# jhbastek/PhysicsInformedDiffusionModels

Measured on AMD Instinct MI355X. Metric: training samples/sec (UNet+PDE-residual step), 64x64 Darcy, higher is better.
Workload: dtype f32

## Files before the change

include/pidm.h:

```cpp
#ifndef PIDM_H
#define PIDM_H
#include <stddef.h>
#include <stdint.h>

#ifdef __cplusplus
extern "C" {
#endif

#define PIDM_ABI_VERSION 1

int pidm_version(void);
const char* pidm_last_error(void);
const char* pidm_backend(void);

int pidm_prof_enable(int on);
int pidm_prof_collect(double* ms4, long long* launches4, double* work4);
int pidm_prof_kernels_begin(void* stream);
long long pidm_prof_kernels_collect(char* buf, size_t cap);

int pidm_darcy_residual_fwd(const float* x0, const float* f_s, float inv_h0, float inv_h1,
                            float* residual, int B, int P, void* stream);
int pidm_darcy_residual_bwd(const float* x0, const float* grad_res, float inv_h0, float inv_h1,
                            float* grad_x0, int B, int P, void* stream);

size_t pidm_darcy_loss_ws(int B, int P);
int pidm_darcy_loss_fwd_bwd(const float* x0, const float* x0_pred, const float* f_s, const float* p2w,
                            const float* inv_var, float c_data, float c_residual, float inv_h0, float inv_h1,
                            float* residual, float* grad_x0_pred, float* out_scalars, void* workspace,
                            int B, int P, void* stream);
int pidm_darcy_loss_fwd_bwd_t(const float* x0, const float* x0_pred, const float* f_s, const int64_t* t,
                              const float* p2w_table, const float* var_table, float c_data, float c_residual,
                              float inv_h0, float inv_h1, float* residual, float* grad_x0_pred, float* out_scalars,
                              void* workspace, int B, int P, void* stream);

int pidm_darcy_jacobian_max(const float* x0, float inv_h0, float inv_h1, float* max_dr_dp, int B, int P, void* stream);

#define PIDM_STENCIL_MAX_OPS 5
#define PIDM_STENCIL_MAX_TAPS 49
typedef struct pidm_stencil_op {
  const int32_t* table;
  int mio, max_offset, ntaps;
} pidm_stencil_op;
int pidm_stencil_apply(const float* x, long long x_stride, const pidm_stencil_op* ops_host, float* const* outs_host, int K,
                       long long out_stride, int N, int H, int W, int periodic, void* stream);
int pidm_stencil_apply_adjoint(const float* const* gs_host, long long g_stride, const pidm_stencil_op* ops_host, int K,
                               const float* add, long long add_stride, float* gx, long long gx_stride, int N, int H, int W,
                               int periodic, void* stream);
size_t pidm_darcy_general_ws(int B, int P);
int pidm_darcy_residual_general_fwd(const float* x0, const float* f_s, const pidm_stencil_op* ops4_host, int periodic, float bc1_sign,
                                    float* residual, void* workspace, int B, int P, void* stream);
int pidm_darcy_residual_general_bwd(const float* x0, const float* grad_res, const pidm_stencil_op* ops4_host, int periodic,
                                    float bc1_sign, float* grad_x0, void* workspace, int B, int P, void* stream);

int pidm_qsample_nhwc(const float* x0, const float* eps, const float* a_t, const float* am1_t, float* xt_nhwc,
                      int B, int C, int HW, void* stream);
int pidm_qsample_nhwc_t(const float* x0, const float* eps, const int64_t* t, const float* a_table, const float* am1_table,
                        float* xt_nhwc, int B, int C, int HW, void* stream);
int pidm_psample_update(const float* x0_pred, const float* x_t, const float* z, float c1, float c2, float sigma,
                        float* x_prev, size_t n, void* stream);

size_t pidm_clip_adam_ws_bytes(void);
int pidm_clip_adam_step(float* param, const float* grad, float* exp_avg, float* exp_avg_sq, size_t n, double lr, double beta1,
                        double beta2, double eps, long long step, double max_norm, float* total_norm_out, void* workspace,
                        void* stream);

int pidm_clip_adam_ema_step(float* param, const float* grad, float* exp_avg, float* exp_avg_sq, float* ema_shadow, size_t n,
// ... 38 lines not shown
int pidm_mech_fields(const float* u_dofs, const float* rho, const float* kloc, int kloc_stride, const int32_t* elem_dofs, int nel,
                     double nu, float* fields, int B, void* stream);

typedef struct pidm_unet pidm_unet;
typedef struct pidm_unet_cfg {
  int dim;
  int channels;
  int out_dim;
  int n_levels;
  int dim_mults[8];
  int heads;
  int dim_head;
  int groups;
  int init_kernel;
  int image_size;
  int sigmoid_last_channel;
  int self_condition;
} pidm_unet_cfg;

int pidm_unet_create(const pidm_unet_cfg* cfg, pidm_unet** out);
void pidm_unet_destroy(pidm_unet* h);
int pidm_unet_num_params(const pidm_unet* h);
const char* pidm_unet_param_name(const pidm_unet* h, int i);
size_t pidm_unet_param_numel(const pidm_unet* h, int i);
size_t pidm_unet_workspace_bytes(const pidm_unet* h, int B, int training);
int pidm_unet_bind(pidm_unet* h, const void* const* param_ptrs_host, void* const* grad_ptrs_host);
int pidm_unet_forward(pidm_unet* h, const float* x_nhwc, const int64_t* t, float* out_nchw, int B,
                      int save_for_backward, int repack_weights, void* workspace, size_t workspace_bytes, void* stream);
int pidm_unet_num_cond_params(const pidm_unet* h);
int pidm_unet_enable_cond(pidm_unet* h, int on);
int pidm_unet_set_condition(pidm_unet* h, const float* cond_nhwc);
int pidm_unet_backward(pidm_unet* h, const float* grad_out_nchw, float* grad_x_nhwc, int B, void* workspace,
                       size_t workspace_bytes, void* stream);

int pidm_unet_set_grad_events(pidm_unet* h, int n_phases, void* const* events);
int pidm_unet_grad_phase_range(const pidm_unet* h, int n_phases, int phase, int* first_param, int* end_param);

typedef struct pidm_conv_desc {
  int B, Hi, Wi;
  int C0, C1;
  int ld0, ld1;
  int Cout;
  int KH, KW, stride, pad;
  int transposed;
  int out_nchw;
  int ldo;
} pidm_conv_desc;
size_t pidm_conv_packed_weight_floats(const pidm_conv_desc* d);
int pidm_conv_pack_weights(const pidm_conv_desc* d, const float* w_ref, float* w_packed, int mode, void* stream);
int pidm_conv_forward(const pidm_conv_desc* d, const float* src0, const float* src1, const float* w_packed,
                      const float* bias, const float* residual, float* out, void* stream);
int pidm_conv_forward_gn_partials(const pidm_conv_desc* d, const float* src0, const float* src1, const float* w_packed,
                                  const float* bias, float* out, int groups, double* partial, void* stream);
size_t pidm_conv_dgrad_packed_weight_floats(const pidm_conv_desc* d);
int pidm_conv_dgrad(const pidm_conv_desc* d, const float* dy, int ld_dy, const float* w_packed_dgrad,
                    const float* residual, float* dx, int ld_dx, void* stream);
size_t pidm_conv_wgrad_ws(const pidm_conv_desc* d);
int pidm_conv_wgrad(const pidm_conv_desc* d, const float* src0, const float* src1, const float* dy, int ld_dy,
                    float* dw_ref, float* dbias, void* workspace, void* stream);

size_t pidm_linear_attention_ws(int B, int N, int heads);
int pidm_linear_attention_forward(const float* qkv, float* out, float* kstat, float* ctx, float* qstat, int B, int N,
                                  int heads, void* workspace, void* stream);
int pidm_linear_attention_backward(const float* qkv, const float* kstat, const float* qstat, const float* ctx,
                                   const float* d_out, float* dqkv, int B, int N, int heads, void* workspace, void* stream);
int pidm_linear_attention_out_forward(const float* qkv, const float* w_out, const float* bias, const float* residual, float* y,
                                      int Cout, float* kstat, float* ctx, float* qstat, int B, int N, int heads, void* workspace,
                                      void* stream);
size_t pidm_linear_attention_out_backward_ws(int B, int N, int heads, int Cout);
int pidm_linear_attention_out_backward(const float* qkv, const float* kstat, const float* qstat, const float* ctx,
                                       const float* d_y, int ld_dy, const float* w_out, int Cout, float* dqkv, float* dw_out,
                                       int B, int N, int heads, void* workspace, void* stream);

size_t pidm_lap_ws(int B, int N, int heads, int C);
size_t pidm_lap_saved_floats(int B, int heads, int C);
int pidm_lap_forward(const float* xn, const float* w_qkv, const float* w_out, const float* bias, const float* resid, float* y,
                     float* saved, float* qstat, int C, int B, int N, int heads, void* workspace, void* stream);
int pidm_lap_backward(const float* xn, const float* dy, const float* w_qkv, const float* w_out, const float* saved,
                      const float* qstat, float* d_xn, float* d_w_qkv, float* d_w_out, int C, int B, int N, int heads,
                      void* workspace, void* stream);

int pidm_debug_stream_trace(unsigned long long* out256);
int pidm_debug_conv_rs_trace(unsigned long long* out4);
int pidm_debug_lap_trace(unsigned long long* out256);
long long pidm_debug_reduce_table_uploads(void);
int pidm_debug_launch_counts(long long* out4);
int pidm_comm_available(void);
int pidm_comm_unique_id(void* out128);
int pidm_comm_init(int rank, int world, const void* unique_id128, void** comm);
int pidm_allreduce_f32(void* comm, float* buf, size_t count, int average, void* stream);
int pidm_comm_destroy(void* comm);

int pidm_reload_knobs(void);

#ifdef __cplusplus
}
#endif
#endif
```

physicsinformeddiffusionmodels_amd/_engine.py:

```python
from __future__ import annotations

import contextlib
import ctypes as C
import math

import torch

from ._lib import PidmError, PidmLib, UnetCfg, get_lib, ptr, stream_ptr, vp


class UnetEngine:

    def __init__(self, model, image_size: int, lib: PidmLib | None = None):
        self.lib = lib or get_lib()
        cfg = UnetCfg()
        cfg.dim = model.dim
        cfg.channels = model.channels
        cfg.out_dim = model.out_dim
        cfg.n_levels = len(model.dim_mults)
        for i, m in enumerate(model.dim_mults):
            cfg.dim_mults[i] = int(m)
        cfg.heads = model.attn_heads
        cfg.dim_head = model.attn_dim_head
        cfg.groups = model.resnet_groups
        cfg.init_kernel = model.init_kernel_size
        cfg.image_size = image_size
        cfg.sigmoid_last_channel = int(bool(model.sigmoid_last_channel))
        cfg.self_condition = int(bool(model.self_condition))
        self.image_size = image_size
        self.handle = vp()
        self.lib.check(self.lib.pidm_unet_create(C.byref(cfg), C.byref(self.handle)), "pidm_unet_create")
        n = self.lib.pidm_unet_num_params(self.handle)
        self.names = [self.lib.pidm_unet_param_name(self.handle, i).decode() for i in range(n)]
        self.numels = [self.lib.pidm_unet_param_numel(self.handle, i) for i in range(n)]
        named = dict(model.named_parameters())
        missing = [k for k in self.names if k not in named]
        if missing:
            raise PidmError(f"engine parameter(s) not found in the model: {missing[:4]}")
        for k, ne in zip(self.names, self.numels):
            if named[k].numel() != ne:
                raise PidmError(f"parameter {k}: numel {named[k].numel()} != engine's {ne}")
        self.params = [named[k] for k in self.names]
        self.n_cond = self.lib.pidm_unet_num_cond_params(self.handle)
        self.cond_enabled = False
        self.flat_grad = None
        self.grad_views = None
        self.early_grad = None
        self.early_views = None
        self.early_generation = -1
        self._bound_key = None
        self.workspace = None
        self.backward_calls = 0
        self.tape_generation = 0
        self.tape_busy = False
        self._packed_for = None

    def __del__(self):
        try:
            if self.handle:
                self.lib.pidm_unet_destroy(self.handle)
        except Exception:
            pass

    def _flat_buffer(self, dev):
        total = sum(self.numels)
        flat = torch.zeros(total, dtype=torch.float32, device=dev)
        views, off = [], 0
        for p, ne in zip(self.params, self.numels):
            views.append(flat[off:off + ne].view(p.shape))
            off += ne
        return flat, views

    def _ensure_bound(self, need_grad: bool, early: bool = False):
        dev = self.params[0].device
        for p in self.params:
            if p.dtype != torch.float32 or not p.is_contiguous() or p.device != dev:
                raise PidmError("engine parameters must be contiguous fp32 tensors on one device")
        if need_grad and (self.flat_grad is None or self.flat_grad.device != dev):
            self.flat_grad, self.grad_views = self._flat_buffer(dev)
            self._bound_key = None
        if early and (self.early_grad is None or self.early_grad.device != dev):
            self.early_grad, self.early_views = self._flat_buffer(dev)
        with_grad = need_grad or self.flat_grad is not None
        target = (self.early_views if early else self.grad_views) if with_grad else None
        key = (tuple(p.data_ptr() for p in self.params), with_grad and target[0].data_ptr())
        if key != self._bound_key:
            n = len(self.params)
            pp = (vp * n)(*[vp(p.data_ptr()) for p in self.params])
            if with_grad:
                gp = (vp * n)(*[vp(g.data_ptr()) for g in target])
                self.lib.check(self.lib.pidm_unet_bind(self.handle, pp, gp), "pidm_unet_bind")
            else:
                self.lib.check(self.lib.pidm_unet_bind(self.handle, pp, None), "pidm_unet_bind")
            self._bound_key = key

    def _ensure_workspace(self, B: int, training: bool, device):
        nbytes = self.lib.pidm_unet_workspace_bytes(self.handle, B, int(training))
        if nbytes == 0:
            raise PidmError("pidm_unet_workspace_bytes: " + self.lib.lib.pidm_last_error().decode())
        if self.workspace is None or self.workspace.numel() < nbytes + 256 or self.workspace.device != torch.device(device):
            self.workspace = None
            self.workspace = torch.empty(nbytes + 256, dtype=torch.uint8, device=device)
        return self.workspace

    def forward(self, x_nhwc: torch.Tensor, t: torch.Tensor, training: bool, repack: bool = True,
                cond: torch.Tensor | None = None, early: bool = False, frozen=None) -> torch.Tensor:
        B = x_nhwc.shape[0]
        dev = x_nhwc.device
        self._ensure_bound(training, early=early)
        if cond is not None:
            if not self.cond_enabled:
                self.lib.check(self.lib.pidm_unet_enable_cond(self.handle, 1), "pidm_unet_enable_cond")
                self.cond_enabled = True
            self.lib.check(self.lib.pidm_unet_set_condition(self.handle, ptr(cond)), "pidm_unet_set_condition")
        ws = self._ensure_workspace(B, training, dev)
        P = self.image_size
        out = torch.empty(B, self.lib_out_dim, P, P, dtype=torch.float32, device=dev)
        base = ws.data_ptr()
        al = (-base) % 256
        if frozen is not None and not training and repack:
            key = (frozen, self._bound_key, base)
            repack = key != self._packed_for
            self._packed_for = key
        else:
            self._packed_for = None
        self.lib.check(self.lib.pidm_unet_forward(self.handle, ptr(x_nhwc), ptr(t), ptr(out), B, int(training), int(repack),
                                                  vp(base + al), ws.numel() - al, stream_ptr(dev)), "pidm_unet_forward")
        return out

    def backward(self, grad_out: torch.Tensor, want_grad_x: bool, channels: int):
        B = grad_out.shape[0]
        dev = grad_out.device
        ws = self.workspace
        gx = torch.empty(B, self.image_size * self.image_size, channels, dtype=torch.float32, device=dev) if want_grad_x else None
        base = ws.data_ptr()
        al = (-base) % 256
        self.lib.check(self.lib.pidm_unet_backward(self.handle, ptr(grad_out), ptr(gx), B, vp(base + al), ws.numel() - al,
                                                   stream_ptr(dev)), "pidm_unet_backward")
        return gx


class _TapeLease:

    __slots__ = ("engine", "generation")

    def __init__(self, engine, generation):
        self.engine, self.generation = engine, generation

    def release(self):
        eng = self.engine
        if eng is not None and eng.tape_generation == self.generation:
            eng.tape_busy = False
        self.engine = None

    def __del__(self):
        try:
            self.release()
        except Exception:
            pass


class _UnetFunction(torch.autograd.Function):

    @staticmethod
    def forward(ctx, engine: UnetEngine, x_nhwc, t, anchor, training: bool, cond=None, primary=None, frozen=None):
        ctx.engine = engine
        ctx.primary = primary if primary is not None else engine
        ctx.used_cond = cond is not None
        ctx.x_requires_grad = x_nhwc.requires_grad
        ctx.channels = x_nhwc.shape[-1]
        ctx.training = training
        if training:
            engine.tape_generation += 1
            engine.tape_busy = True
        ctx.generation = engine.tape_generation
        ctx.lease = _TapeLease(engine, engine.tape_generation) if training else None
        out = engine.forward(x_nhwc, t, training=training, cond=cond, frozen=frozen)
        if cond is not None:
            ctx.save_for_backward(out, x_nhwc, cond)
        else:
            ctx.save_for_backward(out, x_nhwc)
        return out

    @staticmethod
    def backward(ctx, grad_out):
        eng = ctx.engine
        if not ctx.training:
            raise PidmError("backward through a forward that ran without gradient tracking")
        if ctx.generation != eng.tape_generation:
            raise PidmError("the engine's activation tape was overwritten by a later training-mode forward of the same "
                            "model: only the latest differentiable UNet call can be differentiated (the two calls of "
                            "x0_estimation='sample' get one tape each through DenoisingDiffusion.ddim_sample_x0)")
        primary = ctx.primary
        first = eng.params[0]
        if primary.flat_grad is None:
            primary._ensure_bound(True)
        aliased = first.grad is not None and first.grad.data_ptr() == primary.grad_views[0].data_ptr()
        prev = primary.flat_grad.clone() if (aliased and eng is primary) else None
        gx = eng.backward(grad_out.contiguous(), ctx.x_requires_grad, ctx.channels)
        if prev is not None:
            eng.flat_grad.add_(prev)
        if eng is not primary:
            if aliased:
                primary.flat_grad.add_(eng.flat_grad)
            else:
                primary.flat_grad.copy_(eng.flat_grad)
        if ctx.lease is not None:
            ctx.lease.release()
        eng.tape_busy = False
        primary.backward_calls += 1 if (eng is primary and prev is None) else 2
        n_plain = len(eng.params) - eng.n_cond
        for i, (p, g) in enumerate(zip(eng.params, primary.grad_views)):
            if not p.requires_grad:
                continue
            if i >= n_plain and not ctx.used_cond:
                continue
            if p.grad is None:
                p.grad = g
            elif p.grad.data_ptr() != g.data_ptr():
                p.grad.add_(eng.grad_views[i] if eng is not primary else g)
        return None, gx, None, None, None, None, None, None


def get_engine(model, image_size: int, lib: PidmLib | None = None, slot: int = 0) -> UnetEngine:
    cache = model.__dict__.setdefault("_engines", {})
    key = (image_size, id(lib), slot)
    eng = cache.get(key)
    if eng is None:
        eng = UnetEngine(model, image_size, lib)
        eng.lib_out_dim = model.out_dim
        cache[key] = eng
    return eng


def used_parameter_names(model, image_size: int = 64, with_condition: bool = False):
    eng = get_engine(model, image_size)
    return list(eng.names) if with_condition else list(eng.names[:len(eng.names) - eng.n_cond])


@contextlib.contextmanager
def frozen_weights(model):
    prev = getattr(model, "_pidm_frozen", None)
    model._pidm_frozen = prev if prev is not None else object()
    try:
        yield
    finally:
        model._pidm_frozen = prev


def unet_apply(model, x, time, lib: PidmLib | None = None, cond=None, x_self_cond=None):
    video = False
    if x.dim() == 3:
        B, N, Cc = x.shape
        P = int(math.isqrt(N))
        if P * P != N:
            raise ValueError('Input [B, P*P, C] needs a square number of pixels.')
        x_nhwc = x
    elif x.dim() == 4:
        B, Cc, P, P2 = x.shape
        x_nhwc = x.permute(0, 2, 3, 1).reshape(B, P * P2, Cc)
    elif x.dim() == 5:
        video = True
        B, Cc, F_, P, P2 = x.shape
# ... 4 lines not shown
        raise ValueError('Input must be image [BxCxPxP] or image sequence [BxCxFxPxP].')
    if Cc != model.channels:
        raise ValueError(f'expected {model.channels} input channels, got {Cc}')
    if lib is None and not x.is_cuda:
        raise PidmError("Unet3D.forward needs tensors on an MI355X (cuda device): the gfx950 engine has no CPU fallback")
    if model.self_condition:
        if x_self_cond is None:
            sc = torch.zeros_like(x_nhwc)
        elif x_self_cond.dim() == 3:
            sc = x_self_cond
        elif x_self_cond.dim() == 4:
            sc = x_self_cond.permute(0, 2, 3, 1).reshape(B, P * P, Cc)
        else:
            sc = x_self_cond[:, :, 0].permute(0, 2, 3, 1).reshape(B, P * P, Cc)
        x_nhwc = torch.cat((sc.to(x_nhwc.dtype), x_nhwc), dim=-1)
    elif x_self_cond is not None:
        raise ValueError('x_self_cond given but the model was built with self_condition=False')
    x_nhwc = x_nhwc.contiguous().float()
    t = time.to(device=x.device, dtype=torch.int64).contiguous()
    if t.numel() != B:
        raise ValueError('time must have one entry per batch element')
    primary = eng = get_engine(model, P, lib)
    anchor = eng.params[0]
    training = torch.is_grad_enabled() and (anchor.requires_grad or x_nhwc.requires_grad)
    slot = getattr(model, "_pidm_tape_slot", None)
    if training and slot:
        eng = get_engine(model, P, lib, int(slot))
    if not training and eng.tape_busy:
        eng = get_engine(model, P, lib, slot=-1)
    if cond is not None:
        if cond.shape != (B, P * P, model.channels):
            raise ValueError(f'cond must be [B, P*P, {model.channels}], got {tuple(cond.shape)}')
        cond = cond.detach().contiguous().float()
    out = _UnetFunction.apply(eng, x_nhwc, t, anchor, training, cond, primary, getattr(model, "_pidm_frozen", None))
    if video:
        out = out.unsqueeze(2)
    return out
```

physicsinformeddiffusionmodels_amd/_lib.py:

```python
from __future__ import annotations

import ctypes as C
import os

_HERE = os.path.dirname(os.path.abspath(__file__))
DEFAULT_LIB = os.path.join(_HERE, "csrc", "libpidm_hip.so")

c_float_p = C.POINTER(C.c_float)
vp = C.c_void_p


class UnetCfg(C.Structure):
    _fields_ = [("dim", C.c_int), ("channels", C.c_int), ("out_dim", C.c_int), ("n_levels", C.c_int),
                ("dim_mults", C.c_int * 8), ("heads", C.c_int), ("dim_head", C.c_int), ("groups", C.c_int),
                ("init_kernel", C.c_int), ("image_size", C.c_int), ("sigmoid_last_channel", C.c_int),
                ("self_condition", C.c_int)]


class ConvDesc(C.Structure):
    _fields_ = [("B", C.c_int), ("Hi", C.c_int), ("Wi", C.c_int), ("C0", C.c_int), ("C1", C.c_int),
                ("ld0", C.c_int), ("ld1", C.c_int), ("Cout", C.c_int), ("KH", C.c_int), ("KW", C.c_int),
                ("stride", C.c_int), ("pad", C.c_int), ("transposed", C.c_int), ("out_nchw", C.c_int),
                ("ldo", C.c_int)]

# ... 4 lines not shown

class PidmError(RuntimeError):
    pass


_loaded: list = []


class PidmLib:
    def __init__(self, path: str | None = None):
        path = path or DEFAULT_LIB
        if not os.path.exists(path):
            raise PidmError(
                f"{path} not found: the gfx950 engine is not built. Run `python -c 'import __graft_entry__ as g; "
                f"g.build()'` (or `make -C physicsinformeddiffusionmodels_amd/csrc`). There is no CPU fallback.")
        self.path = path
        self.lib = C.CDLL(path)
        L = self.lib
        L.pidm_version.restype = C.c_int
        L.pidm_last_error.restype = C.c_char_p
        L.pidm_backend.restype = C.c_char_p
        i, f, sz = C.c_int, C.c_float, C.c_size_t
        self._sig("pidm_debug_reduce_table_uploads", [], C.c_longlong)
        self._sig("pidm_debug_launch_counts", [C.POINTER(C.c_longlong)])
        self._sig("pidm_prof_enable", [i])
        self._sig("pidm_prof_collect", [C.POINTER(C.c_double), C.POINTER(C.c_longlong), C.POINTER(C.c_double)])
        self._sig("pidm_prof_kernels_begin", [vp])
        self._sig("pidm_prof_kernels_collect", [C.c_char_p, sz], C.c_longlong)
        self._sig("pidm_darcy_residual_fwd", [vp, vp, f, f, vp, i, i, vp])
        self._sig("pidm_darcy_residual_bwd", [vp, vp, f, f, vp, i, i, vp])
        self._sig("pidm_darcy_loss_ws", [i, i], sz)
        self._sig("pidm_darcy_loss_fwd_bwd", [vp, vp, vp, vp, vp, f, f, f, f, vp, vp, vp, vp, i, i, vp])
        self._sig("pidm_darcy_loss_fwd_bwd_t", [vp, vp, vp, vp, vp, vp, f, f, f, f, vp, vp, vp, vp, i, i, vp])
        self._sig("pidm_darcy_jacobian_max", [vp, f, f, vp, i, i, vp])
        ll, ops = C.c_longlong, C.POINTER(StencilOp)
        self._sig("pidm_stencil_apply", [vp, ll, ops, C.POINTER(vp), i, ll, i, i, i, i, vp])
        self._sig("pidm_stencil_apply_adjoint", [C.POINTER(vp), ll, ops, i, vp, ll, vp, ll, i, i, i, i, vp])
        self._sig("pidm_darcy_general_ws", [i, i], sz)
        self._sig("pidm_darcy_residual_general_fwd", [vp, vp, ops, i, f, vp, vp, i, i, vp])
        self._sig("pidm_darcy_residual_general_bwd", [vp, vp, ops, i, f, vp, vp, i, i, vp])
        self._sig("pidm_qsample_nhwc", [vp, vp, vp, vp, vp, i, i, i, vp])
        self._sig("pidm_qsample_nhwc_t", [vp, vp, vp, vp, vp, vp, i, i, i, vp])
        self._sig("pidm_psample_update", [vp, vp, vp, f, f, f, vp, sz, vp])
        self._sig("pidm_mech_apply", [vp, vp, vp, vp, i, vp, vp, i, vp, vp, i, vp])
        self._sig("pidm_mech_solve_ws_bytes", [i, i], sz)
        self._sig("pidm_mech_solve", [vp, vp, vp, i, vp, vp, i, f, f, f, i, C.c_double, vp, vp, vp, vp, vp, vp, i, vp])
        self._sig("pidm_floating_material", [vp, f, i, vp, i, vp])
        self._sig("pidm_darcy_gen_lds_bytes", [i], sz)
        self._sig("pidm_darcy_gen", [vp, vp, i, vp, i, C.c_double, C.c_double, C.c_double, vp, vp, i, C.c_double, vp, vp, vp, vp, vp,
                                     i, vp])
        d = C.c_double
        self._sig("pidm_simp_ws_bytes", [i, i], sz)
        self._sig("pidm_simp_step", [vp, vp, vp, vp, vp, vp, i, vp, vp, i, d, d, d, d, i, i, d, vp, vp, vp, vp, vp, vp, vp, i, vp])
        self._sig("pidm_mech_fields", [vp, vp, vp, i, vp, i, d, vp, i, vp])
        self._sig("pidm_unet_num_cond_params", [vp])
        self._sig("pidm_unet_enable_cond", [vp, i])
        self._sig("pidm_unet_set_condition", [vp, vp])
        self._sig("pidm_clip_adam_ws_bytes", [], sz)
        self._sig("pidm_clip_adam_step", [vp, vp, vp, vp, sz, C.c_double, C.c_double, C.c_double, C.c_double, C.c_longlong,
                                          C.c_double, vp, vp, vp])
        self._sig("pidm_clip_adam_ema_step", [vp, vp, vp, vp, vp, sz, C.c_double, C.c_double, C.c_double, C.c_double, C.c_longlong,
                                              C.c_double, C.c_double, vp, vp, vp])
        self._sig("pidm_ema_update", [vp, vp, sz, C.c_double, vp])
        self._sig("pidm_mech_loss_ws", [i], sz)
        self._sig("pidm_mech_loss_fwd_bwd", [vp, vp, vp, vp, vp, vp, vp, f, f, f, f, vp, i, vp, vp, i, vp, vp, vp, i, vp])
        self._sig("pidm_bilinear_resize", [vp, vp, i, i, i, vp])
        self._sig("pidm_mech_residual_fwd", [vp, vp, vp, vp, i, vp, vp, i, vp, vp, vp, i, vp])
        self._sig("pidm_mech_residual_bwd", [vp, vp, vp, i, vp, vp, i, vp, vp, vp, vp, i, vp])
        self._sig("pidm_unet_create", [C.POINTER(UnetCfg), C.POINTER(vp)])
        self._sig("pidm_unet_destroy", [vp], None)
        self._sig("pidm_unet_num_params", [vp])
        self._sig("pidm_unet_param_name", [vp, i], C.c_char_p)
        self._sig("pidm_unet_param_numel", [vp, i], sz)
        self._sig("pidm_unet_workspace_bytes", [vp, i, i], sz)
        self._sig("pidm_unet_bind", [vp, C.POINTER(vp), C.POINTER(vp)])
        self._sig("pidm_unet_forward", [vp, vp, vp, vp, i, i, i, vp, sz, vp])
        self._sig("pidm_unet_backward", [vp, vp, vp, i, vp, sz, vp])
        self._sig("pidm_unet_set_grad_events", [vp, i, C.POINTER(vp)])
        self._sig("pidm_unet_grad_phase_range", [vp, i, i, C.POINTER(C.c_int), C.POINTER(C.c_int)])
        self._sig("pidm_conv_packed_weight_floats", [C.POINTER(ConvDesc)], sz)
        self._sig("pidm_conv_pack_weights", [C.POINTER(ConvDesc), vp, vp, i, vp])
        self._sig("pidm_conv_forward", [C.POINTER(ConvDesc), vp, vp, vp, vp, vp, vp, vp])
        self._sig("pidm_conv_dgrad_packed_weight_floats", [C.POINTER(ConvDesc)], sz)
        self._sig("pidm_conv_dgrad", [C.POINTER(ConvDesc), vp, i, vp, vp, vp, i, vp])
        self._sig("pidm_conv_forward_gn_partials", [C.POINTER(ConvDesc), vp, vp, vp, vp, vp, i, vp, vp])
        self._sig("pidm_conv_wgrad_ws", [C.POINTER(ConvDesc)], sz)
        self._sig("pidm_conv_wgrad", [C.POINTER(ConvDesc), vp, vp, vp, i, vp, vp, vp, vp])
        self._sig("pidm_linear_attention_ws", [i, i, i], sz)
        self._sig("pidm_linear_attention_forward", [vp, vp, vp, vp, vp, i, i, i, vp, vp])
        self._sig("pidm_linear_attention_backward", [vp, vp, vp, vp, vp, vp, i, i, i, vp, vp])
        self._sig("pidm_linear_attention_out_forward", [vp, vp, vp, vp, vp, i, vp, vp, vp, i, i, i, vp, vp])
        self._sig("pidm_linear_attention_out_backward_ws", [i, i, i, i], sz)
        self._sig("pidm_linear_attention_out_backward", [vp, vp, vp, vp, vp, i, vp, i, vp, vp, i, i, i, vp, vp])
        self._sig("pidm_lap_ws", [i, i, i, i], sz)
        self._sig("pidm_lap_saved_floats", [i, i, i], sz)
        self._sig("pidm_lap_forward", [vp, vp, vp, vp, vp, vp, vp, vp, i, i, i, i, vp, vp])
        self._sig("pidm_lap_backward", [vp, vp, vp, vp, vp, vp, vp, vp, vp, i, i, i, i, vp, vp])
        self._sig("pidm_debug_stream_trace", [vp])
        self._sig("pidm_debug_conv_rs_trace", [C.POINTER(C.c_ulonglong)])
        self._sig("pidm_debug_lap_trace", [vp])
        self._sig("pidm_reload_knobs", [])
        self._sig("pidm_comm_available", [])
        self._sig("pidm_comm_unique_id", [vp])
        self._sig("pidm_comm_init", [i, i, vp, C.POINTER(vp)])
        self._sig("pidm_allreduce_f32", [vp, vp, sz, i, vp])
        self._sig("pidm_comm_destroy", [vp])
        _loaded.append(self)
        if L.pidm_version() != 1:
            raise PidmError(f"{path}: ABI version {L.pidm_version()} != 1")

# ... 49 lines not shown
```

physicsinformeddiffusionmodels_amd/csrc/k_attn.hip:

```cpp
#include "pidm_launch.h"

namespace pidm {

static const int DH = 32;

__device__ __forceinline__ float fexp(float x) { return __expf(x); }

__global__ void __launch_bounds__(256) la_kstats_kernel(const float* __restrict__ qkv, int N, int HD, int nseg,
                                                        float* __restrict__ kpart, float* __restrict__ kstat) {
  __shared__ float sm[4][64], ssum[4][64];
  const int b = blockIdx.y, seg = blockIdx.z, tid = threadIdx.x, cl = tid & 63, rl = tid >> 6;
  const int j = blockIdx.x * 64 + cl;
  const int per = (N + nseg - 1) / nseg;
  const int n_lo = seg * per, n_hi = (n_lo + per < N) ? n_lo + per : N;
  float m = -3.0e38f, s = 0.f;
  if (j < HD) {
    const float* base = qkv + (size_t)b * N * 3 * HD + HD + j;
    int n = n_lo + rl;
    for (; n + 28 < n_hi; n += 32) {
      float v[8];
#pragma unroll
      for (int u = 0; u < 8; ++u) v[u] = base[(size_t)(n + 4 * u) * 3 * HD];
      float gm = v[0];
#pragma unroll
// ... 17 lines not shown
  __syncthreads();
  if (rl == 0 && j < HD) {
    float M = fmaxf(fmaxf(sm[0][cl], sm[1][cl]), fmaxf(sm[2][cl], sm[3][cl]));
    float S = 0.f;
    for (int r = 0; r < 4; ++r) S += ssum[r][cl] * fexp(sm[r][cl] - M);
    if (kstat) {
      kstat[((size_t)b * HD + j) * 2] = M;
      kstat[((size_t)b * HD + j) * 2 + 1] = 1.f / S;
    } else {
      kpart[(((size_t)b * nseg + seg) * HD + j) * 2] = M;
      kpart[(((size_t)b * nseg + seg) * HD + j) * 2 + 1] = S;
    }
  }
}
__global__ void la_kstats_final_kernel(const float* __restrict__ kpart, int B, int HD, int nseg, float* __restrict__ kstat) {
  const int i = blockIdx.x * blockDim.x + threadIdx.x;
  if (i >= B * HD) return;
  const int b = i / HD, j = i % HD;
  float M = -3.0e38f;
  for (int sg = 0; sg < nseg; ++sg) M = fmaxf(M, kpart[(((size_t)b * nseg + sg) * HD + j) * 2]);
  float S = 0.f;
  for (int sg = 0; sg < nseg; ++sg) {
    const float* p = kpart + (((size_t)b * nseg + sg) * HD + j) * 2;
    S += p[1] * fexp(p[0] - M);
  }
  kstat[(size_t)i * 2] = M;
  kstat[(size_t)i * 2 + 1] = 1.f / S;
}

template <int MODE>
__global__ void __launch_bounds__(256) la_nreduce_kernel(const float* __restrict__ qkv, const float* __restrict__ stat,
                                                         const float* __restrict__ dA, const float* __restrict__ ctx,
                                                         float* __restrict__ Dpart, int N, int heads, float scale,
                                                         float* __restrict__ Dfinal, float* __restrict__ rowdot, float alpha) {
  __shared__ float red[4][1024];
  const int bh = blockIdx.x, b = bh / heads, h = bh % heads;
  const int ns = blockIdx.y, NS = gridDim.y;
  const int HD = heads * DH;
  const int tid = threadIdx.x, lane = tid & 63, half = lane >> 5, l31 = lane & 31;
  const int wave = __builtin_amdgcn_readfirstlane(tid >> 6);
  f32x16 acc;
  for (int r = 0; r < 16; ++r) acc[r] = 0.f;
  const float* q0 = qkv + (size_t)b * N * 3 * HD;
  float cm = 0.f, cis = 0.f;
  if (MODE == 0) {
    cm = stat[((size_t)b * HD + h * DH + l31) * 2];
    cis = stat[((size_t)b * HD + h * DH + l31) * 2 + 1];
  }
  const int per_blk = (N + NS - 1) / NS;
  const int blk_lo = ns * per_blk, blk_hi = (blk_lo + per_blk < N) ? blk_lo + per_blk : N;
  const int per = (blk_hi - blk_lo + 3) / 4;
  const int n_lo = blk_lo + wave * per, n_hi = (n_lo + per < blk_hi) ? n_lo + per : blk_hi;
  int n0 = n_lo;
  {
    constexpr int UNR = 4;
    const int la = half * 3 * HD + (MODE == 0 ? HD : 0) + h * DH + l31;
    const int lb = (MODE == 0) ? half * 3 * HD + 2 * HD + h * DH + l31 : half * HD + h * DH + l31;
    const int ls = (half * heads + h) * 2;
    for (; n0 + 2 * UNR <= n_hi; n0 += 2 * UNR) {
      const float* qrow = q0 + (size_t)n0 * 3 * HD;
      const float* brow = (MODE == 0) ? qrow : dA + ((size_t)b * N + n0) * HD;
      const float* srow = (MODE == 0) ? nullptr : stat + ((size_t)b * N + n0) * heads * 2;
      float av[UNR], bvv[UNR];
      float2 qs[UNR];
#pragma unroll
      for (int u = 0; u < UNR; ++u) {
        av[u] = (qrow + (size_t)(2 * u) * 3 * HD)[la];
        bvv[u] = (brow + (size_t)(2 * u) * (MODE == 0 ? 3 * HD : HD))[lb];
        if (MODE == 1) qs[u] = *reinterpret_cast<const float2*>(srow + (size_t)(2 * u) * heads * 2 + ls);
      }
#pragma unroll
      for (int u = 0; u < UNR; ++u) {
        const float a = (MODE == 0) ? fexp(av[u] - cm) * cis : fexp(av[u] - qs[u].x) * qs[u].y * scale;
        acc = __builtin_amdgcn_mfma_f32_32x32x2f32(a, bvv[u], acc, 0, 0, 0);
      }
    }
  }
  for (; n0 < n_hi; n0 += 2) {
// ... 892 lines not shown
#pragma unroll 8
      for (int s2 = 0; s2 < 32; ++s2)
        acc = __builtin_amdgcn_mfma_f32_32x32x2f32(sdS_[(32 * t + l31) * LS + 2 * s2 + half], sk[2 * s2 + half][l31], acc, 0, 0, 0);
    } else {
#pragma unroll 8
      for (int s2 = 0; s2 < 32; ++s2)
        acc = __builtin_amdgcn_mfma_f32_32x32x2f32(sdS_[(2 * s2 + half) * LS + 32 * t + l31], sq[2 * s2 + half][l31], acc, 0, 0, 0);
    }
    const float f = wave < 2 ? scale : 1.f;
    const size_t col = (wave < 2 ? 0 : HD) + h * DH + l31;
#pragma unroll
    for (int r = 0; r < 16; ++r)
      out[((size_t)b * N + 32 * t + (r & 3) + 8 * (r >> 2) + 4 * half) * 3 * HD + col] = acc[r] * f;
  }
}

static int la_nsplit(int N) {
  int ns = N / 512;
  if (ns < 1) ns = 1;
  if (ns > 8) ns = 8;
  return ns;
}
static int la_kseg(int N) {
  int s = N / 256;
  if (s < 1) s = 1;
  if (s > 16) s = 16;
  return s;
}
size_t la_scratch_floats(int B, int N, int heads) {
  const size_t a = (size_t)B * la_kseg(N) * heads * DH * 2, b = (size_t)B * heads * la_nsplit(N) * 1024;
  return a + b + (size_t)heads * DH * 128 + 64;
}

int launch_la_forward(const float* qkv, float* kstat, float* ctx, float* attn, float* qstat, int B, int N, int heads,
                      float* scratch, hipStream_t st) {
  const int HD = heads * DH;
  const float scale = 0.17677669529663687f;
  const int nseg = la_kseg(N), NS = la_nsplit(N);
  float* kpart = scratch;
  float* dpart = scratch + (size_t)B * nseg * HD * 2;
  hipLaunchKernelGGL(la_kstats_kernel, dim3(cdiv(HD, 64), B, nseg), dim3(256), 0, st, qkv, N, HD, nseg, kpart, nseg == 1 ? kstat : nullptr);
  PIDM_CHECK_LAUNCH("la_kstats_kernel");
  if (nseg > 1) {
    hipLaunchKernelGGL(la_kstats_final_kernel, dim3(cdiv(B * HD, 256)), dim3(256), 0, st, kpart, B, HD, nseg, kstat);
    PIDM_CHECK_LAUNCH("la_kstats_final_kernel");
  }
  hipLaunchKernelGGL(HIP_KERNEL_NAME(la_nreduce_kernel<0>), dim3(B * heads, NS), dim3(256), 0, st, qkv, kstat, nullptr, nullptr,
                     dpart, N, heads, scale, NS == 1 ? ctx : nullptr, nullptr, 1.f / (float)N);
  PIDM_CHECK_LAUNCH("la_context");
  if (NS > 1) {
    hipLaunchKernelGGL(HIP_KERNEL_NAME(la_nreduce_final_kernel<0>), dim3(B * heads), dim3(256), 0, st, dpart, nullptr, ctx, nullptr, NS,
                       1.f / (float)N);
    PIDM_CHECK_LAUNCH("la_context_final");
  }
  const size_t npix = (size_t)B * N;
  if (N % 32 == 0)
    hipLaunchKernelGGL(HIP_KERNEL_NAME(la_out_kernel<true>), dim3((unsigned)((npix + 127) / 128), (npix + 127) / 128 < 1024 ? heads : 1), dim3(256), 0, st, qkv, ctx, attn,
                       qstat, N, heads, npix, scale);
  else
    hipLaunchKernelGGL(HIP_KERNEL_NAME(la_out_kernel<false>), dim3((unsigned)((npix + 127) / 128), (npix + 127) / 128 < 1024 ? heads : 1), dim3(256), 0, st, qkv, ctx, attn,
                       qstat, N, heads, npix, scale);
  PIDM_CHECK_LAUNCH("la_out_kernel");
  return 0;
}

int launch_la_backward(const float* qkv, const float* kstat, const float* qstat, const float* ctx, const float* dA, float* dctx,
                       float* rowdot, float* dqkv, int B, int N, int heads, float* scratch, hipStream_t st) {
  const float scale = 0.17677669529663687f;
  const int NS = la_nsplit(N);
  float* dpart = scratch;
  hipLaunchKernelGGL(HIP_KERNEL_NAME(la_nreduce_kernel<1>), dim3(B * heads, NS), dim3(256), 0, st, qkv, qstat, dA, ctx, dpart, N, heads,
                     scale, NS == 1 ? dctx : nullptr, rowdot, 1.f);
  PIDM_CHECK_LAUNCH("la_dctx");
  if (NS > 1) {
    hipLaunchKernelGGL(HIP_KERNEL_NAME(la_nreduce_final_kernel<1>), dim3(B * heads), dim3(256), 0, st, dpart, ctx, dctx, rowdot, NS, 1.f);
    PIDM_CHECK_LAUNCH("la_dctx_final");
  }
  if (N % 32 == 0 && N >= 64) {
    const size_t npix = (size_t)B * N;
    int ppb = N % 128 == 0 ? 128 : (N % 64 == 0 ? 64 : 32);
    (void)npix;
    if (const char* pe = knob("PIDM_LA_PPB")) { const int v = atoi(pe); if ((v == 32 || v == 64 || v == 128) && N % v == 0) ppb = v; }
    PIDM_PROF_NAME("la_bwd_pix_mfma_kernel");
    hipLaunchKernelGGL(la_bwd_pix_mfma_kernel, dim3((unsigned)((size_t)B * N / ppb), heads), dim3(2 * ppb), 0, st, qkv, kstat, qstat, ctx,
                       dctx, rowdot, dA, dqkv, N, heads, scale, ppb);
  } else {
    hipLaunchKernelGGL(la_bwd_pix_kernel, dim3(cdiv(N, 256), B * heads), dim3(256), 0, st, qkv, kstat, qstat, ctx, dctx, rowdot,
                       dA, dqkv, N, heads, scale);
  }
  PIDM_CHECK_LAUNCH("la_bwd_pix_kernel");
  return 0;
}

bool la_fused_ok(int N, int heads, int Cout, int ld_dy) {
  const bool off = knob("PIDM_NO_LA_FUSED") != nullptr;
  return !off && N % 128 == 0 && (Cout == 32 || Cout == 64 || Cout == 128) && (ld_dy & 3) == 0 && heads >= 1 && heads <= 14;
}
int launch_la_forward_fused(const float* qkv, float* kstat, float* ctx, float* qstat, const float* w_out, const float* bias,
                            const float* resid, float* y, int Cout, int B, int N, int heads, float* scratch, hipStream_t st) {
  if (!la_fused_ok(N, heads, Cout, Cout)) return fail("fused attention forward: N=%d Cout=%d not eligible", N, Cout);
  const int HD = heads * DH;
  const float scale = 0.17677669529663687f;
  const int nseg = la_kseg(N), NS = la_nsplit(N);
  float* kpart = scratch;
  float* dpart = scratch + (size_t)B * nseg * HD * 2;
  hipLaunchKernelGGL(la_kstats_kernel, dim3(cdiv(HD, 64), B, nseg), dim3(256), 0, st, qkv, N, HD, nseg, kpart, nseg == 1 ? kstat : nullptr);
  PIDM_CHECK_LAUNCH("la_kstats_kernel");
  if (nseg > 1) {
    hipLaunchKernelGGL(la_kstats_final_kernel, dim3(cdiv(B * HD, 256)), dim3(256), 0, st, kpart, B, HD, nseg, kstat);
    PIDM_CHECK_LAUNCH("la_kstats_final_kernel");
  }
  hipLaunchKernelGGL(HIP_KERNEL_NAME(la_nreduce_kernel<0>), dim3(B * heads, NS), dim3(256), 0, st, qkv, kstat, nullptr, nullptr,
                     dpart, N, heads, scale, NS == 1 ? ctx : nullptr, nullptr, 1.f / (float)N);
  PIDM_CHECK_LAUNCH("la_context");
  if (NS > 1) {
    hipLaunchKernelGGL(HIP_KERNEL_NAME(la_nreduce_final_kernel<0>), dim3(B * heads), dim3(256), 0, st, dpart, nullptr, ctx, nullptr, NS,
                       1.f / (float)N);
    PIDM_CHECK_LAUNCH("la_context_final");
  }
  float* wt = dpart + (size_t)B * heads * NS * 1024;
  hipLaunchKernelGGL(la_wt_kernel, dim3(cdiv(Cout * HD, 256)), dim3(256), 0, st, w_out, wt, Cout, HD);
  PIDM_CHECK_LAUNCH("la_wt_kernel");
  const dim3 grid((unsigned)((size_t)B * N / 128));
  if (Cout == 32)
    hipLaunchKernelGGL(HIP_KERNEL_NAME(la_out_proj_kernel<1>), grid, dim3(256), 0, st, qkv, ctx, wt, bias, resid, y, qstat, N, heads, scale);
  else if (Cout == 64)
    hipLaunchKernelGGL(HIP_KERNEL_NAME(la_out_proj_kernel<2>), grid, dim3(256), 0, st, qkv, ctx, wt, bias, resid, y, qstat, N, heads, scale);
  else
    hipLaunchKernelGGL(HIP_KERNEL_NAME(la_out_proj_kernel<4>), grid, dim3(256), 0, st, qkv, ctx, wt, bias, resid, y, qstat, N, heads, scale);
  PIDM_CHECK_LAUNCH("la_out_proj_kernel");
  return 0;
}

bool la_fused_pays(int B, int N) {
  const char* mw = knob("PIDM_LA_FUSED_MIN_WGS");
  const long min_wgs = mw ? atol(mw) : 256;
  return (long)B * N / 128 >= min_wgs;
}
size_t la_fused_scratch_floats(int B, int N, int heads, int Cout) {
  return (size_t)B * heads * la_nsplit(N) * (Cout / 32) * 1024 + 64;
}
int launch_la_backward_fused(const float* qkv, const float* kstat, const float* qstat, const float* ctx, const float* dy, int ld_dy,
                             const float* w_out, int Cout, float* dctx, float* rowdot, float* dqkv, float* dwpart, int B, int N,
                             int heads, float* scratch, hipStream_t st) {
  if (!la_fused_ok(N, heads, Cout, ld_dy)) return fail("fused attention backward: N=%d Cout=%d not eligible", N, Cout);
  const float scale = 0.17677669529663687f;
  const int NS = la_nsplit(N);
  float* gpart = scratch;
  const dim3 grid(B * heads, NS);
#define PIDM_LA_G(NT_)                                                                                                        \
  {                                                                                                                           \
    hipLaunchKernelGGL(HIP_KERNEL_NAME(la_g_kernel<NT_>), grid, dim3(256), 0, st, qkv, qstat, dy, ld_dy, gpart, N, heads, scale); \
// ... 108 lines not shown
```

physicsinformeddiffusionmodels_amd/csrc/k_darcy.hip:

```cpp
#include <stdlib.h>

#include "pidm_common.h"

namespace pidm {

struct FdAxis {
  float c1[3][4];
  float c2[3][4];
};

__device__ __forceinline__ float fd_apply(const float (&c)[3][4], const float* a, int i, int P, int s, int ntap_edge) {
  float r = 0.f;
  if (i == 0) {
    for (int k = 0; k < ntap_edge; ++k) r = fmaf(c[0][k], a[k * s], r);
  } else if (i == P - 1) {
    for (int k = 0; k < ntap_edge; ++k) r = fmaf(c[2][k], a[(P - 1 - k) * s], r);
  } else {
    for (int k = 0; k < 3; ++k) r = fmaf(c[1][k], a[(i - 1 + k) * s], r);
  }
  return r;
}

__device__ __forceinline__ float fd_coef(const float (&c)[3][4], int i, int m, int P, int ntap_edge) {
  if (i == 0) return (m < ntap_edge) ? c[0][m] : 0.f;
// ... 75 lines not shown
}
struct FdTaps5 {
  int idx[5];
  float w1[5], w2[5];
};
__device__ __forceinline__ FdTaps5 fd_taps_T(const FdAxis& ax, int m, int P, int lo, int hi) {
  FdTaps5 t;
  const int rows[5] = {0, P - 1, m - 1, m, m + 1};
#pragma unroll
  for (int k = 0; k < 5; ++k) {
    const int i = rows[k];
    float a1 = 0.f, a2 = 0.f;
    if (k == 0) {
      const int q = m < 4 ? m : 3;
      a1 = (m < 3) ? ax.c1[0][q] : 0.f;
      a2 = (m < 4) ? ax.c2[0][q] : 0.f;
    } else if (k == 1) {
      const int d = P - 1 - m, q = d < 4 ? d : 3;
      a1 = (d < 3) ? ax.c1[2][q] : 0.f;
      a2 = (d < 4) ? ax.c2[2][q] : 0.f;
    } else {
      const bool ok = (i >= 1) & (i <= P - 2);
      const int q = m - (i - 1);
      a1 = ok ? ax.c1[1][q] : 0.f;
      a2 = ok ? ax.c2[1][q] : 0.f;
    }
    t.w1[k] = a1;
    t.w2[k] = a2;
    t.idx[k] = i < lo ? lo : (i > hi ? hi : i);
  }
  return t;
}

template <int MODE>
__global__ void __launch_bounds__(256) darcy_kernel(const float* __restrict__ x0,
                                                    const float* __restrict__ pred,
                                                    const float* __restrict__ f_s,
                                                    const float* __restrict__ grad_res,
                                                    const float* __restrict__ p2w, const float* __restrict__ inv_var,
                                                    const long long* __restrict__ tsteps,
                                                    float c_data, float c_res, float bc1_sign, FdAxis ax0, FdAxis ax1,
                                                    float* __restrict__ residual, float* __restrict__ grad_pred,
                                                    double* __restrict__ partial,
                                                    int B, int P, int R, int nb, int lds_rows) {
  HIP_DYNAMIC_SHARED(float, smem)
  const int N = P * P;
  const int b = blockIdx.x / nb, band = blockIdx.x - b * nb;
  const int tid = threadIdx.x;
  const int r0 = band * R, r1 = (r0 + R < P) ? r0 + R : P;
  int ilo = r0, ihi = r1;
  if (MODE != DARCY_RES_ONLY) {
    ilo = (r0 < 4) ? 0 : r0 - 1;
    ihi = (r1 > P - 4) ? P : r1 + 1;
  }
  int dlo = (ilo > 0) ? ilo - 1 : 0, dhi = (ihi < P) ? ihi + 1 : P;
  if (ilo == 0 && dhi < 4) dhi = 4;
  if (ihi == P && dlo > P - 4) dlo = P - 4;
  const int F = lds_rows * P;
  float* sp = smem - dlo * P;
  float* sK = sp + F;
  float* skg = sp + 2 * F;
  float* sa0 = sp + 3 * F;
  float* sa1 = sp + 4 * F;
  float* sb0 = sp + 5 * F;
  float* sb1 = sp + 6 * F;
  float* sd = sp + 7 * F;
  const float* pb = pred + (size_t)b * 2 * N;
  const int dj = 256 % P, di = 256 / P;

  double acc_data = 0.0, acc_r2 = 0.0, acc_rabs = 0.0;
  for (int n = dlo * P + tid; n < dhi * P; n += 256) {
    float vp = pb[n], vK = pb[N + n];
    sp[n] = vp;
    sK[n] = vK;
    if (MODE == DARCY_LOSS && n >= r0 * P && n < r1 * P) {
      float d0 = x0[(size_t)b * 2 * N + n] - vp, d1 = x0[(size_t)b * 2 * N + N + n] - vK;
      acc_data += (double)(d0 * d0) + (double)(d1 * d1);
// ... 64 lines not shown
        ++i;
        tj = fd_taps(ax1, j, P, 0, P - 1);
      } else if (dj) {
        tj = fd_taps(ax1, j, P, 0, P - 1);
      }
    }
  }
  if (MODE == DARCY_RES_ONLY) return;
  __syncthreads();

  const float dscale = (MODE == DARCY_LOSS) ? 2.f * c_data * darcy_p2w(p2w, tsteps, b) / ((float)B * 2.f * (float)N) : 0.f;
  {
    int i = r0 + tid / P, j = tid - (tid / P) * P;
    FdTaps5 tj = fd_taps_T(ax1, j, P, 0, P - 1);
    for (int n = r0 * P + tid; n < r1 * P; n += 256) {
      const FdTaps5 ti = fd_taps_T(ax0, i, P, ilo, ihi - 1);
      float g00 = 0.f, g11 = 0.f, ga0 = 0.f, ga1 = 0.f, gb0 = 0.f, gb1 = 0.f;
#pragma unroll
      for (int k = 0; k < 5; ++k) {
        const int c0 = ti.idx[k] * P + j, c1 = i * P + tj.idx[k];
        g00 = fmaf(ti.w2[k], skg[c0], g00);
        ga0 = fmaf(ti.w1[k], sa0[c0], ga0);
        gb0 = fmaf(ti.w1[k], sb0[c0], gb0);
        g11 = fmaf(tj.w2[k], skg[c1], g11);
        ga1 = fmaf(tj.w1[k], sa1[c1], ga1);
        gb1 = fmaf(tj.w1[k], sb1[c1], gb1);
      }
      float gp = ((g00 + g11) + ga0) + ga1;
      float gK = (sd[n] + gb0) + gb1;
      if (MODE == DARCY_LOSS) {
        gp += dscale * (sp[n] - x0[(size_t)b * 2 * N + n]);
        gK += dscale * (sK[n] - x0[(size_t)b * 2 * N + N + n]);
      }
      grad_pred[(size_t)b * 2 * N + n] = gp;
      grad_pred[(size_t)b * 2 * N + N + n] = gK;
      j += dj;
      i += di;
      if (j >= P) {
        j -= P;
        ++i;
        tj = fd_taps_T(ax1, j, P, 0, P - 1);
      } else if (dj) {
        tj = fd_taps_T(ax1, j, P, 0, P - 1);
      }
    }
  }

  if (MODE == DARCY_LOSS) {
    __shared__ double red[3][4];
    double v[3] = {acc_data, acc_r2, acc_rabs};
    for (int q = 0; q < 3; ++q) {
      double x = v[q];
      for (int off = 32; off > 0; off >>= 1) x += __shfl_down(x, off);
      if ((tid & 63) == 0) red[q][tid >> 6] = x;
    }
    __syncthreads();
    if (tid < 3) {
      double s = red[tid][0] + red[tid][1] + red[tid][2] + red[tid][3];
      partial[(size_t)blockIdx.x * 4 + tid] = s;
    }
  }
}

__device__ __forceinline__ float fd_edge3(const float (&c)[4], float a0, float a1, float a2) { return fmaf(c[2], a2, fmaf(c[1], a1, c[0] * a0)); }
__device__ __forceinline__ float fd_edge4(const float (&c)[4], float a0, float a1, float a2, float a3) {
  return fmaf(c[3], a3, fmaf(c[2], a2, fmaf(c[1], a1, c[0] * a0)));
}
__device__ __forceinline__ void quad_d1(const FdAxis& ax, const float (&w)[6], bool lowq, bool highq, float (&d)[4]) {
// ... 20 lines not shown
    const int col = j0 + m, d = P - 1 - col;
    const int qa = col < 4 ? col : 3, qb = d < 4 ? d : 3;
    t.e0[m] = (col < nt) ? c[0][qa] : 0.f;
    t.eP[m] = (d < nt) ? c[2][qb] : 0.f;
    t.m1[m] = (col - 1 >= 1 && col - 1 <= P - 2) ? c[1][2] : 0.f;
    t.z0[m] = (col >= 1 && col <= P - 2) ? c[1][1] : 0.f;
    t.p1[m] = (col + 1 >= 1 && col + 1 <= P - 2) ? c[1][0] : 0.f;
  }
  return t;
}
__device__ __forceinline__ void quad_gather(const QuadT& t, float a0, float aP, const float (&w)[6], float (&g)[4]) {
#pragma unroll
  for (int m = 0; m < 4; ++m) {
    float r = t.e0[m] * a0;
    r = fmaf(t.eP[m], aP, r);
    r = fmaf(t.m1[m], w[m], r);
    r = fmaf(t.z0[m], w[m + 1], r);
    g[m] = fmaf(t.p1[m], w[m + 2], r);
  }
}
__device__ __forceinline__ void quad_window(const float* rowp, int j0, int P, float (&w)[6]) {
  const f32x4 v = *reinterpret_cast<const f32x4*>(rowp + j0);
  w[0] = rowp[j0 > 0 ? j0 - 1 : 0];
  w[1] = v[0]; w[2] = v[1]; w[3] = v[2]; w[4] = v[3];
  w[5] = rowp[j0 + 4 < P ? j0 + 4 : P - 1];
}

template <int MODE>
__global__ void __launch_bounds__(512) darcy_quad_kernel(const float* __restrict__ x0, const float* __restrict__ pred,
                                                         const float* __restrict__ f_s, const float* __restrict__ grad_res,
                                                         const float* __restrict__ p2w, const float* __restrict__ inv_var,
                                                         const long long* __restrict__ tsteps, float c_data, float c_res, float bc1_sign,
                                                         FdAxis ax0, FdAxis ax1, float* __restrict__ residual, float* __restrict__ grad_pred,
                                                         double* __restrict__ partial, int B, int P, int R, int nb, int lds_rows) {
  HIP_DYNAMIC_SHARED(float, smem)
  const int N = P * P, QP = P >> 2;
  const int b = blockIdx.x / nb, band = blockIdx.x - b * nb;
  const int tid = threadIdx.x;
  const int r0 = band * R, r1 = (r0 + R < P) ? r0 + R : P;
  int ilo = r0, ihi = r1;
  if (MODE != DARCY_RES_ONLY) {
    ilo = (r0 < 4) ? 0 : r0 - 1;
    ihi = (r1 > P - 4) ? P : r1 + 1;
  }
  int dlo = (ilo > 0) ? ilo - 1 : 0, dhi = (ihi < P) ? ihi + 1 : P;
  if (ilo == 0 && dhi < 4) dhi = 4;
  if (ihi == P && dlo > P - 4) dlo = P - 4;
  const int F = lds_rows * P;
  float* sp = smem - dlo * P;
  float* sK = sp + F;
  float* skg = sp + 2 * F;
  float* sa0 = sp + 3 * F;
  float* sa1 = sp + 4 * F;
  float* sb0 = sp + 5 * F;
  float* sb1 = sp + 6 * F;
  float* sd = sp + 7 * F;
  const float* pb = pred + (size_t)b * 2 * N;
  const float* tb = x0 + (size_t)b * 2 * N;
  const int q = tid & (QP - 1), j0 = 4 * q, rstep = (int)blockDim.x / QP, rt = tid / QP;
  const bool lowq = q == 0, highq = q == QP - 1;

  double acc_data = 0.0, acc_r2 = 0.0, acc_rabs = 0.0;
  for (int i = dlo + rt; i < dhi; i += rstep) {
    const int n = i * P + j0;
    const f32x4 vp = *reinterpret_cast<const f32x4*>(pb + n), vK = *reinterpret_cast<const f32x4*>(pb + N + n);
    *reinterpret_cast<f32x4*>(sp + n) = vp;
    *reinterpret_cast<f32x4*>(sK + n) = vK;
// ... 107 lines not shown
      const f32x4 vkg = *reinterpret_cast<const f32x4*>(skg + c0), va = *reinterpret_cast<const f32x4*>(sa0 + c0),
                  vb = *reinterpret_cast<const f32x4*>(sb0 + c0);
#pragma unroll
      for (int m = 0; m < 4; ++m) {
        g00[m] = fmaf(ti.w2[k], vkg[m], g00[m]);
        ga0[m] = fmaf(ti.w1[k], va[m], ga0[m]);
        gb0[m] = fmaf(ti.w1[k], vb[m], gb0[m]);
      }
    }
    float w[6], g11[4], ga1[4], gb1[4];
    const int row = i * P;
    quad_window(skg + row, j0, P, w);
    quad_gather(t2, skg[row], skg[row + P - 1], w, g11);
    quad_window(sa1 + row, j0, P, w);
    quad_gather(t1, sa1[row], sa1[row + P - 1], w, ga1);
    quad_window(sb1 + row, j0, P, w);
    quad_gather(t1, sb1[row], sb1[row + P - 1], w, gb1);
    const f32x4 vd = *reinterpret_cast<const f32x4*>(sd + n);
    f32x4 gp, gK;
#pragma unroll
    for (int m = 0; m < 4; ++m) {
      gp[m] = ((g00[m] + g11[m]) + ga0[m]) + ga1[m];
      gK[m] = (vd[m] + gb0[m]) + gb1[m];
    }
    if (MODE == DARCY_LOSS) {
      const f32x4 vp = *reinterpret_cast<const f32x4*>(sp + n), vK = *reinterpret_cast<const f32x4*>(sK + n);
      const f32x4 t0 = *reinterpret_cast<const f32x4*>(tb + n), t1v = *reinterpret_cast<const f32x4*>(tb + N + n);
#pragma unroll
      for (int m = 0; m < 4; ++m) {
        gp[m] += dscale * (vp[m] - t0[m]);
        gK[m] += dscale * (vK[m] - t1v[m]);
      }
    }
    *reinterpret_cast<f32x4*>(grad_pred + (size_t)b * 2 * N + n) = gp;
    *reinterpret_cast<f32x4*>(grad_pred + (size_t)b * 2 * N + N + n) = gK;
  }

  if (MODE == DARCY_LOSS) {
    __shared__ double red[3][8];
    double v[3] = {acc_data, acc_r2, acc_rabs};
    for (int qq = 0; qq < 3; ++qq) {
      double x = v[qq];
      for (int off = 32; off > 0; off >>= 1) x += __shfl_down(x, off);
      if ((tid & 63) == 0) red[qq][tid >> 6] = x;
    }
    __syncthreads();
    if (tid < 3) {
      double sv = 0.0;
      for (int w = 0; w < (int)blockDim.x >> 6; ++w) sv += red[tid][w];
      partial[(size_t)blockIdx.x * 4 + tid] = sv;
    }
  }
}

__device__ __forceinline__ void quad_window_regs(const float (&v)[4], bool lowq, bool highq, float (&w)[6]) {
  const float left = __shfl_up(v[3], 1, 16), right = __shfl_down(v[0], 1, 16);
  w[0] = lowq ? v[0] : left;
  w[1] = v[0]; w[2] = v[1]; w[3] = v[2]; w[4] = v[3];
  w[5] = highq ? v[3] : right;
}
template <int MODE, int NT>
__global__ void __launch_bounds__(NT, 2) darcy_full_kernel(const float* __restrict__ x0, const float* __restrict__ pred,
                                                        const float* __restrict__ f_s, const float* __restrict__ grad_res,
                                                        const float* __restrict__ p2w, const float* __restrict__ inv_var,
                                                        const long long* __restrict__ tsteps, float c_data, float c_res, float bc1_sign,
                                                        FdAxis ax0, FdAxis ax1, float* __restrict__ residual, float* __restrict__ grad_pred,
                                                        double* __restrict__ partial, int B) {
  constexpr int P = 64, N = P * P, RS = NT / 16, NIT = P / RS;
  HIP_DYNAMIC_SHARED(float, smem)
  float* sp = smem;
  float* sK = sp + N;
  float* skg = sp + 2 * N;
  float* sa0 = sp + 3 * N;
  float* sb0 = sp + 4 * N;
  const int b = blockIdx.x, tid = threadIdx.x;
  const int q = tid & 15, j0 = 4 * q, rt = tid >> 4;
  const bool lowq = q == 0, highq = q == 15;
  const float* pb = pred + (size_t)b * 2 * N;
  const float* tb = x0 + (size_t)b * 2 * N;
  f32x4 vp[NIT], vK[NIT], t0[NIT], t1[NIT];
#pragma unroll
  for (int it = 0; it < NIT; ++it) {
    const int n = (rt + RS * it) * P + j0;
    vp[it] = *reinterpret_cast<const f32x4*>(pb + n);
    vK[it] = *reinterpret_cast<const f32x4*>(pb + N + n);
    if (MODE == DARCY_LOSS) {
      t0[it] = *reinterpret_cast<const f32x4*>(tb + n);
      t1[it] = *reinterpret_cast<const f32x4*>(tb + N + n);
    }
  }
  double acc_data = 0.0, acc_r2 = 0.0, acc_rabs = 0.0;
#pragma unroll
  for (int it = 0; it < NIT; ++it) {
    const int n = (rt + RS * it) * P + j0;
    *reinterpret_cast<f32x4*>(sp + n) = vp[it];
    *reinterpret_cast<f32x4*>(sK + n) = vK[it];
    if (MODE == DARCY_LOSS) {
#pragma unroll
      for (int m = 0; m < 4; ++m) {
        t0[it][m] = vp[it][m] - t0[it][m];
// ... 105 lines not shown
    float g00[4] = {0.f, 0.f, 0.f, 0.f}, ga0[4] = {0.f, 0.f, 0.f, 0.f}, gb0[4] = {0.f, 0.f, 0.f, 0.f};
#pragma unroll
    for (int k = 0; k < 5; ++k) {
      const int c0 = ti.idx[k] * P + j0;
      const f32x4 vkg = *reinterpret_cast<const f32x4*>(skg + c0), va = *reinterpret_cast<const f32x4*>(sa0 + c0),
                  vb = *reinterpret_cast<const f32x4*>(sb0 + c0);
#pragma unroll
      for (int m = 0; m < 4; ++m) {
        g00[m] = fmaf(ti.w2[k], vkg[m], g00[m]);
        ga0[m] = fmaf(ti.w1[k], va[m], ga0[m]);
        gb0[m] = fmaf(ti.w1[k], vb[m], gb0[m]);
      }
    }
    float w[6], g11[4], ga1[4], gb1[4];
    quad_window_regs(rkg[it], lowq, highq, w);
    quad_gather(tq2, __shfl(rkg[it][0], 0, 16), __shfl(rkg[it][3], 15, 16), w, g11);
    quad_window_regs(ra1[it], lowq, highq, w);
    quad_gather(tq1, __shfl(ra1[it][0], 0, 16), __shfl(ra1[it][3], 15, 16), w, ga1);
    quad_window_regs(rb1[it], lowq, highq, w);
    quad_gather(tq1, __shfl(rb1[it][0], 0, 16), __shfl(rb1[it][3], 15, 16), w, gb1);
    f32x4 gp, gK;
#pragma unroll
    for (int m = 0; m < 4; ++m) {
      gp[m] = ((g00[m] + g11[m]) + ga0[m]) + ga1[m];
      gK[m] = (rd[it][m] + gb0[m]) + gb1[m];
    }
    if (MODE == DARCY_LOSS) {
#pragma unroll
      for (int m = 0; m < 4; ++m) {
        gp[m] += dscale * t0[it][m];
        gK[m] += dscale * t1[it][m];
      }
    }
    *reinterpret_cast<f32x4*>(grad_pred + (size_t)b * 2 * N + n) = gp;
    *reinterpret_cast<f32x4*>(grad_pred + (size_t)b * 2 * N + N + n) = gK;
  }

  if (MODE == DARCY_LOSS) {
    double (*red)[NT / 64] = reinterpret_cast<double (*)[NT / 64]>(sp);
    double v[3] = {acc_data, acc_r2, acc_rabs};
    for (int qq = 0; qq < 3; ++qq) {
      double x = v[qq];
      for (int off = 32; off > 0; off >>= 1) x += __shfl_down(x, off);
      if ((tid & 63) == 0) red[qq][tid >> 6] = x;
    }
    __syncthreads();
    if (tid < 3) {
      double sv = 0.0;
      for (int w = 0; w < NT / 64; ++w) sv += red[tid][w];
      partial[(size_t)blockIdx.x * 4 + tid] = sv;
    }
  }
}

#ifndef PIDM_DARCY_TRACE_BUILD
#define PIDM_DARCY_TRACE_BUILD 0
#endif
#if PIDM_DARCY_TRACE_BUILD
__device__ unsigned long long g_darcy_trace[4 * 64];
#define PIDM_DARCY_STAMP(slot_) \
  do { if (blockIdx.x == 0 && threadIdx.x == 0 && n_done < 64) g_darcy_trace[4 * n_done + (slot_)] = clock64(); } while (0)
#else
#define PIDM_DARCY_STAMP(slot_) ((void)0)
#endif
__global__ void __launch_bounds__(512, 2) darcy_stream_kernel(const float* __restrict__ x0, const float* __restrict__ pred,
                                                              const float* __restrict__ f_s, const float* __restrict__ p2w,
                                                              const float* __restrict__ inv_var, const long long* __restrict__ tsteps,
                                                              float c_data, float c_res, float bc1_sign, FdAxis ax0, FdAxis ax1,
                                                              float* __restrict__ residual, float* __restrict__ grad_pred,
                                                              double* __restrict__ partial, int B) {
  constexpr int P = 64, N = P * P, NT = 512, RS = NT / 16, NIT = P / RS;
  HIP_DYNAMIC_SHARED(float, smem)
  float* spb = smem;
  float* sKb = smem + 2 * N;
  float* tg = smem + 3 * N;
  float* skg = smem + 5 * N;
  float* sa0 = smem + 6 * N;
  float* sb0 = smem + 7 * N;
  float* sfs = smem + 8 * N;
  double (*red)[NT / 64] = reinterpret_cast<double (*)[NT / 64]>(smem + 9 * N);
  FdTaps4* tab4 = reinterpret_cast<FdTaps4*>(smem + 9 * N + 48);
  int* tab5 = reinterpret_cast<int*>(smem + 9 * N + 48 + 64 * 12);
  QuadT* tabq = reinterpret_cast<QuadT*>(smem + 9 * N + 48 + 64 * 12 + 64 * 16);
  const int tid = threadIdx.x, wave = __builtin_amdgcn_readfirstlane(tid >> 6), lane = tid & 63;
  const int q0 = tid & 15, rt0 = tid >> 4;
  auto fetch = [&](const float* g, float* l) {
#pragma unroll
    for (int k = 0; k < 2; ++k) {
      const int piece = wave + 8 * k;
      pidm_glds_b128_untracked(g + piece * 256 + lane * 4, l + piece * 256);
    }
  };
  if (tid < P) {
    tab4[tid] = fd_taps(ax0, tid, P, 0, P - 1);
    *reinterpret_cast<FdTaps5*>(tab5 + tid * 16) = fd_taps_T(ax0, tid, P, 0, P - 1);
  } else if (tid < P + 16) {
    tabq[2 * (tid - P)] = quad_T(ax1.c1, 4 * (tid - P), P, 3);
    tabq[2 * (tid - P) + 1] = quad_T(ax1.c2, 4 * (tid - P), P, 4);
  }
  int b = blockIdx.x, b_prev = -1, cur = 0;
  [[maybe_unused]] int n_done = 0;
  if (b < B) {
    fetch(f_s, sfs);
// ... 126 lines not shown
    const QuadT tq1 = tabq[2 * q], tq2 = tabq[2 * q + 1];
#pragma unroll
    for (int it = 0; it < NIT; ++it) {
      const int i = rt + RS * it, n = i * P + j0;
      const FdTaps5 ti = *reinterpret_cast<const FdTaps5*>(tab5 + i * 16);
      float g00[4] = {0.f, 0.f, 0.f, 0.f}, ga0[4] = {0.f, 0.f, 0.f, 0.f}, gb0[4] = {0.f, 0.f, 0.f, 0.f};
#pragma unroll
      for (int k = 0; k < 5; ++k) {
        const int c0 = ti.idx[k] * P + j0;
        const f32x4 vkg = *reinterpret_cast<const f32x4*>(skg + c0), va = *reinterpret_cast<const f32x4*>(sa0 + c0),
                    vb = *reinterpret_cast<const f32x4*>(sb0 + c0);
#pragma unroll
        for (int m = 0; m < 4; ++m) {
          g00[m] = fmaf(ti.w2[k], vkg[m], g00[m]);
          ga0[m] = fmaf(ti.w1[k], va[m], ga0[m]);
          gb0[m] = fmaf(ti.w1[k], vb[m], gb0[m]);
        }
      }
      float w[6], g11[4], ga1[4], gb1[4];
      quad_window_regs(rkg[it], lowq, highq, w);
      quad_gather(tq2, __shfl(rkg[it][0], 0, 16), __shfl(rkg[it][3], 15, 16), w, g11);
      quad_window_regs(ra1[it], lowq, highq, w);
      quad_gather(tq1, __shfl(ra1[it][0], 0, 16), __shfl(ra1[it][3], 15, 16), w, ga1);
      quad_window_regs(rb1[it], lowq, highq, w);
      quad_gather(tq1, __shfl(rb1[it][0], 0, 16), __shfl(rb1[it][3], 15, 16), w, gb1);
      f32x4 gp, gK;
#pragma unroll
      for (int m = 0; m < 4; ++m) {
        gp[m] = ((g00[m] + g11[m]) + ga0[m]) + ga1[m];
        gK[m] = (rd[it][m] + gb0[m]) + gb1[m];
        gp[m] += dscale * t0[it][m];
        gK[m] += dscale * t1[it][m];
      }
      *reinterpret_cast<f32x4*>(grad_pred + (size_t)b * 2 * N + n) = gp;
      *reinterpret_cast<f32x4*>(grad_pred + (size_t)b * 2 * N + N + n) = gK;
    }
    double v[3] = {acc_data, acc_r2, acc_rabs};
    for (int qq = 0; qq < 3; ++qq) {
      double x = v[qq];
      for (int off = 32; off > 0; off >>= 1) x += __shfl_down(x, off);
      if (lane == 0) red[qq][wave] = x;
    }
    PIDM_DARCY_STAMP(3);
    ++n_done;
  }
  __syncthreads();
  if (b_prev >= 0 && tid < 3) {
    double sv = 0.0;
    for (int w = 0; w < NT / 64; ++w) sv += red[tid][w];
    partial[(size_t)b_prev * 4 + tid] = sv;
  }
}

__global__ void __launch_bounds__(256) darcy_loss_finalize(const double* __restrict__ partial, const float* __restrict__ p2w,
                                                           const float* __restrict__ inv_var, const long long* __restrict__ tsteps,
                                                           float c_data, float c_res, int B, int N, int nb, float* __restrict__ out) {
  __shared__ double red[3][4];
  const int tid = threadIdx.x;
  double v[3] = {0.0, 0.0, 0.0};
  for (int b = tid; b < B; b += 256) {
    double d = 0.0, r = 0.0, a = 0.0;
    for (int k = 0; k < nb; ++k) {
      const double* pp = partial + ((size_t)b * nb + k) * 4;
      d += pp[0];
      r += pp[1];
      a += pp[2];
    }
    v[0] += d / (2.0 * N) * (double)darcy_p2w(p2w, tsteps, b);
// ... 43 lines not shown
  float mx = 0.f;
  for (int n = tid; n < N; n += 256) {
    const int i = n / P, j = n - i * P;
    const float Kv = sK[n];
    const float K0 = fd_apply(ax0.c1, sK + j, i, P, P, 3);
    const float K1 = fd_apply(ax1.c1, sK + i * P, j, P, 1, 3);
    const float s0 = (i == 0) ? -1.f : ((i == P - 1) ? 1.f : 0.f);
    const float s1 = (j == 0) ? bc1_sign : ((j == P - 1) ? -bc1_sign : 0.f);
    const int klo = (i == 0) ? 0 : ((i == P - 1) ? P - 4 : i - 1), khi = (i == 0) ? 3 : ((i == P - 1) ? P - 1 : i + 1);
    const int llo = (j == 0) ? 0 : ((j == P - 1) ? P - 4 : j - 1), lhi = (j == 0) ? 3 : ((j == P - 1) ? P - 1 : j + 1);
    const float e1_c = -Kv * fd_coef(ax1.c2, j, j, P, 4) - K1 * fd_coef(ax1.c1, j, j, P, 3);
    for (int k = klo; k <= khi; ++k) {
      const float d0 = fd_coef(ax0.c1, i, k, P, 3);
      float e = -Kv * fd_coef(ax0.c2, i, k, P, 4) - K0 * d0;
      if (k == i) e += e1_c;
      mx = fmaxf(mx, e);
      mx = fmaxf(mx, s0 * d0);
    }
    for (int l = llo; l <= lhi; ++l) {
      const float d1 = fd_coef(ax1.c1, j, l, P, 3);
      if (l != j) mx = fmaxf(mx, -Kv * fd_coef(ax1.c2, j, l, P, 4) - K1 * d1);
      mx = fmaxf(mx, s1 * d1);
    }
  }
  for (int off = 32; off > 0; off >>= 1) mx = fmaxf(mx, __shfl_down(mx, off));
  if ((tid & 63) == 0) red[tid >> 6] = mx;
  __syncthreads();
  if (tid == 0) out[b] = fmaxf(fmaxf(red[0], red[1]), fmaxf(red[2], red[3]));
}

template <int MODE>
static int launch_darcy(const float* x0, const float* pred, const float* f_s, const float* grad_res, const float* p2w,
                        const float* inv_var, const long long* tsteps, float c_data, float c_res, float inv_h0, float inv_h1,
                        float* residual, float* grad_pred, double* partial, int B, int P, hipStream_t st) {
  if (B <= 0 || P < 5) return fail("darcy: need B>0 and P>=5 (got B=%d P=%d)", B, P);
  const DarcyBands bd = darcy_bands(B, P, MODE == DARCY_RES_ONLY);
  const int rows = darcy_lds_rows(P, bd.R);
  size_t lds = (size_t)(MODE == DARCY_RES_ONLY ? 2 : 8) * rows * P * sizeof(float);
  if (lds > 160 * 1024 - 256) return fail("darcy: P=%d does not fit the 160 KiB LDS", P);
  static bool attr_done = false;
  if (!attr_done) {
    (void)hipFuncSetAttribute(reinterpret_cast<const void*>(&darcy_kernel<MODE>),
                              hipFuncAttributeMaxDynamicSharedMemorySize, 160 * 1024 - 256);
    attr_done = true;
  }
  const int QP = P >> 2;
  const char* qe = knob("PIDM_DARCY_QUAD");
  const bool quad = (P & 3) == 0 && P >= 8 && QP <= 256 && (QP & (QP - 1)) == 0 && !(qe && !atoi(qe)) &&
                    ((reinterpret_cast<size_t>(pred) | reinterpret_cast<size_t>(x0) | reinterpret_cast<size_t>(f_s) |
                      reinterpret_cast<size_t>(residual) | reinterpret_cast<size_t>(grad_pred) | reinterpret_cast<size_t>(grad_res)) & 15) == 0;
  if (quad && MODE == DARCY_LOSS && darcy_full_on(B, P) && darcy_stream_on()) {
    static bool attr_s = false;
    const size_t lds_s = (size_t)9 * 64 * 64 * sizeof(float) + 3 * 8 * sizeof(double) + (64 * 12 + 64 * 16 + 16 * 40) * sizeof(float);
    if (!attr_s) {
      if (hipFuncSetAttribute(reinterpret_cast<const void*>(&darcy_stream_kernel), hipFuncAttributeMaxDynamicSharedMemorySize, (int)lds_s) != hipSuccess) {
        (void)hipGetLastError();
        return fail("darcy_stream_kernel: the device refuses %zu bytes of dynamic LDS", lds_s);
      }
      attr_s = true;
    }
    const char* e = knob("PIDM_DARCY_STREAM_WGS");
    int wgs = e ? atoi(e) : 256;
    if (wgs < 1) wgs = 1;
    if (wgs > B) wgs = B;
    hipLaunchKernelGGL(darcy_stream_kernel, dim3((unsigned)wgs), dim3(512), lds_s, st, x0, pred, f_s, p2w, inv_var, tsteps, c_data, c_res,
                       (inv_h1 < 0.f) ? 1.f : -1.f, make_axis(inv_h0), make_axis(inv_h1), residual, grad_pred, partial, B);
    PIDM_CHECK_LAUNCH("darcy_stream_kernel");
    return 0;
  }
  if (quad && MODE != DARCY_RES_ONLY && darcy_full_on(B, P)) {
    static bool attr_f = false;
    const size_t lds_f = (size_t)5 * 64 * 64 * sizeof(float);
    if (!attr_f) {
      if (hipFuncSetAttribute(reinterpret_cast<const void*>(&darcy_full_kernel<MODE, 512>), hipFuncAttributeMaxDynamicSharedMemorySize, (int)lds_f) != hipSuccess) {
        (void)hipGetLastError();
        return fail("darcy_full_kernel: the device refuses %zu bytes of dynamic LDS", lds_f);
      }
      attr_f = true;
    }
    hipLaunchKernelGGL(HIP_KERNEL_NAME(darcy_full_kernel<MODE, 512>), dim3((unsigned)B), dim3(512), lds_f, st, x0, pred, f_s, grad_res, p2w, inv_var,
                       tsteps, c_data, c_res, (inv_h1 < 0.f) ? 1.f : -1.f, make_axis(inv_h0), make_axis(inv_h1), residual, grad_pred, partial, B);
    PIDM_CHECK_LAUNCH("darcy_full_kernel");
    return 0;
  }
  if (quad) {
    static bool attr_q = false;
    if (!attr_q) {
      (void)hipFuncSetAttribute(reinterpret_cast<const void*>(&darcy_quad_kernel<MODE>), hipFuncAttributeMaxDynamicSharedMemorySize, 160 * 1024 - 256);
      attr_q = true;
    }
    int nt = QP * ((bd.R + 4 < P) ? bd.R + 4 : P);
    nt = (nt + 63) / 64 * 64;
    if (nt > 256) nt = 256;
    if (nt < QP) nt = QP;
    if (nt < 64) nt = 64;
    hipLaunchKernelGGL(HIP_KERNEL_NAME(darcy_quad_kernel<MODE>), dim3((unsigned)B * bd.nb), dim3(nt), lds, st, x0, pred, f_s, grad_res, p2w,
                       inv_var, tsteps, c_data, c_res, (inv_h1 < 0.f) ? 1.f : -1.f, make_axis(inv_h0), make_axis(inv_h1), residual,
                       grad_pred, partial, B, P, bd.R, bd.nb, rows);
    PIDM_CHECK_LAUNCH("darcy_quad_kernel");
    return 0;
  }
  hipLaunchKernelGGL(HIP_KERNEL_NAME(darcy_kernel<MODE>), dim3((unsigned)B * bd.nb), dim3(256), lds, st, x0, pred, f_s, grad_res, p2w,
                     inv_var, tsteps, c_data, c_res, (inv_h1 < 0.f) ? 1.f : -1.f, make_axis(inv_h0), make_axis(inv_h1), residual,
                     grad_pred, partial, B, P, bd.R, bd.nb, rows);
  PIDM_CHECK_LAUNCH("darcy_kernel");
  return 0;
}

static int darcy_loss_impl(const float* x0, const float* x0_pred, const float* f_s, const float* p2w, const float* inv_var,
                           const long long* tsteps, float c_data, float c_residual, float inv_h0, float inv_h1, float* residual,
                           float* grad_x0_pred, float* out_scalars, void* workspace, int B, int P, hipStream_t st) {
  double* partial = reinterpret_cast<double*>(workspace);
  int rc = launch_darcy<DARCY_LOSS>(x0, x0_pred, f_s, nullptr, p2w, inv_var, tsteps, c_data, c_residual, inv_h0, inv_h1, residual,
                                    grad_x0_pred, partial, B, P, st);
  if (rc) return rc;
  hipLaunchKernelGGL(darcy_loss_finalize, dim3(1), dim3(256), 0, st, partial, p2w, inv_var, tsteps, c_data, c_residual, B, P * P,
                     darcy_bands(B, P).nb, out_scalars);
  PIDM_CHECK_LAUNCH("darcy_loss_finalize");
  return 0;
}

}

using namespace pidm;

extern "C" int pidm_darcy_residual_fwd(const float* x0, const float* f_s, float inv_h0, float inv_h1, float* residual,
                                       int B, int P, void* stream) {
  return launch_darcy<DARCY_RES_ONLY>(nullptr, x0, f_s, nullptr, nullptr, nullptr, nullptr, 0.f, 0.f, inv_h0, inv_h1, residual,
                                      nullptr, nullptr, B, P, as_stream(stream));
}

extern "C" int pidm_darcy_residual_bwd(const float* x0, const float* grad_res, float inv_h0, float inv_h1,
                                       float* grad_x0, int B, int P, void* stream) {
  return launch_darcy<DARCY_BWD>(nullptr, x0, nullptr, grad_res, nullptr, nullptr, nullptr, 0.f, 0.f, inv_h0, inv_h1, nullptr,
                                 grad_x0, nullptr, B, P, as_stream(stream));
}

extern "C" size_t pidm_darcy_loss_ws(int B, int P) {
  if (B <= 0 || P < 5) return 0;
  return (size_t)B * darcy_bands(B, P).nb * 4 * sizeof(double);
}

extern "C" int pidm_darcy_loss_fwd_bwd(const float* x0, const float* x0_pred, const float* f_s, const float* p2w,
                                       const float* inv_var, float c_data, float c_residual, float inv_h0,
                                       float inv_h1, float* residual, float* grad_x0_pred, float* out_scalars,
                                       void* workspace, int B, int P, void* stream) {
  return darcy_loss_impl(x0, x0_pred, f_s, p2w, inv_var, nullptr, c_data, c_residual, inv_h0, inv_h1, residual, grad_x0_pred,
                         out_scalars, workspace, B, P, as_stream(stream));
}

extern "C" int pidm_darcy_loss_fwd_bwd_t(const float* x0, const float* x0_pred, const float* f_s, const int64_t* t,
                                         const float* p2w_table, const float* var_table, float c_data, float c_residual,
                                         float inv_h0, float inv_h1, float* residual, float* grad_x0_pred, float* out_scalars,
                                         void* workspace, int B, int P, void* stream) {
  if (!t || !p2w_table || !var_table) return fail("darcy_loss_fwd_bwd_t: null time steps / tables");
  return darcy_loss_impl(x0, x0_pred, f_s, p2w_table, var_table, reinterpret_cast<const long long*>(t), c_data, c_residual, inv_h0,
                         inv_h1, residual, grad_x0_pred, out_scalars, workspace, B, P, as_stream(stream));
}

extern "C" int pidm_darcy_jacobian_max(const float* x0, float inv_h0, float inv_h1, float* max_dr_dp, int B, int P, void* stream) {
  if (!x0 || !max_dr_dp) return fail("darcy_jacobian_max: null buffer");
  if (B <= 0 || P < 5) return fail("darcy: need B>0 and P>=5 (got B=%d P=%d)", B, P);
  const size_t lds = (size_t)P * P * sizeof(float);
  if (lds > 160 * 1024 - 256) return fail("darcy: P=%d does not fit the 160 KiB LDS", P);
  static bool attr_done = false;
  if (!attr_done) {
    (void)hipFuncSetAttribute(reinterpret_cast<const void*>(&darcy_jacmax_kernel), hipFuncAttributeMaxDynamicSharedMemorySize, 160 * 1024 - 256);
    attr_done = true;
  }
  hipLaunchKernelGGL(darcy_jacmax_kernel, dim3(B), dim3(256), lds, as_stream(stream), x0, (inv_h1 < 0.f) ? 1.f : -1.f,
                     make_axis(inv_h0), make_axis(inv_h1), max_dr_dp, P);
  PIDM_CHECK_LAUNCH("darcy_jacmax_kernel");
  return 0;
}

#if PIDM_DARCY_TRACE_BUILD
extern "C" int pidm_debug_darcy_trace(unsigned long long* out256) {
  return hipMemcpyFromSymbol(out256, HIP_SYMBOL(pidm::g_darcy_trace), sizeof(unsigned long long) * 256) == hipSuccess ? 0 : -1;
}
#endif
```

physicsinformeddiffusionmodels_amd/csrc/k_norm.hip:

```cpp
#include "pidm_launch.h"

namespace pidm {

__device__ __forceinline__ float sigmoidf_(float v) { return pidm_sigmoid(v); }

__global__ void __launch_bounds__(256) gn_stats_partial_kernel(const float* __restrict__ x, int HW, int C, int G, int ppb,
                                                               double* __restrict__ partial) {
  __shared__ double red[4][64][2];
  const int b = blockIdx.y, chunk = blockIdx.x, tid = threadIdx.x;
  const int cpg = C / G;
  const int g = tid % G, pl = tid / G, ppi = 256 / G;
  const int p0 = chunk * ppb;
  const int p1 = (p0 + ppb < HW) ? p0 + ppb : HW;
  float s = 0.f, ss = 0.f;
  for (int p = p0 + pl; p < p1; p += ppi) {
    const float* row = x + ((size_t)b * HW + p) * C + g * cpg;
    if ((cpg & 3) == 0) {
      for (int k = 0; k < cpg; k += 4) {
        const float4 v = *reinterpret_cast<const float4*>(row + k);
        s += (v.x + v.y) + (v.z + v.w);
        ss += (v.x * v.x + v.y * v.y) + (v.z * v.z + v.w * v.w);
      }
    } else {
      for (int k = 0; k < cpg; ++k) {
// ... 692 lines not shown
  for (size_t i = (size_t)blockIdx.x * blockDim.x + threadIdx.x; i < n; i += (size_t)gridDim.x * blockDim.x) {
    const float v = x[i];
    y[i] = act == 0 ? v * sigmoidf_(v) : 0.5f * v * (1.f + erff(v * 0.70710678118654752440f));
  }
}
__global__ void act_bwd_kernel(const float* __restrict__ x, const float* __restrict__ dy, float* __restrict__ dx, size_t n,
                               int act) {
  for (size_t i = (size_t)blockIdx.x * blockDim.x + threadIdx.x; i < n; i += (size_t)gridDim.x * blockDim.x) {
    const float v = x[i];
    float d;
    if (act == 0) {
      const float sg = sigmoidf_(v);
      d = sg * (1.f + v * (1.f - sg));
    } else {
      const float cdf = 0.5f * (1.f + erff(v * 0.70710678118654752440f));
      d = cdf + v * 0.39894228040143267794f * expf(-0.5f * v * v);
    }
    dx[i] = dy[i] * d;
  }
}

__global__ void sinusoid_kernel(const int64_t* __restrict__ t, float* __restrict__ emb, int B, int dim) {
  const int i = blockIdx.x * blockDim.x + threadIdx.x;
  const int half = dim / 2;
  if (i >= B * half) return;
  const int b = i / half, k = i % half;
  const float e = (float)(9.210340371976184 / (double)(half - 1));
  const float w = expf((float)k * -e);
  const float arg = (float)t[b] * w;
  emb[(size_t)b * dim + k] = sinf(arg);
  emb[(size_t)b * dim + half + k] = cosf(arg);
}

__global__ void copy_add_kernel(float* __restrict__ dst, int ldd, const float* __restrict__ a, int lda,
                                const float* __restrict__ b, int ldb, size_t rows, int cols) {
  const int c4 = cols / 4;
  const size_t total = rows * c4;
  for (size_t i = (size_t)blockIdx.x * blockDim.x + threadIdx.x; i < total; i += (size_t)gridDim.x * blockDim.x) {
    const size_t r = i / c4;
    const int c = (int)(i % c4) * 4;
    float4 v = *reinterpret_cast<const float4*>(a + r * lda + c);
    if (b) {
      const float4 w = *reinterpret_cast<const float4*>(b + r * ldb + c);
      v.x += w.x; v.y += w.y; v.z += w.z; v.w += w.w;
    }
    *reinterpret_cast<float4*>(dst + r * ldd + c) = v;
  }
}

__global__ void nchw_to_nhwc_kernel(const float* __restrict__ src, float* __restrict__ dst, int B, int C, int HW,
                                    const float* __restrict__ y_for_sigmoid_bwd) {
  const size_t total = (size_t)B * C * HW;
  for (size_t i = (size_t)blockIdx.x * blockDim.x + threadIdx.x; i < total; i += (size_t)gridDim.x * blockDim.x) {
    const int c = (int)(i % C);
    const size_t p = (i / C) % HW, b = i / ((size_t)C * HW);
    float v = src[(b * C + c) * HW + p];
    if (y_for_sigmoid_bwd && c == C - 1) {
      const float y = y_for_sigmoid_bwd[(b * C + c) * HW + p];
      v *= y * (1.f - y);
    }
    dst[i] = v;
  }
}

__global__ void qsample_kernel(const float* __restrict__ x0, const float* __restrict__ eps, const float* __restrict__ a,
                               const float* __restrict__ am1, const long long* __restrict__ t, float* __restrict__ xt, int B, int C,
// ... 169 lines not shown
  else if (C <= 512)
    hipLaunchKernelGGL(HIP_KERNEL_NAME(layernorm_kernel<true, 2>), dim3(nb), dim3(256), 0, st, x, gamma, dy, res, dx, partial, partial2, npix, C,
                     1e-5f, gs);
  else
    hipLaunchKernelGGL(HIP_KERNEL_NAME(layernorm_kernel<true, 4>), dim3(nb), dim3(256), 0, st, x, gamma, dy, res, dx, partial, partial2, npix, C,
                     1e-5f, gs);
  PIDM_CHECK_LAUNCH("layernorm_bwd");
  if (defer) {
    defer->push(partial, dgamma, nullptr, nullptr, (size_t)C, nb, 1, C, 1, 1, C);
    if (res_colsum) defer->push(partial2, res_colsum, nullptr, nullptr, (size_t)C, nb, 1, C, 1, 1, C);
    return 0;
  }
  char* ws2 = reinterpret_cast<char*>(ws) + (size_t)2 * nb * C * sizeof(float);
  if (launch_colsum(partial, (size_t)nb, C, C, dgamma, ws2, st)) return -1;
  return res_colsum ? launch_colsum(partial2, (size_t)nb, C, C, res_colsum, ws2, st) : 0;
}

int launch_act_fwd(const float* x, float* y, size_t n, int act, hipStream_t st) {
  hipLaunchKernelGGL(act_fwd_kernel, dim3(ew_blocks(n)), dim3(256), 0, st, x, y, n, act);
  PIDM_CHECK_LAUNCH("act_fwd_kernel");
  return 0;
}
int launch_act_bwd(const float* x, const float* dy, float* dx, size_t n, int act, hipStream_t st) {
  hipLaunchKernelGGL(act_bwd_kernel, dim3(ew_blocks(n)), dim3(256), 0, st, x, dy, dx, n, act);
  PIDM_CHECK_LAUNCH("act_bwd_kernel");
  return 0;
}
int launch_sinusoid(const int64_t* t, float* emb, int B, int dim, hipStream_t st) {
  if (dim < 4 || (dim & 1)) return fail("sinusoidal embedding: dim=%d must be even and >= 4", dim);
  hipLaunchKernelGGL(sinusoid_kernel, dim3(cdiv(B * dim / 2, 256)), dim3(256), 0, st, t, emb, B, dim);
  PIDM_CHECK_LAUNCH("sinusoid_kernel");
  return 0;
}
int launch_copy_add(float* dst, int ldd, const float* a, int lda, const float* b, int ldb, size_t rows, int cols, hipStream_t st) {
  if ((cols | ldd | lda | (b ? ldb : 0)) & 3) return fail("copy_add: widths must be multiples of 4");
  hipLaunchKernelGGL(copy_add_kernel, dim3(ew_blocks(rows * (cols / 4))), dim3(256), 0, st, dst, ldd, a, lda, b, ldb, rows, cols);
  PIDM_CHECK_LAUNCH("copy_add_kernel");
  return 0;
}
int launch_nchw_to_nhwc(const float* src, float* dst, int B, int C, int HW, const float* y_sig, hipStream_t st) {
  hipLaunchKernelGGL(nchw_to_nhwc_kernel, dim3(ew_blocks((size_t)B * C * HW)), dim3(256), 0, st, src, dst, B, C, HW, y_sig);
  PIDM_CHECK_LAUNCH("nchw_to_nhwc_kernel");
  return 0;
}

}

using namespace pidm;

extern "C" int pidm_qsample_nhwc(const float* x0, const float* eps, const float* a_t, const float* am1_t, float* xt_nhwc,
                                 int B, int C, int HW, void* stream) {
  hipLaunchKernelGGL(qsample_kernel, dim3(ew_blocks((size_t)B * C * HW)), dim3(256), 0, as_stream(stream), x0, eps, a_t,
                     am1_t, static_cast<const long long*>(nullptr), xt_nhwc, B, C, HW);
  PIDM_CHECK_LAUNCH("qsample_kernel");
  return 0;
}

extern "C" int pidm_qsample_nhwc_t(const float* x0, const float* eps, const int64_t* t, const float* a_table, const float* am1_table,
                                   float* xt_nhwc, int B, int C, int HW, void* stream) {
  if (!t || !a_table || !am1_table) return fail("qsample_nhwc_t: null time steps / tables");
  hipLaunchKernelGGL(qsample_kernel, dim3(ew_blocks((size_t)B * C * HW)), dim3(256), 0, as_stream(stream), x0, eps, a_table,
                     am1_table, reinterpret_cast<const long long*>(t), xt_nhwc, B, C, HW);
  PIDM_CHECK_LAUNCH("qsample_kernel");
  return 0;
}

// ... 8 lines not shown
```

physicsinformeddiffusionmodels_amd/csrc/pidm_launch.h:

```cpp
#pragma once
#include <vector>

#include "pidm_common.h"

namespace pidm {
struct ReduceQueue {
  std::vector<ReduceDesc> v;
  unsigned nblocks = 0;
  void push(const float* src, float* dst, const float* bsrc, float* bdst, size_t sstride, int nsplit, int M, int N, int T,
            int MP, int NP) {
    ReduceDesc d{};
    d.src = src; d.dst = dst; d.bsrc = bsrc; d.bdst = bdst; d.sstride = sstride;
    d.nsplit = nsplit; d.M = M; d.N = N; d.T = T; d.MP = MP; d.NP = NP;
    const size_t total = (size_t)M * N * T + (bdst ? M : 0);
    const size_t flat = (size_t)MP * T * NP;
    d.blk0 = nblocks;
    d.mode = (nsplit <= 8 && T <= 16 && (size_t)M * N * T >= 32768) ? 1 : 0;
    if (d.mode == 0 && nsplit > 8 && flat >= 4096 && (flat & 3) == 0 && (sstride & 3) == 0 && (reinterpret_cast<size_t>(src) & 15) == 0) {
      d.mode = 2;
      d.bsrc = nullptr;
      d.bdst = nullptr;
      d.nblk = (unsigned)((flat / 4 + 31) / 32);
      nblocks += d.nblk;
      v.push_back(d);
// ... 86 lines not shown
size_t wgrad_ws_bytes(const ConvGeom& g);
int launch_wgrad(const ConvGeom& g, const float* src0, const float* src1, const float* dy, int ld_dy, float* dw_ref,
                 float* dbias, void* workspace, hipStream_t st, ReduceQueue* defer = nullptr, WgradQueue* wq = nullptr);
bool launch_wgrad_rs(const WgradGeom& plan, const float* src0, const float* src1, const float* dy, int ld_dy, float* partial,
                     float* bias_partial, hipStream_t st, WgradGeom* used, WgradQueue* wq = nullptr);
bool wgrad_rs_queueable(const ConvGeom& g, const float* src0, const float* dy, int ld_dy);
bool wgrad_rs4_eligible(const ConvGeom& g, int ld_dy);
bool launch_wgrad_rs4(const WgradGeom& plan, const float* src0, const float* src1, const float* dy, int ld_dy, float* partial,
                      float* bias_partial, hipStream_t st, WgradGeom* used, WgradQueue* wq = nullptr);
bool launch_wgrad_rs7(const WgradGeom& plan, const float* src0, const float* dy, int ld_dy, float* partial, float* bias_partial,
                      hipStream_t st, WgradGeom* used);
size_t colsum_ws_bytes(size_t rows, int C);
int launch_colsum(const float* x, size_t rows, int C, int ld, float* out, void* workspace, hipStream_t st,
                  ReduceQueue* defer = nullptr);
size_t gn_ws_bytes(int B, int HW, int C, int G);
int launch_gn_stats(const float* x, int B, int HW, int C, int G, float* stats, void* ws, hipStream_t st);
bool gn_apply_ln_ok(int C);
int launch_gn_apply(const float* x, float* stats, const float* gamma, const float* beta, const float* ss, const float* ssb,
                    int ldss, const float* res, float* y, int B, int HW, int C, int G, void* ws, hipStream_t st, int part_chunks = 0,
                    const float* ln_gamma = nullptr, float* ln_out = nullptr);
int launch_gn_bwd(const float* x, const float* dy, const float* stats, const float* gamma, const float* beta, const float* ss,
                  const float* ssb, int ldss, float* dss, float* dx, float* dgamma, float* dbeta, int B, int HW, int C, int G,
                  void* ws, hipStream_t st, float* dgb_persist = nullptr, ReduceQueue* defer = nullptr, int part_chunks = 0);
int launch_layernorm_fwd(const float* x, const float* gamma, float* y, size_t npix, int C, hipStream_t st);
size_t layernorm_bwd_ws_bytes(int C);
int layernorm_bwd_gn_chunks(int B, int HW);
int launch_layernorm_bwd(const float* x, const float* gamma, const float* dy, const float* res, float* dx, float* dgamma,
                         size_t npix, int C, void* ws, hipStream_t st, ReduceQueue* defer = nullptr, float* res_colsum = nullptr,
                         const float* gn_x = nullptr, const float* gn_stats = nullptr, const float* gn_gamma = nullptr,
                         const float* gn_beta = nullptr, int gn_G = 0, int gn_B = 0, int gn_HW = 0, void* gn_part = nullptr);
int launch_act_fwd(const float* x, float* y, size_t n, int act, hipStream_t st);
int launch_act_bwd(const float* x, const float* dy, float* dx, size_t n, int act, hipStream_t st);
int launch_sinusoid(const int64_t* t, float* emb, int B, int dim, hipStream_t st);
int launch_copy_add(float* dst, int ldd, const float* a, int lda, const float* b, int ldb, size_t rows, int cols, hipStream_t st);
int launch_nchw_to_nhwc(const float* src, float* dst, int B, int C, int HW, const float* y_sig, hipStream_t st);
size_t la_scratch_floats(int B, int N, int heads);
int launch_la_forward(const float* qkv, float* kstat, float* ctx, float* attn, float* qstat, int B, int N, int heads,
                      float* scratch, hipStream_t st);
bool la_fused_ok(int N, int heads, int Cout, int ld_dy);
bool la_fused_pays(int B, int N);
size_t la_fused_scratch_floats(int B, int N, int heads, int Cout);
int launch_la_forward_fused(const float* qkv, float* kstat, float* ctx, float* qstat, const float* w_out, const float* bias,
                            const float* resid, float* y, int Cout, int B, int N, int heads, float* scratch, hipStream_t st);
int launch_la_backward_fused(const float* qkv, const float* kstat, const float* qstat, const float* ctx, const float* dy, int ld_dy,
                             const float* w_out, int Cout, float* dctx, float* rowdot, float* dqkv, float* dwpart, int B, int N,
                             int heads, float* scratch, hipStream_t st);
int launch_la_backward(const float* qkv, const float* kstat, const float* qstat, const float* ctx, const float* dA, float* dctx,
                       float* rowdot, float* dqkv, int B, int N, int heads, float* scratch, hipStream_t st);
bool lap_ok(int N, int heads, int C, int Cout);
size_t lap_scratch_floats(int B, int N, int heads, int C);
size_t lap_saved_floats(int B, int heads, int C);
size_t lap_dw_ranges(int N, int C);
size_t lap_bwd_tmp_floats(int B, int heads, int C);
int launch_lap_forward(const float* xn, const float* wqkv, const float* wout, const float* bias, const float* resid, float* y,
                       float* saved, float* qstat, int C, int B, int N, int heads, float* scratch, hipStream_t st);
int launch_lap_backward(const float* xn, const float* dy, const float* wqkv, const float* wout, const float* saved, const float* qstat,
                        float* dxn, float* dwqk_part, float* dwv_part, float* dwout_part, float* tmp, int C, int B, int N, int heads,
                        float* scratch, hipStream_t st);
int launch_mid_attn(const float* qkv, const float* dO, float* out, int B, int N, int heads, bool bwd, hipStream_t st);
}
```

physicsinformeddiffusionmodels_amd/csrc/unet_engine.hip:

```cpp
#include <map>
#include <string>
#include <vector>

#include <stdlib.h>

#include "pidm_launch.h"

extern char** environ;

namespace pidm {

struct Arena {
  char* base = nullptr;
  size_t off = 0, hwm = 0, cap = 0;
  bool dry = false;
  float* alloc(size_t nfloats) {
    off = align_up(off, 256);
    char* p = base + off;
    off += nfloats * sizeof(float);
    if (off > hwm) hwm = off;
    return reinterpret_cast<float*>(p);
  }
  size_t mark() const { return off; }
  void release(size_t m) { off = m; }
// ... 158 lines not shown
static int wgrad_group_limit() {
  const char* e = knob("PIDM_WGRAD_GROUP");
  int n = e ? atoi(e) : kWgradGroupDefault;
  return n < 0 ? 0 : n;
}
static bool backward_eager(int widest) {
  const char* e = knob("PIDM_GRAPH");
  if (e && !atoi(e)) return true;
  const char* b = knob("PIDM_GRAPH_BWD");
  if (b) return !atoi(b);
  const char* w = knob("PIDM_GRAPH_BWD_WIDE");
  return widest >= (w && atoi(w) > 0 ? atoi(w) : 512);
}
struct Run {
  pidm_unet* U;
  int B;
  bool train, dry;
  hipStream_t st;
  float* wpack;
  Arena tape, tmp;
  float* scratch = nullptr;
  size_t scratch_floats = 0;
  Arena defer;
  ReduceQueue rq;
  WgradQueue wq;
  WgradItem* wq_dev = nullptr;
  bool group_on = false;
  bool defer_on = false;
  bool overlap = false;
  bool keep_frames() const { return overlap || group_on || (dry && side_allowed); }
  bool side_allowed = false;
  bool side_pending = false;
  GraphCapture* cap = nullptr;
  float* part_alloc(size_t bytes) { return defer_on ? defer.alloc(bytes / 4 + 64) : scratch; }
  ReduceQueue* q() { return defer_on ? &rq : nullptr; }
  WgradQueue* wgq() {
    if (!(defer_on && group_on)) return nullptr;
    for (const auto& q : wq.f)
      if (q.v.size() >= kMaxWgradItems) return nullptr;
    return &wq;
  }
};

#define RUN(call)                 \
  do {                            \
    if (!r.dry) {                 \
      int rc__ = (call);          \
      if (rc__) return rc__;      \
    }                             \
  } while (0)

static int add_param(pidm_unet* U, const std::string& name, size_t numel) {
  U->index[name] = (int)U->names.size();
  U->names.push_back(name);
  U->numels.push_back(numel);
  return (int)U->names.size() - 1;
}

static pidm_conv_desc desc_of(const ConvLayer& L, int B) {
  pidm_conv_desc d;
  memset(&d, 0, sizeof(d));
  d.B = B; d.Hi = L.H; d.Wi = L.H; d.C0 = L.C0; d.C1 = L.C1; d.ld0 = L.C0; d.ld1 = L.C1; d.Cout = L.Cout;
  d.KH = d.KW = L.K; d.stride = L.stride; d.pad = L.pad; d.transposed = L.transposed; d.out_nchw = 0; d.ldo = L.Cout;
  return d;
}

// ... 457 lines not shown
  if (!a.mid && (la_fused_ok(N, heads, C, C) && la_fused_pays(B, N))) {
    a.attn = nullptr;
    a.kstat = act_alloc(r, (size_t)B * HD * 2);
    a.ctx = act_alloc(r, (size_t)B * heads * 1024);
    a.qstat = act_alloc(r, npix * heads * 2);
    RUN(launch_la_forward_fused(a.qkvb, a.kstat, a.ctx, a.qstat, U->P[a.out.w], a.out.b >= 0 ? U->P[a.out.b] : nullptr, x, out, C, B,
                                N, heads, r.scratch, r.st));
    r.tmp.release(mk);
    *out_p = out;
    return 0;
  }
  a.attn = act_alloc(r, npix * HD);
  if (a.mid) {
    RUN(launch_mid_attn(a.qkvb, nullptr, a.attn, B, N, heads, false, r.st));
  } else {
    a.kstat = act_alloc(r, (size_t)B * HD * 2);
    a.ctx = act_alloc(r, (size_t)B * heads * 1024);
    a.qstat = act_alloc(r, npix * heads * 2);
    RUN(launch_la_forward(a.qkvb, a.kstat, a.ctx, a.attn, a.qstat, B, N, heads, r.scratch, r.st));
  }
  if (conv_fwd(r, a.out, a.attn, nullptr, x, out)) return -1;
  r.tmp.release(mk);
  *out_p = out;
  return 0;
}

static int forward_impl(Run& r, const float* x_nhwc, const int64_t* t, float* out_nchw, const float* cond_nhwc) {
  pidm_unet* U = r.U;
  const int B = r.B, P = U->cfg.image_size, dim = U->cfg.dim, n = U->n_lv, td = U->tdim;
  U->tape_B = B;
  U->x_in = x_nhwc;
  U->out_nchw = out_nchw;
  U->emb = act_alloc(r, (size_t)B * dim);
  RUN(launch_sinusoid(t, U->emb, B, dim, r.st));
  U->h1 = act_alloc(r, (size_t)B * td);
  if (conv_fwd(r, U->lin1, U->emb, nullptr, nullptr, U->h1)) return -1;
  U->h1g = act_alloc(r, (size_t)B * td);
  RUN(launch_act_fwd(U->h1, U->h1g, (size_t)B * td, 1, r.st));
  U->temb = act_alloc(r, (size_t)B * td);
  if (conv_fwd(r, U->lin2, U->h1g, nullptr, nullptr, U->temb)) return -1;
  U->st = act_alloc(r, (size_t)B * td);
  RUN(launch_act_fwd(U->temb, U->st, (size_t)B * td, 0, r.st));
  U->ss = act_alloc(r, (size_t)B * U->ss_total);
  if (conv_fwd(r, U->lincat, U->st, nullptr, nullptr, U->ss)) return -1;

  U->h0 = act_alloc(r, (size_t)B * P * P * dim);
  if (conv_fwd(r, U->init_conv, x_nhwc, nullptr, nullptr, U->h0)) return -1;
  U->tape_cond = cond_nhwc != nullptr;
  if (cond_nhwc) {
    const size_t nh = (size_t)B * P * P * dim;
    U->cond_in = cond_nhwc;
    U->h0pre = U->h0;
    U->e1 = act_alloc(r, nh);
    if (conv_fwd(r, U->emb1, cond_nhwc, nullptr, nullptr, U->e1)) return -1;
    U->e1g = act_alloc(r, nh);
    RUN(launch_act_fwd(U->e1, U->e1g, nh, 1, r.st));
    U->e2 = act_alloc(r, nh);
    if (conv_fwd(r, U->emb2, U->e1g, nullptr, nullptr, U->e2)) return -1;
    float* hc = act_alloc(r, nh);
    if (conv_fwd(r, U->comb, U->h0pre, U->e2, nullptr, hc)) return -1;
    U->h0 = hc;
  }
  float* x = U->h0;
  int irb = 0, iat = 0;
  for (int i = 0; i < n; ++i) {
    if (resblock_fwd(r, U->rb[irb++], x, nullptr, &x)) return -1;
    if (resblock_fwd(r, U->rb[irb++], x, nullptr, &x, &U->attn[iat])) return -1;
    if (attn_fwd(r, U->attn[iat++], x, &x)) return -1;
    U->skip[i] = x;
    if (i < n - 1) {
      U->down_in[i] = x;
      const int Ho = out_h(U->down[i]);
      float* y = act_alloc(r, (size_t)B * Ho * Ho * U->down[i].Cout);
      if (conv_fwd(r, U->down[i], x, nullptr, nullptr, y)) return -1;
      x = y;
    }
  }
// ... 390 lines not shown
      if (hipMemcpyAsync(red_dev + first, U->red_table.data() + first, (n - first) * sizeof(ReduceDesc), hipMemcpyHostToDevice, r.st) != hipSuccess)
        return fail("backward: reduction table upload failed");
      ++g_red_table_uploads;
      U->red_table_dev = red_dev;
      U->red_table_owner = U->arena_sig;
    }
    const unsigned blk0 = r.rq.v[first].blk0;
    RUN(launch_reduce_multi(red_dev + first, (int)(n - first), r.rq.nblocks - blk0, r.st, blk0));
    *done = n;
  }
  hipEvent_t ev = (phase >= 0 && phase < 3) ? U->phase_ev[phase] : nullptr;
  if (r.cap) {
    if (ev || final_flush) return cap_end_segment(r, ev, !final_flush);
    return 0;
  }
  if (ev && hipEventRecord(ev, r.st) != hipSuccess) return fail("backward: phase event record failed");
  return 0;
}

static int backward_impl(Run& r, const float* grad_out_nchw, float* grad_x_nhwc) {
  pidm_unet* U = r.U;
  const int B = r.B, P = U->cfg.image_size, dim = U->cfg.dim, n = U->n_lv, td = U->tdim, od = U->cfg.out_dim;
  const size_t HW = (size_t)P * P;
  r.defer_on = true;
  r.rq.v.clear();
  r.rq.nblocks = 0;
  ReduceDesc* red_dev = reinterpret_cast<ReduceDesc*>(r.defer.alloc(kMaxReduceDesc * sizeof(ReduceDesc) / 4));
  size_t red_done = 0;
  r.wq.clear();
  r.wq_dev = reinterpret_cast<WgradItem*>(r.defer.alloc(kWgFams * kMaxWgradItems * sizeof(WgradItem) / 4));
  const int n_phases = U->n_phases;
  float* dss = r.tmp.alloc((size_t)B * U->ss_total);
  float* g_o = r.tmp.alloc((size_t)B * HW * od);
  RUN(launch_nchw_to_nhwc(grad_out_nchw, g_o, B, od, (int)HW, U->cfg.sigmoid_last_channel ? U->out_nchw : nullptr, r.st));
  {
    const ConvLayer& L = U->final_conv;
    if (U->have_grads || r.dry) {
      ConvGeom g;
      if (geom_fwd_layer(L, B, 0, &g)) return -1;
      float* part = r.part_alloc(wgrad_ws_bytes(g));
      RUN(launch_wgrad(g, U->xfinal, nullptr, g_o, od, U->G[L.w], U->G[L.b], part, r.st, r.q()));
    }
  }
  float* g_x = r.tmp.alloc((size_t)B * HW * dim);
  if (conv_dgrad(r, U->final_conv, g_o, nullptr, g_x)) return -1;
  int irb = (int)U->rb.size() - 1, iat = (int)U->attn.size() - 1;
  float* g_cat = r.tmp.alloc((size_t)B * HW * 2 * dim);
  if (resblock_bwd(r, U->rb[irb--], g_x, g_cat, dss)) return -1;
  const float* g_r = g_cat + dim;
  g_x = r.tmp.alloc((size_t)B * HW * dim);
  RUN(launch_copy_add(g_x, dim, g_cat, 2 * dim, nullptr, 0, (size_t)B * HW, dim, r.st));
  std::vector<const float*> g_skip(n, nullptr);
  std::vector<int> g_skip_ld(n, 0);
  int ld_gx = 0;
  for (int j = n - 1; j >= 0; --j) {
    const int lvl = n - 1 - j;
    const int din = U->dims[lvl], dout = U->dims[lvl + 1], H = P >> lvl;
    const size_t npix = (size_t)B * H * H;
    if (j < n - 1) {
      const ConvLayer& L = U->up[j];
      if (conv_wgrad(r, L, U->up_in[j], nullptr, g_x, ld_gx)) return -1;
      float* g = r.tmp.alloc(npix * din);
      if (conv_dgrad(r, L, g_x, nullptr, g, ld_gx)) return -1;
      g_x = g;
      ld_gx = 0;
    }
    float* g1 = r.tmp.alloc(npix * din);
// ... 309 lines not shown
}
static void touch_arena(pidm_unet* h, int B, bool train, const void* workspace, size_t workspace_bytes) {
  const uint64_t w[4] = {(uint64_t)B, (uint64_t)train, (uint64_t)reinterpret_cast<uintptr_t>(workspace), (uint64_t)workspace_bytes};
  const uint64_t sig = hash_words(w, 4);
  if (sig != h->arena_sig && sig != h->red_table_owner && h->red_table_dev) {
    size_t tape_b = 0, tmp_b = 0;
    const char* ws = reinterpret_cast<const char*>(workspace);
    const char* tab = reinterpret_cast<const char*>(h->red_table_dev);
    const size_t packed_b = packed_region_bytes(h) + io_region(h, B, nullptr).total;
    const bool planned = plan_sizes(h, B, train ? 1 : 0, &tape_b, &tmp_b) == 0;
    const bool inside = tab >= ws && tab < ws + workspace_bytes;
    if (knob("PIDM_DEBUG_ARENA")) fprintf(stderr, "[pidm] arena touch B=%d train=%d: extent %zu, table at %zu\n", B, (int)train, packed_b + tape_b + tmp_b, (size_t)(tab - ws));
    if (!planned || !inside || ws + packed_b + tape_b + tmp_b > tab) h->red_table_dev = h->wq_table_dev = nullptr;
  }
  h->arena_sig = sig;
}

static int forward_body(pidm_unet* h, const float* x_nhwc, const int64_t* t, float* out_nchw, int B, bool train, bool repack,
                        const float* cond, void* workspace, size_t workspace_bytes, hipStream_t st, GraphCapture* cap) {
  Run r;
  r.cap = cap;
  if (setup_run(r, h, B, train, workspace, workspace_bytes, st)) return -1;
  if (cap && cap_begin(r)) return -1;
  if (repack || h->packed_zeroed_for != r.wpack || !h->pack_table_valid) {
    if (pack_all(r)) return -1;
  }
  if (forward_impl(r, x_nhwc, t, out_nchw, cond)) return -1;
  if (r.tape.overflow() || r.tmp.overflow()) return fail("unet_forward: internal arena overflow");
  if (cap && cap->open && cap_end_segment(r, nullptr, false)) return -1;
  return 0;
}

static int backward_body(pidm_unet* h, const float* grad_out_nchw, float* grad_x_nhwc, int B, void* workspace, size_t workspace_bytes,
                         hipStream_t st, GraphCapture* cap) {
  Run r;
  r.cap = cap;
  if (setup_run(r, h, B, true, workspace, workspace_bytes, st, true)) return -1;
  r.side_allowed = backward_eager(widest_level(h));
  r.overlap = h->side_ok && !prof_enabled() && !cap && r.side_allowed;
  r.group_on = wgrad_group_on(B, h->cfg.image_size, r.side_allowed);
  if (!r.group_on && h->wq_table_dev) {
    h->wq_table_dev = nullptr;
    for (auto& t : h->wq_table) t.clear();
  }
  if (cap && cap_begin(r)) return -1;
  if (backward_impl(r, grad_out_nchw, grad_x_nhwc)) return -1;
  if (r.tmp.overflow() || r.defer.overflow()) return fail("unet_backward: internal arena overflow");
  if (cap && cap->open && cap_end_segment(r, nullptr, false)) return -1;
  return 0;
}

static void cap_abort(pidm_unet* h, GraphCapture* cap) {
  if (cap->open) {
    hipGraph_t g = nullptr;
    (void)hipStreamEndCapture(h->cap_stream, &g);
    if (g) (void)hipGraphDestroy(g);
    (void)hipGetLastError();
    cap->open = false;
  }
}

}

extern "C" int pidm_unet_forward(pidm_unet* h, const float* x_nhwc, const int64_t* t, float* out_nchw, int B,
                                 int save_for_backward, int repack_weights, void* workspace, size_t workspace_bytes,
                                 void* stream) {
  if (!h || !x_nhwc || !t || !out_nchw || !workspace) return fail("unet_forward: null argument");
  if (B <= 0) return fail("unet_forward: B must be positive");
  for (size_t i = 0; i < h->P.size(); ++i)
    if (!h->P[i]) return fail("unet_forward: parameters not bound (pidm_unet_bind)");
  const float* cond = h->cond_next;
  h->cond_next = nullptr;
  if (cond && !h->cond_enabled) return fail("unet_forward: conditioning input given but pidm_unet_enable_cond was not called");
  const bool train = save_for_backward != 0;
  const hipStream_t st = as_stream(stream);
  touch_arena(h, B, train, workspace, workspace_bytes);
  if (reinterpret_cast<uintptr_t>(workspace) & 255) return fail("unet: workspace must be 256-byte aligned");
  if (workspace_bytes < packed_region_bytes(h) + io_region(h, B, nullptr).total) return fail("unet: workspace too small");
  const IoRegion io = io_region(h, B, reinterpret_cast<char*>(workspace) + packed_region_bytes(h));
  if (x_nhwc != io.x && hipMemcpyAsync(io.x, x_nhwc, io.x_bytes, hipMemcpyDeviceToDevice, st) != hipSuccess) return fail("unet_forward: input copy failed");
  if (hipMemcpyAsync(io.t, t, io.t_bytes, hipMemcpyDeviceToDevice, st) != hipSuccess) return fail("unet_forward: time-step copy failed");
  if (cond && hipMemcpyAsync(io.cond, cond, io.cond_bytes, hipMemcpyDeviceToDevice, st) != hipSuccess) return fail("unet_forward: condition copy failed");
  const float* cond_s = cond ? io.cond : nullptr;
  const uint64_t kw[11] = {0xF0, (uint64_t)B, (uint64_t)train, (uint64_t)(repack_weights != 0), (uint64_t)(cond != nullptr),
                           (uint64_t)reinterpret_cast<uintptr_t>(workspace), (uint64_t)workspace_bytes,
                           h->param_sig, env_signature(), (uint64_t)h->cond_enabled, 0};
  const std::vector<uint64_t> key(kw, kw + 11);
  if (train) h->fwd_key_hash = hash_words(kw, 11);
  int rc = -1;
  bool done = false;
  const bool tables_ok = h->packed_zeroed_for == workspace && h->pack_table_valid;
  if (graphs_enabled() && tables_ok) {
    if (GraphEntry* e = graph_find(h, 0, key)) {
      rc = graph_replay(e, st);
      if (rc == 0 && train) tape_restore(h, e->tape);
      done = true;
    } else if (graph_second_sighting(h, 0, key) && ensure_cap_stream(h)) {
      e = graph_new_entry(h, 0, key);
      GraphCapture cap;
      cap.entry = e;
      cap.user_st = st;
      rc = forward_body(h, io.x, io.t, io.out, B, train, repack_weights != 0, cond_s, workspace, workspace_bytes, h->cap_stream, &cap);
      cap_abort(h, &cap);
      if (rc == 0 && !cap.failed) {
        ++g_graph_captures;
        if (train) tape_save(h, &e->tape);
        done = true;
      } else {
        graph_drop_entry(h, 0, e);
      }
    }
  }
  if (!done) rc = forward_body(h, io.x, io.t, io.out, B, train, repack_weights != 0, cond_s, workspace, workspace_bytes, st, nullptr);
  if (rc) return rc;
  if (out_nchw != io.out && hipMemcpyAsync(out_nchw, io.out, io.out_bytes, hipMemcpyDeviceToDevice, st) != hipSuccess) return fail("unet_forward: output copy failed");
  return 0;
}

extern "C" int pidm_unet_backward(pidm_unet* h, const float* grad_out_nchw, float* grad_x_nhwc, int B, void* workspace,
                                  size_t workspace_bytes, void* stream) {
  if (!h || !grad_out_nchw || !workspace) return fail("unet_backward: null argument");
  if (h->tape_B != B) return fail("unet_backward: no matching forward (tape holds B=%d)", h->tape_B);
  if (!h->have_grads) return fail("unet_backward: gradient buffers not bound");
  const hipStream_t st = as_stream(stream);
  if (!h->side_ok && !h->side) {
    const char* e = knob("PIDM_NO_OVERLAP");
    if (!(e && atoi(e))) {
      h->side_ok = hipStreamCreateWithFlags(&h->side, hipStreamNonBlocking) == hipSuccess &&
                   hipEventCreateWithFlags(&h->ev_fork, hipEventDisableTiming) == hipSuccess &&
                   hipEventCreateWithFlags(&h->ev_join, hipEventDisableTiming) == hipSuccess;
    } else {
      h->side = reinterpret_cast<hipStream_t>(1);
    }
  }
  touch_arena(h, B, true, workspace, workspace_bytes);
  if (!h->tape_cond && h->cond_grads_dirty) {
    for (size_t i = (size_t)h->cond_first_param; i < h->names.size(); ++i)
      if (hipMemsetAsync(h->G[i], 0, h->numels[i] * sizeof(float), st) != hipSuccess) return fail("backward: memset failed");
    h->cond_grads_dirty = false;
  }
  const IoRegion io = io_region(h, B, reinterpret_cast<char*>(workspace) + packed_region_bytes(h));
  if (grad_out_nchw != io.gout && hipMemcpyAsync(io.gout, grad_out_nchw, io.out_bytes, hipMemcpyDeviceToDevice, st) != hipSuccess)
    return fail("unet_backward: gradient copy failed");
  float* gx_s = grad_x_nhwc ? io.gx : nullptr;
  const uint64_t kw[14] = {0xB0, (uint64_t)B, (uint64_t)(grad_x_nhwc != nullptr),
                           (uint64_t)reinterpret_cast<uintptr_t>(workspace), (uint64_t)workspace_bytes, h->bind_sig, env_signature(),
                           h->fwd_key_hash, (uint64_t)h->n_phases, (uint64_t)reinterpret_cast<uintptr_t>(h->phase_ev[0]),
                           (uint64_t)reinterpret_cast<uintptr_t>(h->phase_ev[1]), (uint64_t)reinterpret_cast<uintptr_t>(h->phase_ev[2]),
                           (uint64_t)h->tape_cond, (uint64_t)h->side_ok};
  const std::vector<uint64_t> key(kw, kw + 14);
  int rc = -1;
  bool done = false;
  if (graphs_enabled() && !backward_eager(widest_level(h))) {
    GraphEntry* e = graph_find(h, 1, key);
    if (e && e->red_dev == h->red_table_dev && h->red_table_dev) {
      rc = graph_replay(e, st);
      done = true;
    } else if (!e && h->red_table_dev && graph_second_sighting(h, 1, key) && ensure_cap_stream(h)) {
      e = graph_new_entry(h, 1, key);
      GraphCapture cap;
      cap.entry = e;
      cap.user_st = st;
      rc = backward_body(h, io.gout, gx_s, B, workspace, workspace_bytes, h->cap_stream, &cap);
      cap_abort(h, &cap);
      if (rc == 0 && !cap.failed) {
        ++g_graph_captures;
        e->red_dev = h->red_table_dev;
        done = true;
      } else {
        graph_drop_entry(h, 1, e);
      }
    }
  }
  if (!done) rc = backward_body(h, io.gout, gx_s, B, workspace, workspace_bytes, st, nullptr);
  if (rc == 0 && h->tape_cond) h->cond_grads_dirty = true;
  if (rc == 0 && grad_x_nhwc && grad_x_nhwc != io.gx &&
      hipMemcpyAsync(grad_x_nhwc, io.gx, io.x_bytes, hipMemcpyDeviceToDevice, st) != hipSuccess)
    return fail("unet_backward: input-gradient copy failed");
  return rc;
}

extern "C" int pidm_debug_launch_counts(long long* out4) {
  if (!out4) return fail("debug_launch_counts: null argument");
  out4[0] = pidm::g_kernel_enqueues;
  out4[1] = pidm::g_graph_launches;
  out4[2] = pidm::g_graph_kernels;
  out4[3] = pidm::g_graph_captures;
  return 0;
}

extern "C" int pidm_unet_set_grad_events(pidm_unet* h, int n_phases, void* const* events) {
  if (!h) return fail("unet_set_grad_events: null handle");
  if (n_phases < 1 || n_phases > 3) return fail("unet_set_grad_events: n_phases must be 1..3 (got %d)", n_phases);
  h->n_phases = n_phases;
  for (int i = 0; i < 3; ++i) h->phase_ev[i] = (events && i < n_phases) ? reinterpret_cast<hipEvent_t>(events[i]) : nullptr;
  return 0;
}

extern "C" int pidm_unet_grad_phase_range(const pidm_unet* h, int n_phases, int phase, int* first_param, int* end_param) {
  if (!h || !first_param || !end_param) return fail("unet_grad_phase_range: null argument");
  if (n_phases < 1 || n_phases > 3 || phase < 0 || phase >= n_phases) return fail("unet_grad_phase_range: bad phase %d of %d", phase, n_phases);
  const int n = (int)h->names.size();
  if (n_phases == 1) { *first_param = 0; *end_param = n; return 0; }
  if (phase == 0) { *first_param = h->idx_ups_first; *end_param = h->cond_first_param; return 0; }
  if (n_phases == 3 && phase == 1) { *first_param = h->idx_downs_first; *end_param = h->idx_ups_first; return 0; }
  *first_param = 0;
  *end_param = (n_phases == 3) ? h->idx_downs_first : h->idx_ups_first;
  return 0;
}

extern "C" long long pidm_debug_reduce_table_uploads(void) { return pidm::g_red_table_uploads; }

extern "C" int pidm_unet_num_cond_params(const pidm_unet* h) { return h ? (int)h->names.size() - h->cond_first_param : 0; }

extern "C" int pidm_unet_enable_cond(pidm_unet* h, int on) {
  if (!h) return fail("unet_enable_cond: null handle");
  const bool v = on != 0;
  if (v != h->cond_enabled) {
    h->cond_enabled = v;
    h->ws_cache[0].clear();
// ... 12 lines not shown
```

physicsinformeddiffusionmodels_amd/denoising_utils.py:

```python
from __future__ import annotations

import contextlib
import os
from pathlib import Path

import numpy as np
import torch
import torch.nn as nn
import torch.nn.functional as F
import yaml

from ._lib import get_lib, ptr, stream_ptr
from .residuals_darcy import ResidualsDarcy
from .unet_model import (default, exists, generalized_b_xy_c_to_image, generalized_image_to_b_xy_c,
                         noop)

device = torch.device('cuda' if torch.cuda.is_available() else 'cpu')


def fix_seeds(seed=42):
    torch.manual_seed(seed)
    torch.cuda.manual_seed(seed)
    np.random.seed(seed)

# ... 262 lines not shown
    def _v(self):
        v = self._src.values()
        for i in self._idx:
            v = v[i]
        return v

    def __float__(self): return float(self._v())
    def __format__(self, spec): return format(self._v(), spec)
    def __repr__(self): return repr(self._v())
    __str__ = __repr__
    def __bool__(self): return bool(self._v())
    def __hash__(self): return hash(self._v())
    def __eq__(self, o): return self._v() == float(o)
    def __lt__(self, o): return self._v() < float(o)
    def __le__(self, o): return self._v() <= float(o)
    def __gt__(self, o): return self._v() > float(o)
    def __ge__(self, o): return self._v() >= float(o)
    def __neg__(self): return -self._v()
    def __abs__(self): return abs(self._v())
    def __add__(self, o): return self._v() + float(o)
    __radd__ = __add__
    def __sub__(self, o): return self._v() - float(o)
    def __rsub__(self, o): return float(o) - self._v()
    def __mul__(self, o): return self._v() * float(o)
    __rmul__ = __mul__
    def __truediv__(self, o): return self._v() / float(o)
    def __rtruediv__(self, o): return float(o) / self._v()
    def item(self): return self._v()


class _DarcyPidmLossFn(torch.autograd.Function):

    @staticmethod
    def forward(ctx, x0_pred, x0, f_s, t, p2w_table, var_table, c_data, c_residual, inv_h0, inv_h1, lib):
        pred = x0_pred.contiguous()
        B, C, P, _ = pred.shape
        dev = pred.device
        res = torch.empty(B, P * P, 3, dtype=torch.float32, device=dev)
        grad = torch.empty_like(pred)
        out = torch.empty(4, dtype=torch.float32, device=dev)
        ws = torch.empty(lib.pidm_darcy_loss_ws(B, P), dtype=torch.uint8, device=dev)
        lib.check(lib.pidm_darcy_loss_fwd_bwd_t(ptr(x0), ptr(pred), ptr(f_s), ptr(t), ptr(p2w_table), ptr(var_table),
                                                float(c_data), float(c_residual), inv_h0, inv_h1, ptr(res), ptr(grad), ptr(out),
                                                ptr(ws), B, P, stream_ptr(dev)), 'pidm_darcy_loss_fwd_bwd_t')
        ctx.save_for_backward(grad)
        ctx.mark_non_differentiable(out, res)
        return out[0].clone(), out, res

    @staticmethod
    def backward(ctx, g_loss, _g_out, _g_res):
        (grad,) = ctx.saved_tensors
        return grad * g_loss, None, None, None, None, None, None, None, None, None, None


class _EarlyStepFn(torch.autograd.Function):

    @staticmethod
    def forward(ctx, anchor, eng, diffusion, x_bxyc, t, loss_call):
        eng.tape_generation += 1
        ctx.generation = eng.tape_generation
        pred = eng.forward(x_bxyc, t, training=True, early=True)
        grad, out = loss_call(pred)
        ctx.fetch = diffusion._start_scalar_fetch(out) if out.is_cuda else None
        loss_t = out[0].clone()
        eng.backward(grad, False, x_bxyc.shape[-1])
        eng.early_generation = ctx.generation
        eng.tape_busy = False
        ctx.eng = eng
        diffusion._early_fetch = ctx.fetch
        ctx.mark_non_differentiable(out)
        return loss_t, out

    @staticmethod
    def backward(ctx, g_loss, _g_out):
        eng = ctx.eng
        if eng.early_generation != ctx.generation:
            from ._lib import PidmError
            raise PidmError("the staged gradients of this step were overwritten by a later training-mode forward of the same model "
                            "(only the latest step can be differentiated)")
        first = eng.params[0]
        aliased = first.grad is not None and first.grad.data_ptr() == eng.grad_views[0].data_ptr()
        g = g_loss.to(eng.early_grad.dtype)
        if aliased:
            eng.flat_grad.add_(eng.early_grad * g)
        else:
            torch.mul(eng.early_grad, g, out=eng.flat_grad)
        eng.early_generation = -1
        eng.backward_calls += 1 if not aliased else 2
        n_plain = len(eng.params) - eng.n_cond
        for i, (p, gv) in enumerate(zip(eng.params, eng.grad_views)):
            if not p.requires_grad or i >= n_plain:
                continue
            if p.grad is None:
                p.grad = gv
            elif p.grad.data_ptr() != gv.data_ptr():
                p.grad.add_(eng.early_views[i] * g)
        return None, None, None, None, None, None


class DenoisingDiffusion(nn.Module):

    def __init__(self, n_steps, device, residual_grad_guidance=False, lib=None):
        super().__init__()
        self.n_steps = n_steps
        self.device = device
        self.diff_dict = self.create_diff_dict()
        self.residual_grad_guidance = residual_grad_guidance
        self._lib = lib
        self.data_parallel_world = 1
        self.data_parallel_group = None
        self.deferred_scalars = False
        self._scalar_ring, self._scalar_slot = [], 0
        self._early_fetch = None

    def _host_scalars(self, scalars, idx_list):
        if not (self.deferred_scalars and scalars.is_cuda):
            s = scalars.tolist()
            out = []
            for idx in idx_list:
                v = s
                for i in idx:
                    v = v[i]
                out.append(v)
            return out
        fetch = self._start_scalar_fetch(scalars)
        return [DeferredFloat(fetch, tuple(idx)) for idx in idx_list]

    def _start_scalar_fetch(self, scalars):
        if not self._scalar_ring:
            self._scalar_ring = [[torch.empty(16, dtype=torch.float32).pin_memory(), None] for _ in range(64)]
# ... 163 lines not shown
                                                  return_optimizer=return_optimizer, return_inequality=return_inequality,
                                                  ddim_func=self.ddim_sample_x0)
        residual, output = out_dict['residual'], out_dict['model_out']
        if output.dim() == 3:
            output = b_xy_c_to_image(output)
        loss = ((x_0 - output) ** 2).reshape(batch_size, -1).mean(dim=1)
        loss = (loss * extract(self.diff_dict['p2_loss_weight'], t, loss)).mean()
        data_loss = c_data * loss
        data_loss_track = data_loss.item()
        loss = data_loss
        var = extract(self.diff_dict['posterior_variance_clipped'], t, residual)
        residual_loss_track = residual.abs().mean().item()
        loss = loss + (c_residual * 0.5 * residual ** 2 / var).mean()
        ineq_loss_track = 0.
        if return_inequality:
            ineq = out_dict['inequality']
            ineq_loss_track = ineq.mean().item()
            loss = loss + (c_ineq * 0.5 * ineq ** 2 / var).mean()
        opt_loss_track = 0.
        if return_optimizer:
            opt_loss_track = out_dict['optimizer'].mean().item()
            loss = loss + (lambda_opt * out_dict['optimizer']).mean()
        return loss, data_loss_track, residual_loss_track, ineq_loss_track, opt_loss_track

    def _darcy_step(self, x_0, e, t, residual_func, c_data, c_residual):
        lib = residual_func.lib
        B, C, P, _ = x_0.shape
        dev = x_0.device
        dd = self._kernel_tables(dev)
        x_0 = x_0.contiguous()
        t = t.to(device=dev, dtype=torch.int64).contiguous()
        if residual_func._f_s_flat.device != dev:
            residual_func._f_s_flat = residual_func._f_s_flat.to(dev)
        xt = torch.empty(B, P * P, C, dtype=torch.float32, device=dev)
        lib.check(lib.pidm_qsample_nhwc_t(ptr(x_0), ptr(e.contiguous()), ptr(t), ptr(dd['alphas_bar_sqrt']),
                                          ptr(dd['one_minus_alphas_bar_sqrt']), ptr(xt), B, C, P * P, stream_ptr(dev)),
                  'pidm_qsample_nhwc_t')
        eng = self._early_backward_engine(residual_func, xt.shape[-1], P) if not residual_func.use_ddim_x0 else None
        if eng is not None:
            f_s = residual_func._f_s_flat

            def loss_call(pred):
                res = torch.empty(B, P * P, 3, dtype=torch.float32, device=dev)
                grad = torch.empty_like(pred)
                out = torch.empty(4, dtype=torch.float32, device=dev)
                ws = torch.empty(lib.pidm_darcy_loss_ws(B, P), dtype=torch.uint8, device=dev)
                lib.check(lib.pidm_darcy_loss_fwd_bwd_t(ptr(x_0), ptr(pred), ptr(f_s), ptr(t), ptr(dd['p2_loss_weight']),
                                                        ptr(dd['posterior_variance_clipped']), float(c_data), float(c_residual),
                                                        residual_func.inv_h0, residual_func.inv_h1, ptr(res), ptr(grad), ptr(out), ptr(ws),
                                                        B, P, stream_ptr(dev)), 'pidm_darcy_loss_fwd_bwd_t')
                return grad, out
            loss, scalars = _EarlyStepFn.apply(eng.params[0], eng, self, xt, t, loss_call)
            fetch, self._early_fetch = self._early_fetch, None
            if fetch is not None:
                v = fetch.values()
                return loss, v[1], v[2], 0., 0.
            d, r = self._host_scalars(scalars, [(1,), (2,)])
            return loss, d, r, 0., 0.
        if residual_func._f_s_flat.device != dev:
            residual_func._f_s_flat = residual_func._f_s_flat.to(dev)
        args = (residual_func._f_s_flat, t, dd['p2_loss_weight'], dd['posterior_variance_clipped'])
        geo = (residual_func.inv_h0, residual_func.inv_h1, lib)
        if residual_func.use_ddim_x0:
            x0_pred, model_out = self.ddim_sample_x0(xt, t, residual_func.model, xt.shape, residual_func.ddim_steps, 0.)
            l_data, s_data, _ = _DarcyPidmLossFn.apply(model_out, x_0, *args, c_data, 0., *geo)
            l_res, s_res, _res = _DarcyPidmLossFn.apply(x0_pred, x_0, *args, 0., c_residual, *geo)
            d, r = self._host_scalars(torch.stack((s_data, s_res)), [(0, 1), (1, 2)])
            return l_data + l_res, d, r, 0., 0.
        x0_pred = residual_func.model(xt, t)
        loss, scalars, _res = _DarcyPidmLossFn.apply(x0_pred, x_0, *args, c_data, c_residual, *geo)
        d, r = self._host_scalars(scalars, [(1,), (2,)])
        return loss, d, r, 0., 0.

    def _kernel_tables(self, dev):
        cache = self.__dict__.setdefault('_pidm_tables', {})
        got = cache.get(dev)
        if got is None or got[0] is not self.diff_dict:
            tabs = {}
            for k in ('alphas_bar_sqrt', 'one_minus_alphas_bar_sqrt', 'p2_loss_weight', 'posterior_variance_clipped'):
                v = self.diff_dict[k]
                if v.device != dev or v.dtype != torch.float32 or not v.is_contiguous():
                    v = v.to(device=dev, dtype=torch.float32).contiguous()
                if v.dim() != 1 or v.numel() != self.n_steps:
                    raise ValueError(f'schedule table {k!r} has shape {tuple(v.shape)}, expected ({self.n_steps},)')
                tabs[k] = v
            cache[dev] = got = (self.diff_dict, tabs)
        return got[1]

    def _early_backward_engine(self, residual_func, channels, image_size):
        from ._engine import get_engine
        from .unet_model import Unet3D
        model = residual_func.model
        first = next(model.parameters())
        if (self.deferred_scalars or not torch.is_grad_enabled() or os.environ.get('PIDM_EARLY_BACKWARD') == '0'
                or type(model) is not Unet3D or not model.training or model.self_condition
                or not (first.is_cuda or self._lib is not None) or model._forward_hooks or model._forward_pre_hooks
                or channels != model.channels or getattr(model, '_pidm_tape_slot', None)):
            return None
        eng = get_engine(model, image_size, model._pidm_lib)
        if getattr(eng, '_exchange_owner', None) is not None or eng.tape_busy or not all(p.requires_grad for p in eng.params):
            return None
        return eng

    def _mech_step(self, x_0, conditioning, bcs, e, t, residual_func, c_data, c_residual, c_ineq, lambda_opt):
        from .residuals_mechanics_K import _MechLossFn, resize_image
        lib = residual_func.lib
        dd = self.diff_dict
        a = extract(dd['alphas_bar_sqrt'], t, x_0)
        am1 = extract(dd['one_minus_alphas_bar_sqrt'], t, x_0)
        x = torch.cat((x_0 * a + e * am1, conditioning), dim=1)
        P = residual_func.pixels_per_dim
        net_in = torch.cat((resize_image(x, P, lib), resize_image(bcs, P, lib)), dim=1)
        vf = conditioning[:, 0, 0, 0].contiguous()
        p2w = dd['p2_loss_weight'][t].contiguous()
        inv_var = (1.0 / dd['posterior_variance_clipped'][t]).contiguous()
        if residual_func.stiffs.kloc_dev.device != x_0.device:
            residual_func.stiffs.to(x_0.device)
        ivs = None
        if c_ineq > 0. and self.data_parallel_world > 1:
            import torch.distributed as dist
# ... 162 lines not shown
```

Measured before the change: 8140.

## Write UNet IO directly into workspace buffers and fuse linear-attention key stats

Measured after the change: 8197 (median of 6 runs). No clear change (+0.7%).

```diff
diff --git a/include/pidm.h b/include/pidm.h
--- a/include/pidm.h
+++ b/include/pidm.h
@@ -32,6 +32,10 @@
                               const float* p2w_table, const float* var_table, float c_data, float c_residual,
                               float inv_h0, float inv_h1, float* residual, float* grad_x0_pred, float* out_scalars,
                               void* workspace, int B, int P, void* stream);
+int pidm_darcy_loss_fwd_bwd_t_cl(const float* x0, const float* x0_pred, const float* f_s, const int64_t* t,
+                                 const float* p2w_table, const float* var_table, float c_data, float c_residual,
+                                 float inv_h0, float inv_h1, float* residual, float* grad_x0_pred_nhwc, float* out_scalars,
+                                 void* workspace, int B, int P, void* stream);
 
 int pidm_darcy_jacobian_max(const float* x0, float inv_h0, float inv_h1, float* max_dr_dp, int B, int P, void* stream);
 
@@ -136,6 +140,10 @@
 int pidm_unet_set_condition(pidm_unet* h, const float* cond_nhwc);
 int pidm_unet_backward(pidm_unet* h, const float* grad_out_nchw, float* grad_x_nhwc, int B, void* workspace,
                        size_t workspace_bytes, void* stream);
+int pidm_unet_backward_cl(pidm_unet* h, const float* grad_out_nhwc, float* grad_x_nhwc, int B, void* workspace,
+                          size_t workspace_bytes, void* stream);
+int pidm_unet_io_addresses(const pidm_unet* h, int B, void* workspace, size_t workspace_bytes, void** x, void** t, void** out,
+                           void** gout);
 
 int pidm_unet_set_grad_events(pidm_unet* h, int n_phases, void* const* events);
 int pidm_unet_grad_phase_range(const pidm_unet* h, int n_phases, int phase, int* first_param, int* end_param);
@@ -189,6 +197,7 @@
 int pidm_debug_lap_trace(unsigned long long* out256);
 long long pidm_debug_reduce_table_uploads(void);
 int pidm_debug_launch_counts(long long* out4);
+long long pidm_unet_debug_time_path(const pidm_unet* h, float* ss_out, void* stream);
 int pidm_comm_available(void);
 int pidm_comm_unique_id(void* out128);
 int pidm_comm_init(int rank, int world, const void* unique_id128, void** comm);
diff --git a/physicsinformeddiffusionmodels_amd/_engine.py b/physicsinformeddiffusionmodels_amd/_engine.py
--- a/physicsinformeddiffusionmodels_amd/_engine.py
+++ b/physicsinformeddiffusionmodels_amd/_engine.py
@@ -54,6 +54,7 @@
         self.tape_generation = 0
         self.tape_busy = False
         self._packed_for = None
+        self._io_cache = None
 
     def __del__(self):
         try:
@@ -103,8 +104,33 @@
             self.workspace = torch.empty(nbytes + 256, dtype=torch.uint8, device=device)
         return self.workspace
 
+    def io_views(self, B: int, training: bool, device):
+        ws = self._ensure_workspace(B, training, device)
+        base = ws.data_ptr()
+        key = (base, ws.numel(), B)
+        if self._io_cache is not None and self._io_cache[0] == key:
+            return self._io_cache[1]
+        al = (-base) % 256
+        a = [vp() for _ in range(4)]
+        self.lib.check(self.lib.pidm_unet_io_addresses(self.handle, B, vp(base + al), ws.numel() - al, *[C.byref(v) for v in a]),
+                       "pidm_unet_io_addresses")
+        views = None
+        if all(v.value for v in a):
+            P = self.image_size
+            c_in, c_out = self.x_channels, self.lib_out_dim
+
+            def view(addr, nbytes, dtype, shape):
+                off = addr - base
+                return ws[off:off + nbytes].view(dtype).view(shape)
+            views = (view(a[0].value, 4 * B * P * P * c_in, torch.float32, (B, P * P, c_in)),
+                     view(a[1].value, 8 * B, torch.int64, (B,)),
+                     view(a[2].value, 4 * B * P * P * c_out, torch.float32, (B, c_out, P, P)),
+                     view(a[3].value, 4 * B * P * P * c_out, torch.float32, (B, P * P, c_out)))
+        self._io_cache = (key, views)
+        return views
+
     def forward(self, x_nhwc: torch.Tensor, t: torch.Tensor, training: bool, repack: bool = True,
-                cond: torch.Tensor | None = None, early: bool = False, frozen=None) -> torch.Tensor:
+                cond: torch.Tensor | None = None, early: bool = False, frozen=None, out_static: bool = False) -> torch.Tensor:
         B = x_nhwc.shape[0]
         dev = x_nhwc.device
         self._ensure_bound(training, early=early)
@@ -115,7 +141,8 @@
             self.lib.check(self.lib.pidm_unet_set_condition(self.handle, ptr(cond)), "pidm_unet_set_condition")
         ws = self._ensure_workspace(B, training, dev)
         P = self.image_size
-        out = torch.empty(B, self.lib_out_dim, P, P, dtype=torch.float32, device=dev)
+        io = self.io_views(B, training, dev) if out_static else None
+        out = io[2] if io is not None else torch.empty(B, self.lib_out_dim, P, P, dtype=torch.float32, device=dev)
         base = ws.data_ptr()
         al = (-base) % 256
         if frozen is not None and not training and repack:
@@ -128,15 +155,15 @@
                                                   vp(base + al), ws.numel() - al, stream_ptr(dev)), "pidm_unet_forward")
         return out
 
-    def backward(self, grad_out: torch.Tensor, want_grad_x: bool, channels: int):
+    def backward(self, grad_out: torch.Tensor, want_grad_x: bool, channels: int, channels_last: bool = False):
         B = grad_out.shape[0]
         dev = grad_out.device
         ws = self.workspace
         gx = torch.empty(B, self.image_size * self.image_size, channels, dtype=torch.float32, device=dev) if want_grad_x else None
         base = ws.data_ptr()
         al = (-base) % 256
-        self.lib.check(self.lib.pidm_unet_backward(self.handle, ptr(grad_out), ptr(gx), B, vp(base + al), ws.numel() - al,
-                                                   stream_ptr(dev)), "pidm_unet_backward")
+        fn = self.lib.pidm_unet_backward_cl if channels_last else self.lib.pidm_unet_backward
+        self.lib.check(fn(self.handle, ptr(grad_out), ptr(gx), B, vp(base + al), ws.numel() - al, stream_ptr(dev)), "pidm_unet_backward")
         return gx
 
 
@@ -163,7 +190,7 @@
 class _UnetFunction(torch.autograd.Function):
 
     @staticmethod
-    def forward(ctx, engine: UnetEngine, x_nhwc, t, anchor, training: bool, cond=None, primary=None, frozen=None):
+    def forward(ctx, engine: UnetEngine, x_nhwc, t, anchor, training: bool, cond=None, primary=None, frozen=None, out_static=False):
         ctx.engine = engine
         ctx.primary = primary if primary is not None else engine
         ctx.used_cond = cond is not None
@@ -175,7 +202,7 @@
             engine.tape_busy = True
         ctx.generation = engine.tape_generation
         ctx.lease = _TapeLease(engine, engine.tape_generation) if training else None
-        out = engine.forward(x_nhwc, t, training=training, cond=cond, frozen=frozen)
+        out = engine.forward(x_nhwc, t, training=training, cond=cond, frozen=frozen, out_static=out_static)
         if cond is not None:
             ctx.save_for_backward(out, x_nhwc, cond)
         else:
@@ -197,7 +224,12 @@
             primary._ensure_bound(True)
         aliased = first.grad is not None and first.grad.data_ptr() == primary.grad_views[0].data_ptr()
         prev = primary.flat_grad.clone() if (aliased and eng is primary) else None
-        gx = eng.backward(grad_out.contiguous(), ctx.x_requires_grad, ctx.channels)
+        io = eng._io_cache[1] if eng._io_cache is not None else None
+        if (io is not None and grad_out.data_ptr() == io[3].data_ptr() and grad_out.dim() == 4
+                and grad_out.permute(0, 2, 3, 1).is_contiguous() and not eng.sigmoid_last_channel):
+            gx = eng.backward(grad_out, ctx.x_requires_grad, ctx.channels, channels_last=True)
+        else:
+            gx = eng.backward(grad_out.contiguous(), ctx.x_requires_grad, ctx.channels)
         if prev is not None:
             eng.flat_grad.add_(prev)
         if eng is not primary:
@@ -219,7 +251,7 @@
                 p.grad = g
             elif p.grad.data_ptr() != g.data_ptr():
                 p.grad.add_(eng.grad_views[i] if eng is not primary else g)
-        return None, gx, None, None, None, None, None, None
+        return None, gx, None, None, None, None, None, None, None
 
 
 def get_engine(model, image_size: int, lib: PidmLib | None = None, slot: int = 0) -> UnetEngine:
@@ -229,6 +261,8 @@
     if eng is None:
         eng = UnetEngine(model, image_size, lib)
         eng.lib_out_dim = model.out_dim
+        eng.x_channels = model.channels * (2 if model.self_condition else 1)
+        eng.sigmoid_last_channel = bool(model.sigmoid_last_channel)
         cache[key] = eng
     return eng
 
@@ -299,7 +333,8 @@
         if cond.shape != (B, P * P, model.channels):
             raise ValueError(f'cond must be [B, P*P, {model.channels}], got {tuple(cond.shape)}')
         cond = cond.detach().contiguous().float()
-    out = _UnetFunction.apply(eng, x_nhwc, t, anchor, training, cond, primary, getattr(model, "_pidm_frozen", None))
+    out = _UnetFunction.apply(eng, x_nhwc, t, anchor, training, cond, primary, getattr(model, "_pidm_frozen", None),
+                              bool(getattr(model, "_pidm_out_static", False)))
     if video:
         out = out.unsqueeze(2)
     return out
diff --git a/physicsinformeddiffusionmodels_amd/_lib.py b/physicsinformeddiffusionmodels_amd/_lib.py
--- a/physicsinformeddiffusionmodels_amd/_lib.py
+++ b/physicsinformeddiffusionmodels_amd/_lib.py
@@ -60,6 +60,7 @@
         self._sig("pidm_darcy_loss_ws", [i, i], sz)
         self._sig("pidm_darcy_loss_fwd_bwd", [vp, vp, vp, vp, vp, f, f, f, f, vp, vp, vp, vp, i, i, vp])
         self._sig("pidm_darcy_loss_fwd_bwd_t", [vp, vp, vp, vp, vp, vp, f, f, f, f, vp, vp, vp, vp, i, i, vp])
+        self._sig("pidm_darcy_loss_fwd_bwd_t_cl", [vp, vp, vp, vp, vp, vp, f, f, f, f, vp, vp, vp, vp, i, i, vp])
         self._sig("pidm_darcy_jacobian_max", [vp, f, f, vp, i, i, vp])
         ll, ops = C.c_longlong, C.POINTER(StencilOp)
         self._sig("pidm_stencil_apply", [vp, ll, ops, C.POINTER(vp), i, ll, i, i, i, i, vp])
@@ -104,6 +105,9 @@
         self._sig("pidm_unet_bind", [vp, C.POINTER(vp), C.POINTER(vp)])
         self._sig("pidm_unet_forward", [vp, vp, vp, vp, i, i, i, vp, sz, vp])
         self._sig("pidm_unet_backward", [vp, vp, vp, i, vp, sz, vp])
+        self._sig("pidm_unet_backward_cl", [vp, vp, vp, i, vp, sz, vp])
+        self._sig("pidm_unet_io_addresses", [vp, i, vp, sz, C.POINTER(vp), C.POINTER(vp), C.POINTER(vp), C.POINTER(vp)])
+        self._sig("pidm_unet_debug_time_path", [vp, vp, vp], C.c_longlong)
         self._sig("pidm_unet_set_grad_events", [vp, i, C.POINTER(vp)])
         self._sig("pidm_unet_grad_phase_range", [vp, i, i, C.POINTER(C.c_int), C.POINTER(C.c_int)])
         self._sig("pidm_conv_packed_weight_floats", [C.POINTER(ConvDesc)], sz)
diff --git a/physicsinformeddiffusionmodels_amd/csrc/k_attn.hip b/physicsinformeddiffusionmodels_amd/csrc/k_attn.hip
--- a/physicsinformeddiffusionmodels_amd/csrc/k_attn.hip
+++ b/physicsinformeddiffusionmodels_amd/csrc/k_attn.hip
@@ -73,8 +73,10 @@
 __global__ void __launch_bounds__(256) la_nreduce_kernel(const float* __restrict__ qkv, const float* __restrict__ stat,
                                                          const float* __restrict__ dA, const float* __restrict__ ctx,
                                                          float* __restrict__ Dpart, int N, int heads, float scale,
-                                                         float* __restrict__ Dfinal, float* __restrict__ rowdot, float alpha) {
+                                                         float* __restrict__ Dfinal, float* __restrict__ rowdot, float alpha,
+                                                         float* __restrict__ kstat_out) {
   __shared__ float red[4][1024];
+  __shared__ float ksm[4][32], kss[4][32], kfin[2][32];
   const int bh = blockIdx.x, b = bh / heads, h = bh % heads;
   const int ns = blockIdx.y, NS = gridDim.y;
   const int HD = heads * DH;
@@ -84,7 +86,50 @@
   for (int r = 0; r < 16; ++r) acc[r] = 0.f;
   const float* q0 = qkv + (size_t)b * N * 3 * HD;
   float cm = 0.f, cis = 0.f;
-  if (MODE == 0) {
+  if (MODE == 0 && kstat_out) {
+    if (tid < 128) {
+      const int cl = tid & 31, rl = tid >> 5;
+      const float* base = q0 + HD + h * DH + cl;
+      float m = -3.0e38f, s = 0.f;
+      int n = rl;
+      for (; n + 28 < N; n += 32) {
+        float v[8];
+#pragma unroll
+        for (int u = 0; u < 8; ++u) v[u] = base[(size_t)(n + 4 * u) * 3 * HD];
+        float gm = v[0];
+#pragma unroll
+        for (int u = 1; u < 8; ++u) gm = fmaxf(gm, v[u]);
+        const float mn = fmaxf(m, gm);
+        float gs = 0.f;
+#pragma unroll
+        for (int u = 0; u < 8; ++u) gs += fexp(v[u] - mn);
+        s = s * fexp(m - mn) + gs;
+        m = mn;
+      }
+      for (; n < N; n += 4) {
+        const float v = base[(size_t)n * 3 * HD];
+        const float mn = fmaxf(m, v);
+        s = s * fexp(m - mn) + fexp(v - mn);
+        m = mn;
+      }
+      ksm[rl][cl] = m;
+      kss[rl][cl] = s;
+    }
+    __syncthreads();
+    if (tid < 32) {
+      const float M = fmaxf(fmaxf(ksm[0][tid], ksm[1][tid]), fmaxf(ksm[2][tid], ksm[3][tid]));
+      float S = 0.f;
+      for (int r = 0; r < 4; ++r) S += kss[r][tid] * fexp(ksm[r][tid] - M);
+      const float inv = 1.f / S;
+      kstat_out[((size_t)b * HD + h * DH + tid) * 2] = M;
+      kstat_out[((size_t)b * HD + h * DH + tid) * 2 + 1] = inv;
+      kfin[0][tid] = M;
+      kfin[1][tid] = inv;
+    }
+    __syncthreads();
+    cm = kfin[0][l31];
+    cis = kfin[1][l31];
+  } else if (MODE == 0) {
     cm = stat[((size_t)b * HD + h * DH + l31) * 2];
     cis = stat[((size_t)b * HD + h * DH + l31) * 2 + 1];
   }
@@ -1043,27 +1088,39 @@
   return a + b + (size_t)heads * DH * 128 + 64;
 }
 
-int launch_la_forward(const float* qkv, float* kstat, float* ctx, float* attn, float* qstat, int B, int N, int heads,
-                      float* scratch, hipStream_t st) {
+static int la_context(const float* qkv, float* kstat, float* ctx, int B, int N, int heads, float* kpart, float* dpart, hipStream_t st) {
   const int HD = heads * DH;
   const float scale = 0.17677669529663687f;
   const int nseg = la_kseg(N), NS = la_nsplit(N);
-  float* kpart = scratch;
-  float* dpart = scratch + (size_t)B * nseg * HD * 2;
-  hipLaunchKernelGGL(la_kstats_kernel, dim3(cdiv(HD, 64), B, nseg), dim3(256), 0, st, qkv, N, HD, nseg, kpart, nseg == 1 ? kstat : nullptr);
-  PIDM_CHECK_LAUNCH("la_kstats_kernel");
-  if (nseg > 1) {
-    hipLaunchKernelGGL(la_kstats_final_kernel, dim3(cdiv(B * HD, 256)), dim3(256), 0, st, kpart, B, HD, nseg, kstat);
-    PIDM_CHECK_LAUNCH("la_kstats_final_kernel");
+  const char* fk = knob("PIDM_FUSE_LA_STATS");
+  const bool fuse = nseg == 1 && NS == 1 && !(fk && !atoi(fk));
+  if (!fuse) {
+    hipLaunchKernelGGL(la_kstats_kernel, dim3(cdiv(HD, 64), B, nseg), dim3(256), 0, st, qkv, N, HD, nseg, kpart, nseg == 1 ? kstat : nullptr);
+    PIDM_CHECK_LAUNCH("la_kstats_kernel");
+    if (nseg > 1) {
+      hipLaunchKernelGGL(la_kstats_final_kernel, dim3(cdiv(B * HD, 256)), dim3(256), 0, st, kpart, B, HD, nseg, kstat);
+      PIDM_CHECK_LAUNCH("la_kstats_final_kernel");
+    }
   }
   hipLaunchKernelGGL(HIP_KERNEL_NAME(la_nreduce_kernel<0>), dim3(B * heads, NS), dim3(256), 0, st, qkv, kstat, nullptr, nullptr,
-                     dpart, N, heads, scale, NS == 1 ? ctx : nullptr, nullptr, 1.f / (float)N);
+                     dpart, N, heads, scale, NS == 1 ? ctx : nullptr, nullptr, 1.f / (float)N, fuse ? kstat : nullptr);
   PIDM_CHECK_LAUNCH("la_context");
   if (NS > 1) {
     hipLaunchKernelGGL(HIP_KERNEL_NAME(la_nreduce_final_kernel<0>), dim3(B * heads), dim3(256), 0, st, dpart, nullptr, ctx, nullptr, NS,
                        1.f / (float)N);
     PIDM_CHECK_LAUNCH("la_context_final");
   }
+  return 0;
+}
+
+int launch_la_forward(const float* qkv, float* kstat, float* ctx, float* attn, float* qstat, int B, int N, int heads,
+                      float* scratch, hipStream_t st) {
+  const int HD = heads * DH;
+  const float scale = 0.17677669529663687f;
+  const int nseg = la_kseg(N);
+  float* kpart = scratch;
+  float* dpart = scratch + (size_t)B * nseg * HD * 2;
+  if (la_context(qkv, kstat, ctx, B, N, heads, kpart, dpart, st)) return -1;
   const size_t npix = (size_t)B * N;
   if (N % 32 == 0)
     hipLaunchKernelGGL(HIP_KERNEL_NAME(la_out_kernel<true>), dim3((unsigned)((npix + 127) / 128), (npix + 127) / 128 < 1024 ? heads : 1), dim3(256), 0, st, qkv, ctx, attn,
@@ -1081,7 +1138,7 @@
   const int NS = la_nsplit(N);
   float* dpart = scratch;
   hipLaunchKernelGGL(HIP_KERNEL_NAME(la_nreduce_kernel<1>), dim3(B * heads, NS), dim3(256), 0, st, qkv, qstat, dA, ctx, dpart, N, heads,
-                     scale, NS == 1 ? dctx : nullptr, rowdot, 1.f);
+                     scale, NS == 1 ? dctx : nullptr, rowdot, 1.f, nullptr);
   PIDM_CHECK_LAUNCH("la_dctx");
   if (NS > 1) {
     hipLaunchKernelGGL(HIP_KERNEL_NAME(la_nreduce_final_kernel<1>), dim3(B * heads), dim3(256), 0, st, dpart, ctx, dctx, rowdot, NS, 1.f);
@@ -1115,20 +1172,7 @@
   const int nseg = la_kseg(N), NS = la_nsplit(N);
   float* kpart = scratch;
   float* dpart = scratch + (size_t)B * nseg * HD * 2;
-  hipLaunchKernelGGL(la_kstats_kernel, dim3(cdiv(HD, 64), B, nseg), dim3(256), 0, st, qkv, N, HD, nseg, kpart, nseg == 1 ? kstat : nullptr);
-  PIDM_CHECK_LAUNCH("la_kstats_kernel");
-  if (nseg > 1) {
-    hipLaunchKernelGGL(la_kstats_final_kernel, dim3(cdiv(B * HD, 256)), dim3(256), 0, st, kpart, B, HD, nseg, kstat);
-    PIDM_CHECK_LAUNCH("la_kstats_final_kernel");
-  }
-  hipLaunchKernelGGL(HIP_KERNEL_NAME(la_nreduce_kernel<0>), dim3(B * heads, NS), dim3(256), 0, st, qkv, kstat, nullptr, nullptr,
-                     dpart, N, heads, scale, NS == 1 ? ctx : nullptr, nullptr, 1.f / (float)N);
-  PIDM_CHECK_LAUNCH("la_context");
-  if (NS > 1) {
-    hipLaunchKernelGGL(HIP_KERNEL_NAME(la_nreduce_final_kernel<0>), dim3(B * heads), dim3(256), 0, st, dpart, nullptr, ctx, nullptr, NS,
-                       1.f / (float)N);
-    PIDM_CHECK_LAUNCH("la_context_final");
-  }
+  if (la_context(qkv, kstat, ctx, B, N, heads, kpart, dpart, st)) return -1;
   float* wt = dpart + (size_t)B * heads * NS * 1024;
   hipLaunchKernelGGL(la_wt_kernel, dim3(cdiv(Cout * HD, 256)), dim3(256), 0, st, w_out, wt, Cout, HD);
   PIDM_CHECK_LAUNCH("la_wt_kernel");
diff --git a/physicsinformeddiffusionmodels_amd/csrc/k_darcy.hip b/physicsinformeddiffusionmodels_amd/csrc/k_darcy.hip
--- a/physicsinformeddiffusionmodels_amd/csrc/k_darcy.hip
+++ b/physicsinformeddiffusionmodels_amd/csrc/k_darcy.hip
@@ -131,6 +131,18 @@
   return t;
 }
 
+__device__ __forceinline__ void darcy_store_grad4(float* __restrict__ grad_pred, size_t b, int N, int n, f32x4 gp, f32x4 gK, int gcl) {
+  if (gcl) {
+    const f32x4 lo = {gp[0], gK[0], gp[1], gK[1]}, hi = {gp[2], gK[2], gp[3], gK[3]};
+    float* o = grad_pred + (b * N + n) * 2;
+    *reinterpret_cast<f32x4*>(o) = lo;
+    *reinterpret_cast<f32x4*>(o + 4) = hi;
+  } else {
+    *reinterpret_cast<f32x4*>(grad_pred + b * 2 * N + n) = gp;
+    *reinterpret_cast<f32x4*>(grad_pred + b * 2 * N + N + n) = gK;
+  }
+}
+
 template <int MODE>
 __global__ void __launch_bounds__(256) darcy_kernel(const float* __restrict__ x0,
                                                     const float* __restrict__ pred,
@@ -141,7 +153,7 @@
                                                     float c_data, float c_res, float bc1_sign, FdAxis ax0, FdAxis ax1,
                                                     float* __restrict__ residual, float* __restrict__ grad_pred,
                                                     double* __restrict__ partial,
-                                                    int B, int P, int R, int nb, int lds_rows) {
+                                                    int B, int P, int R, int nb, int lds_rows, int gcl) {
   HIP_DYNAMIC_SHARED(float, smem)
   const int N = P * P;
   const int b = blockIdx.x / nb, band = blockIdx.x - b * nb;
@@ -272,8 +284,13 @@
         gp += dscale * (sp[n] - x0[(size_t)b * 2 * N + n]);
         gK += dscale * (sK[n] - x0[(size_t)b * 2 * N + N + n]);
       }
-      grad_pred[(size_t)b * 2 * N + n] = gp;
-      grad_pred[(size_t)b * 2 * N + N + n] = gK;
+      if (gcl) {
+        grad_pred[((size_t)b * N + n) * 2] = gp;
+        grad_pred[((size_t)b * N + n) * 2 + 1] = gK;
+      } else {
+        grad_pred[(size_t)b * 2 * N + n] = gp;
+        grad_pred[(size_t)b * 2 * N + N + n] = gK;
+      }
       j += dj;
       i += di;
       if (j >= P) {
@@ -360,7 +377,7 @@
                                                          const float* __restrict__ p2w, const float* __restrict__ inv_var,
                                                          const long long* __restrict__ tsteps, float c_data, float c_res, float bc1_sign,
                                                          FdAxis ax0, FdAxis ax1, float* __restrict__ residual, float* __restrict__ grad_pred,
-                                                         double* __restrict__ partial, int B, int P, int R, int nb, int lds_rows) {
+                                                         double* __restrict__ partial, int B, int P, int R, int nb, int lds_rows, int gcl) {
   HIP_DYNAMIC_SHARED(float, smem)
   const int N = P * P, QP = P >> 2;
   const int b = blockIdx.x / nb, band = blockIdx.x - b * nb;
@@ -534,8 +551,7 @@
         gK[m] += dscale * (vK[m] - t1v[m]);
       }
     }
-    *reinterpret_cast<f32x4*>(grad_pred + (size_t)b * 2 * N + n) = gp;
-    *reinterpret_cast<f32x4*>(grad_pred + (size_t)b * 2 * N + N + n) = gK;
+    darcy_store_grad4(grad_pred, (size_t)b, N, n, gp, gK, gcl);
   }
 
   if (MODE == DARCY_LOSS) {
@@ -567,7 +583,7 @@
                                                         const float* __restrict__ p2w, const float* __restrict__ inv_var,
                                                         const long long* __restrict__ tsteps, float c_data, float c_res, float bc1_sign,
                                                         FdAxis ax0, FdAxis ax1, float* __restrict__ residual, float* __restrict__ grad_pred,
-                                                        double* __restrict__ partial, int B) {
+                                                        double* __restrict__ partial, int B, int gcl) {
   constexpr int P = 64, N = P * P, RS = NT / 16, NIT = P / RS;
   HIP_DYNAMIC_SHARED(float, smem)
   float* sp = smem;
@@ -739,8 +755,7 @@
         gK[m] += dscale * t1[it][m];
       }
     }
-    *reinterpret_cast<f32x4*>(grad_pred + (size_t)b * 2 * N + n) = gp;
-    *reinterpret_cast<f32x4*>(grad_pred + (size_t)b * 2 * N + N + n) = gK;
+    darcy_store_grad4(grad_pred, (size_t)b, N, n, gp, gK, gcl);
   }
 
   if (MODE == DARCY_LOSS) {
@@ -775,7 +790,7 @@
                                                               const float* __restrict__ inv_var, const long long* __restrict__ tsteps,
                                                               float c_data, float c_res, float bc1_sign, FdAxis ax0, FdAxis ax1,
                                                               float* __restrict__ residual, float* __restrict__ grad_pred,
-                                                              double* __restrict__ partial, int B) {
+                                                              double* __restrict__ partial, int B, int gcl) {
   constexpr int P = 64, N = P * P, NT = 512, RS = NT / 16, NIT = P / RS;
   HIP_DYNAMIC_SHARED(float, smem)
   float* spb = smem;
@@ -968,8 +983,7 @@
         gp[m] += dscale * t0[it][m];
         gK[m] += dscale * t1[it][m];
       }
-      *reinterpret_cast<f32x4*>(grad_pred + (size_t)b * 2 * N + n) = gp;
-      *reinterpret_cast<f32x4*>(grad_pred + (size_t)b * 2 * N + N + n) = gK;
+      darcy_store_grad4(grad_pred, (size_t)b, N, n, gp, gK, gcl);
     }
     double v[3] = {acc_data, acc_r2, acc_rabs};
     for (int qq = 0; qq < 3; ++qq) {
@@ -1079,7 +1093,7 @@
 template <int MODE>
 static int launch_darcy(const float* x0, const float* pred, const float* f_s, const float* grad_res, const float* p2w,
                         const float* inv_var, const long long* tsteps, float c_data, float c_res, float inv_h0, float inv_h1,
-                        float* residual, float* grad_pred, double* partial, int B, int P, hipStream_t st) {
+                        float* residual, float* grad_pred, double* partial, int B, int P, hipStream_t st, int gcl = 0) {
   if (B <= 0 || P < 5) return fail("darcy: need B>0 and P>=5 (got B=%d P=%d)", B, P);
   const DarcyBands bd = darcy_bands(B, P, MODE == DARCY_RES_ONLY);
   const int rows = darcy_lds_rows(P, bd.R);
@@ -1111,7 +1125,7 @@
     if (wgs < 1) wgs = 1;
     if (wgs > B) wgs = B;
     hipLaunchKernelGGL(darcy_stream_kernel, dim3((unsigned)wgs), dim3(512), lds_s, st, x0, pred, f_s, p2w, inv_var, tsteps, c_data, c_res,
-                       (inv_h1 < 0.f) ? 1.f : -1.f, make_axis(inv_h0), make_axis(inv_h1), residual, grad_pred, partial, B);
+                       (inv_h1 < 0.f) ? 1.f : -1.f, make_axis(inv_h0), make_axis(inv_h1), residual, grad_pred, partial, B, gcl);
     PIDM_CHECK_LAUNCH("darcy_stream_kernel");
     return 0;
   }
@@ -1126,7 +1140,7 @@
       attr_f = true;
     }
     hipLaunchKernelGGL(HIP_KERNEL_NAME(darcy_full_kernel<MODE, 512>), dim3((unsigned)B), dim3(512), lds_f, st, x0, pred, f_s, grad_res, p2w, inv_var,
-                       tsteps, c_data, c_res, (inv_h1 < 0.f) ? 1.f : -1.f, make_axis(inv_h0), make_axis(inv_h1), residual, grad_pred, partial, B);
+                       tsteps, c_data, c_res, (inv_h1 < 0.f) ? 1.f : -1.f, make_axis(inv_h0), make_axis(inv_h1), residual, grad_pred, partial, B, gcl);
     PIDM_CHECK_LAUNCH("darcy_full_kernel");
     return 0;
   }
@@ -1143,23 +1157,23 @@
     if (nt < 64) nt = 64;
     hipLaunchKernelGGL(HIP_KERNEL_NAME(darcy_quad_kernel<MODE>), dim3((unsigned)B * bd.nb), dim3(nt), lds, st, x0, pred, f_s, grad_res, p2w,
                        inv_var, tsteps, c_data, c_res, (inv_h1 < 0.f) ? 1.f : -1.f, make_axis(inv_h0), make_axis(inv_h1), residual,
-                       grad_pred, partial, B, P, bd.R, bd.nb, rows);
+                       grad_pred, partial, B, P, bd.R, bd.nb, rows, gcl);
     PIDM_CHECK_LAUNCH("darcy_quad_kernel");
     return 0;
   }
   hipLaunchKernelGGL(HIP_KERNEL_NAME(darcy_kernel<MODE>), dim3((unsigned)B * bd.nb), dim3(256), lds, st, x0, pred, f_s, grad_res, p2w,
                      inv_var, tsteps, c_data, c_res, (inv_h1 < 0.f) ? 1.f : -1.f, make_axis(inv_h0), make_axis(inv_h1), residual,
-                     grad_pred, partial, B, P, bd.R, bd.nb, rows);
+                     grad_pred, partial, B, P, bd.R, bd.nb, rows, gcl);
   PIDM_CHECK_LAUNCH("darcy_kernel");
   return 0;
 }
 
 static int darcy_loss_impl(const float* x0, const float* x0_pred, const float* f_s, const float* p2w, const float* inv_var,
                            const long long* tsteps, float c_data, float c_residual, float inv_h0, float inv_h1, float* residual,
-                           float* grad_x0_pred, float* out_scalars, void* workspace, int B, int P, hipStream_t st) {
+                           float* grad_x0_pred, float* out_scalars, void* workspace, int B, int P, hipStream_t st, int gcl = 0) {
   double* partial = reinterpret_cast<double*>(workspace);
   int rc = launch_darcy<DARCY_LOSS>(x0, x0_pred, f_s, nullptr, p2w, inv_var, tsteps, c_data, c_residual, inv_h0, inv_h1, residual,
-                                    grad_x0_pred, partial, B, P, st);
+                                    grad_x0_pred, partial, B, P, st, gcl);
   if (rc) return rc;
   hipLaunchKernelGGL(darcy_loss_finalize, dim3(1), dim3(256), 0, st, partial, p2w, inv_var, tsteps, c_data, c_residual, B, P * P,
                      darcy_bands(B, P).nb, out_scalars);
@@ -1203,6 +1217,15 @@
   if (!t || !p2w_table || !var_table) return fail("darcy_loss_fwd_bwd_t: null time steps / tables");
   return darcy_loss_impl(x0, x0_pred, f_s, p2w_table, var_table, reinterpret_cast<const long long*>(t), c_data, c_residual, inv_h0,
                          inv_h1, residual, grad_x0_pred, out_scalars, workspace, B, P, as_stream(stream));
+}
+
+extern "C" int pidm_darcy_loss_fwd_bwd_t_cl(const float* x0, const float* x0_pred, const float* f_s, const int64_t* t,
+                                            const float* p2w_table, const float* var_table, float c_data, float c_residual,
+                                            float inv_h0, float inv_h1, float* residual, float* grad_x0_pred_nhwc, float* out_scalars,
+                                            void* workspace, int B, int P, void* stream) {
+  if (!t || !p2w_table || !var_table) return fail("darcy_loss_fwd_bwd_t_cl: null time steps / tables");
+  return darcy_loss_impl(x0, x0_pred, f_s, p2w_table, var_table, reinterpret_cast<const long long*>(t), c_data, c_residual, inv_h0,
+                         inv_h1, residual, grad_x0_pred_nhwc, out_scalars, workspace, B, P, as_stream(stream), 1);
 }
 
 extern "C" int pidm_darcy_jacobian_max(const float* x0, float inv_h0, float inv_h1, float* max_dr_dp, int B, int P, void* stream) {
diff --git a/physicsinformeddiffusionmodels_amd/csrc/k_norm.hip b/physicsinformeddiffusionmodels_amd/csrc/k_norm.hip
--- a/physicsinformeddiffusionmodels_amd/csrc/k_norm.hip
+++ b/physicsinformeddiffusionmodels_amd/csrc/k_norm.hip
@@ -748,6 +748,125 @@
   emb[(size_t)b * dim + half + k] = cosf(arg);
 }
 
+static constexpr int kTpCols = 128;
+template <bool VEC, class RowPtr, class Epi>
+__device__ __forceinline__ void tp_matmul(RowPtr rowp, int J, int K, const float* act, int rs, Epi epi) {
+  const int tid = threadIdx.x, lane = tid & 63, half = lane >> 5, l31 = lane & 31;
+  const int wave = __builtin_amdgcn_readfirstlane(tid >> 6);
+  const int rsp = rs + 1, kh = K / 2;
+  __syncthreads();
+  for (int j0 = wave * 32; j0 < J; j0 += 128) {
+    const int j = j0 + l31;
+    const float* wr = (j < J) ? rowp(j) + half * kh : nullptr;
+    const float* ar = act + (size_t)half * kh * rsp + l31;
+    const bool arow = l31 < rs;
+    f32x16 acc0, acc1;
+#pragma unroll
+    for (int r = 0; r < 16; ++r) acc0[r] = acc1[r] = 0.f;
+    auto wload = [&](int s) {
+      f32x4 w = {0.f, 0.f, 0.f, 0.f};
+      if (wr) {
+        if (VEC) {
+          w = *reinterpret_cast<const f32x4*>(wr + s);
+        } else {
+          w[0] = wr[s]; w[1] = wr[s + 1]; w[2] = wr[s + 2]; w[3] = wr[s + 3];
+        }
+      }
+      return w;
+    };
+    for (int s = 0; s < kh; s += 64) {
+      f32x4 w[16];
+#pragma unroll
+      for (int u = 0; u < 16; ++u) {
+        w[u] = f32x4{0.f, 0.f, 0.f, 0.f};
+        if (s + 4 * u < kh) w[u] = wload(s + 4 * u);
+      }
+#pragma unroll
+      for (int u = 0; u < 16; ++u) {
+        if (s + 4 * u < kh) {
+          const float* ap = ar + (size_t)(s + 4 * u) * rsp;
+          const float a0 = arow ? ap[0] : 0.f, a1 = arow ? ap[rsp] : 0.f, a2 = arow ? ap[2 * rsp] : 0.f, a3 = arow ? ap[3 * rsp] : 0.f;
+          acc0 = __builtin_amdgcn_mfma_f32_32x32x2f32(a0, w[u][0], acc0, 0, 0, 0);
+          acc1 = __builtin_amdgcn_mfma_f32_32x32x2f32(a1, w[u][1], acc1, 0, 0, 0);
+          acc0 = __builtin_amdgcn_mfma_f32_32x32x2f32(a2, w[u][2], acc0, 0, 0, 0);
+          acc1 = __builtin_amdgcn_mfma_f32_32x32x2f32(a3, w[u][3], acc1, 0, 0, 0);
+        }
+      }
+    }
+    if (j < J) {
+#pragma unroll
+      for (int r = 0; r < 16; ++r) {
+        const int row = (r & 3) + 8 * (r >> 2) + 4 * half;
+        if (row < rs) epi(j, row, acc0[r] + acc1[r]);
+      }
+    }
+  }
+}
+
+template <bool VEC>
+__global__ void __launch_bounds__(256) time_path_fwd_kernel(const int64_t* __restrict__ t, const float* __restrict__ w1,
+                                                            const float* __restrict__ b1, const float* __restrict__ w2,
+                                                            const float* __restrict__ b2, TimePathTab tab, float* __restrict__ emb,
+                                                            float* __restrict__ h1, float* __restrict__ h1g, float* __restrict__ temb,
+                                                            float* __restrict__ st, float* __restrict__ ss, int B, int dim, int td,
+                                                            int ss_total, int rs) {
+  HIP_DYNAMIC_SHARED(float, smem)
+  __shared__ const float* rowp_s[kTpCols];
+  const int rsp = rs + 1;
+  float* actA = smem;
+  float* actB = actA + (size_t)td * rsp;
+  const int tid = threadIdx.x;
+  const int b0 = blockIdx.y * rs, nrows = (B - b0 < rs) ? B - b0 : rs;
+  const int c0 = blockIdx.x * kTpCols, ncols = (ss_total - c0 < kTpCols) ? ss_total - c0 : kTpCols;
+  const bool keep = blockIdx.x == 0;
+  if (tid < kTpCols) {
+    const float* p = nullptr;
+    if (tid < ncols) {
+      int i = 0;
+      while (i + 1 < tab.n && tab.off[i + 1] <= c0 + tid) ++i;
+      p = tab.w[i] + (size_t)(c0 + tid - tab.off[i]) * td;
+    }
+    rowp_s[tid] = p;
+  }
+  const int half = dim / 2;
+  for (int i = tid; i < dim * rsp; i += 256) actA[i] = 0.f;
+  __syncthreads();
+  for (int i = tid; i < nrows * half; i += 256) {
+    const int r = i / half, k = i % half;
+    const float e = (float)(9.210340371976184 / (double)(half - 1));
+    const float w = expf((float)k * -e);
+    const float arg = (float)t[b0 + r] * w;
+    const float sv = sinf(arg), cv = cosf(arg);
+    actA[k * rsp + r] = sv;
+    actA[(half + k) * rsp + r] = cv;
+    if (keep) {
+      emb[(size_t)(b0 + r) * dim + k] = sv;
+      emb[(size_t)(b0 + r) * dim + half + k] = cv;
+    }
+  }
+  tp_matmul<VEC>([&](int j) { return w1 + (size_t)j * dim; }, td, dim, actA, rs, [&](int j, int r, float acc) {
+    const float v = acc + b1[j];
+    const float g = 0.5f * v * (1.f + erff(v * 0.70710678118654752440f));
+    actB[j * rsp + r] = g;
+    if (keep && r < nrows) {
+      h1[(size_t)(b0 + r) * td + j] = v;
+      h1g[(size_t)(b0 + r) * td + j] = g;
+    }
+  });
+  tp_matmul<VEC>([&](int j) { return w2 + (size_t)j * td; }, td, td, actB, rs, [&](int j, int r, float acc) {
+    const float v = acc + b2[j];
+    const float sl = v * sigmoidf_(v);
+    actA[j * rsp + r] = sl;
+    if (keep && r < nrows) {
+      temb[(size_t)(b0 + r) * td + j] = v;
+      st[(size_t)(b0 + r) * td + j] = sl;
+    }
+  });
+  tp_matmul<VEC>([&](int j) { return rowp_s[j]; }, ncols, td, actA, rs, [&](int j, int r, float acc) {
+    if (r < nrows) ss[(size_t)(b0 + r) * ss_total + c0 + j] = acc;
+  });
+}
+
 __global__ void copy_add_kernel(float* __restrict__ dst, int ldd, const float* __restrict__ a, int lda,
                                 const float* __restrict__ b, int ldb, size_t rows, int cols) {
   const int c4 = cols / 4;
@@ -983,6 +1102,27 @@
   PIDM_CHECK_LAUNCH("sinusoid_kernel");
   return 0;
 }
+bool time_path_fused_ok(int B, int dim, int td, int nlin) {
+  const char* e = knob("PIDM_FUSE_TIME");
+  return !(e && !atoi(e)) && td <= 512 && dim >= 8 && dim % 8 == 0 && td % 8 == 0 && (long)B * td <= 8192 && nlin <= kTimePathMaxLin;
+}
+int launch_time_path_fwd(const int64_t* t, const float* w1, const float* b1, const float* w2, const float* b2, const TimePathTab& tab,
+                         float* emb, float* h1, float* h1g, float* temb, float* st_out, float* ss, int B, int dim, int td, int ss_total,
+                         hipStream_t st) {
+  const int rs = td <= 224 ? 32 : (td <= 448 ? 16 : 8);
+  const size_t lds = (size_t)2 * td * (rs + 1) * sizeof(float);
+  size_t al = reinterpret_cast<size_t>(w1) | reinterpret_cast<size_t>(w2);
+  for (int i = 0; i < tab.n; ++i) al |= reinterpret_cast<size_t>(tab.w[i]);
+  const dim3 grid(cdiv(ss_total, kTpCols), cdiv(B, rs));
+  if ((al & 15) == 0)
+    hipLaunchKernelGGL(HIP_KERNEL_NAME(time_path_fwd_kernel<true>), grid, dim3(256), lds, st, t, w1, b1, w2, b2, tab, emb, h1, h1g, temb,
+                       st_out, ss, B, dim, td, ss_total, rs);
+  else
+    hipLaunchKernelGGL(HIP_KERNEL_NAME(time_path_fwd_kernel<false>), grid, dim3(256), lds, st, t, w1, b1, w2, b2, tab, emb, h1, h1g, temb,
+                       st_out, ss, B, dim, td, ss_total, rs);
+  PIDM_CHECK_LAUNCH("time_path_fwd_kernel");
+  return 0;
+}
 int launch_copy_add(float* dst, int ldd, const float* a, int lda, const float* b, int ldb, size_t rows, int cols, hipStream_t st) {
   if ((cols | ldd | lda | (b ? ldb : 0)) & 3) return fail("copy_add: widths must be multiples of 4");
   hipLaunchKernelGGL(copy_add_kernel, dim3(ew_blocks(rows * (cols / 4))), dim3(256), 0, st, dst, ldd, a, lda, b, ldb, rows, cols);
diff --git a/physicsinformeddiffusionmodels_amd/csrc/pidm_launch.h b/physicsinformeddiffusionmodels_amd/csrc/pidm_launch.h
--- a/physicsinformeddiffusionmodels_amd/csrc/pidm_launch.h
+++ b/physicsinformeddiffusionmodels_amd/csrc/pidm_launch.h
@@ -142,6 +142,16 @@
 int launch_act_fwd(const float* x, float* y, size_t n, int act, hipStream_t st);
 int launch_act_bwd(const float* x, const float* dy, float* dx, size_t n, int act, hipStream_t st);
 int launch_sinusoid(const int64_t* t, float* emb, int B, int dim, hipStream_t st);
+static const int kTimePathMaxLin = 34;
+struct TimePathTab {
+  const float* w[kTimePathMaxLin];
+  int off[kTimePathMaxLin + 1];
+  int n;
+};
+bool time_path_fused_ok(int B, int dim, int td, int nlin);
+int launch_time_path_fwd(const int64_t* t, const float* w1, const float* b1, const float* w2, const float* b2, const TimePathTab& tab,
+                         float* emb, float* h1, float* h1g, float* temb, float* st_out, float* ss, int B, int dim, int td, int ss_total,
+                         hipStream_t st);
 int launch_copy_add(float* dst, int ldd, const float* a, int lda, const float* b, int ldb, size_t rows, int cols, hipStream_t st);
 int launch_nchw_to_nhwc(const float* src, float* dst, int B, int C, int HW, const float* y_sig, hipStream_t st);
 size_t la_scratch_floats(int B, int N, int heads);
diff --git a/physicsinformeddiffusionmodels_amd/csrc/unet_engine.hip b/physicsinformeddiffusionmodels_amd/csrc/unet_engine.hip
--- a/physicsinformeddiffusionmodels_amd/csrc/unet_engine.hip
+++ b/physicsinformeddiffusionmodels_amd/csrc/unet_engine.hip
@@ -214,6 +214,7 @@
   bool side_allowed = false;
   bool side_pending = false;
   GraphCapture* cap = nullptr;
+  bool gout_cl = false;
   float* part_alloc(size_t bytes) { return defer_on ? defer.alloc(bytes / 4 + 64) : scratch; }
   ReduceQueue* q() { return defer_on ? &rq : nullptr; }
   WgradQueue* wgq() {
@@ -737,17 +738,34 @@
   U->x_in = x_nhwc;
   U->out_nchw = out_nchw;
   U->emb = act_alloc(r, (size_t)B * dim);
-  RUN(launch_sinusoid(t, U->emb, B, dim, r.st));
   U->h1 = act_alloc(r, (size_t)B * td);
-  if (conv_fwd(r, U->lin1, U->emb, nullptr, nullptr, U->h1)) return -1;
   U->h1g = act_alloc(r, (size_t)B * td);
-  RUN(launch_act_fwd(U->h1, U->h1g, (size_t)B * td, 1, r.st));
   U->temb = act_alloc(r, (size_t)B * td);
-  if (conv_fwd(r, U->lin2, U->h1g, nullptr, nullptr, U->temb)) return -1;
   U->st = act_alloc(r, (size_t)B * td);
-  RUN(launch_act_fwd(U->temb, U->st, (size_t)B * td, 0, r.st));
   U->ss = act_alloc(r, (size_t)B * U->ss_total);
-  if (conv_fwd(r, U->lincat, U->st, nullptr, nullptr, U->ss)) return -1;
+  int nlin = 0;
+  for (const auto& m : U->rb) nlin += m.has_mlp ? 1 : 0;
+  if (time_path_fused_ok(B, dim, td, nlin)) {
+    if (!r.dry) {
+      TimePathTab tab;
+      memset(&tab, 0, sizeof(tab));
+      for (const auto& m : U->rb) {
+        if (!m.has_mlp) continue;
+        tab.w[tab.n] = U->P[m.mlpw];
+        tab.off[tab.n++] = m.ss_off;
+      }
+      tab.off[tab.n] = U->ss_total;
+      RUN(launch_time_path_fwd(t, U->P[U->lin1.w], U->P[U->lin1.b], U->P[U->lin2.w], U->P[U->lin2.b], tab, U->emb, U->h1, U->h1g, U->temb,
+                               U->st, U->ss, B, dim, td, U->ss_total, r.st));
+    }
+  } else {
+    RUN(launch_sinusoid(t, U->emb, B, dim, r.st));
+    if (conv_fwd(r, U->lin1, U->emb, nullptr, nullptr, U->h1)) return -1;
+    RUN(launch_act_fwd(U->h1, U->h1g, (size_t)B * td, 1, r.st));
+    if (conv_fwd(r, U->lin2, U->h1g, nullptr, nullptr, U->temb)) return -1;
+    RUN(launch_act_fwd(U->temb, U->st, (size_t)B * td, 0, r.st));
+    if (conv_fwd(r, U->lincat, U->st, nullptr, nullptr, U->ss)) return -1;
+  }
 
   U->h0 = act_alloc(r, (size_t)B * P * P * dim);
   if (conv_fwd(r, U->init_conv, x_nhwc, nullptr, nullptr, U->h0)) return -1;
@@ -1204,7 +1222,8 @@
   const int n_phases = U->n_phases;
   float* dss = r.tmp.alloc((size_t)B * U->ss_total);
   float* g_o = r.tmp.alloc((size_t)B * HW * od);
-  RUN(launch_nchw_to_nhwc(grad_out_nchw, g_o, B, od, (int)HW, U->cfg.sigmoid_last_channel ? U->out_nchw : nullptr, r.st));
+  if (r.gout_cl) g_o = const_cast<float*>(grad_out_nchw);
+  else RUN(launch_nchw_to_nhwc(grad_out_nchw, g_o, B, od, (int)HW, U->cfg.sigmoid_last_channel ? U->out_nchw : nullptr, r.st));
   {
     const ConvLayer& L = U->final_conv;
     if (U->have_grads || r.dry) {
@@ -1580,9 +1599,10 @@
 }
 
 static int backward_body(pidm_unet* h, const float* grad_out_nchw, float* grad_x_nhwc, int B, void* workspace, size_t workspace_bytes,
-                         hipStream_t st, GraphCapture* cap) {
+                         hipStream_t st, GraphCapture* cap, bool gout_cl) {
   Run r;
   r.cap = cap;
+  r.gout_cl = gout_cl;
   if (setup_run(r, h, B, true, workspace, workspace_bytes, st, true)) return -1;
   r.side_allowed = backward_eager(widest_level(h));
   r.overlap = h->side_ok && !prof_enabled() && !cap && r.side_allowed;
@@ -1627,7 +1647,7 @@
   if (workspace_bytes < packed_region_bytes(h) + io_region(h, B, nullptr).total) return fail("unet: workspace too small");
   const IoRegion io = io_region(h, B, reinterpret_cast<char*>(workspace) + packed_region_bytes(h));
   if (x_nhwc != io.x && hipMemcpyAsync(io.x, x_nhwc, io.x_bytes, hipMemcpyDeviceToDevice, st) != hipSuccess) return fail("unet_forward: input copy failed");
-  if (hipMemcpyAsync(io.t, t, io.t_bytes, hipMemcpyDeviceToDevice, st) != hipSuccess) return fail("unet_forward: time-step copy failed");
+  if (t != io.t && hipMemcpyAsync(io.t, t, io.t_bytes, hipMemcpyDeviceToDevice, st) != hipSuccess) return fail("unet_forward: time-step copy failed");
   if (cond && hipMemcpyAsync(io.cond, cond, io.cond_bytes, hipMemcpyDeviceToDevice, st) != hipSuccess) return fail("unet_forward: condition copy failed");
   const float* cond_s = cond ? io.cond : nullptr;
   const uint64_t kw[11] = {0xF0, (uint64_t)B, (uint64_t)train, (uint64_t)(repack_weights != 0), (uint64_t)(cond != nullptr),
@@ -1665,9 +1685,26 @@
   return 0;
 }
 
-extern "C" int pidm_unet_backward(pidm_unet* h, const float* grad_out_nchw, float* grad_x_nhwc, int B, void* workspace,
-                                  size_t workspace_bytes, void* stream) {
+extern "C" int pidm_unet_io_addresses(const pidm_unet* h, int B, void* workspace, size_t workspace_bytes, void** x, void** t, void** out,
+                                      void** gout) {
+  if (!h || !workspace || B <= 0) return fail("unet_io_addresses: bad argument");
+  if (reinterpret_cast<uintptr_t>(workspace) & 255) return fail("unet: workspace must be 256-byte aligned");
+  if (workspace_bytes < packed_region_bytes(h) + io_region(h, B, nullptr).total) return fail("unet: workspace too small");
+  const IoRegion io = io_region(h, B, reinterpret_cast<char*>(workspace) + packed_region_bytes(h));
+  const char* e = knob("PIDM_FUSE_IO");
+  const bool on = !(e && !atoi(e));
+  if (x) *x = on ? io.x : nullptr;
+  if (t) *t = on ? io.t : nullptr;
+  if (out) *out = on ? io.out : nullptr;
+  if (gout) *gout = on ? io.gout : nullptr;
+  return 0;
+}
+
+static int unet_backward_any(pidm_unet* h, const float* grad_out_nchw, float* grad_x_nhwc, int B, void* workspace,
+                             size_t workspace_bytes, void* stream, bool gout_cl) {
   if (!h || !grad_out_nchw || !workspace) return fail("unet_backward: null argument");
+  if (gout_cl && h->cfg.sigmoid_last_channel)
+    return fail("unet_backward_cl: the sigmoid head's backward rides in the layout conversion (use pidm_unet_backward)");
   if (h->tape_B != B) return fail("unet_backward: no matching forward (tape holds B=%d)", h->tape_B);
   if (!h->have_grads) return fail("unet_backward: gradient buffers not bound");
   const hipStream_t st = as_stream(stream);
@@ -1691,12 +1728,12 @@
   if (grad_out_nchw != io.gout && hipMemcpyAsync(io.gout, grad_out_nchw, io.out_bytes, hipMemcpyDeviceToDevice, st) != hipSuccess)
     return fail("unet_backward: gradient copy failed");
   float* gx_s = grad_x_nhwc ? io.gx : nullptr;
-  const uint64_t kw[14] = {0xB0, (uint64_t)B, (uint64_t)(grad_x_nhwc != nullptr),
+  const uint64_t kw[15] = {0xB0, (uint64_t)B, (uint64_t)(grad_x_nhwc != nullptr),
                            (uint64_t)reinterpret_cast<uintptr_t>(workspace), (uint64_t)workspace_bytes, h->bind_sig, env_signature(),
                            h->fwd_key_hash, (uint64_t)h->n_phases, (uint64_t)reinterpret_cast<uintptr_t>(h->phase_ev[0]),
                            (uint64_t)reinterpret_cast<uintptr_t>(h->phase_ev[1]), (uint64_t)reinterpret_cast<uintptr_t>(h->phase_ev[2]),
-                           (uint64_t)h->tape_cond, (uint64_t)h->side_ok};
-  const std::vector<uint64_t> key(kw, kw + 14);
+                           (uint64_t)h->tape_cond, (uint64_t)h->side_ok, (uint64_t)gout_cl};
+  const std::vector<uint64_t> key(kw, kw + 15);
   int rc = -1;
   bool done = false;
   if (graphs_enabled() && !backward_eager(widest_level(h))) {
@@ -1709,7 +1746,7 @@
       GraphCapture cap;
       cap.entry = e;
       cap.user_st = st;
-      rc = backward_body(h, io.gout, gx_s, B, workspace, workspace_bytes, h->cap_stream, &cap);
+      rc = backward_body(h, io.gout, gx_s, B, workspace, workspace_bytes, h->cap_stream, &cap, gout_cl);
       cap_abort(h, &cap);
       if (rc == 0 && !cap.failed) {
         ++g_graph_captures;
@@ -1720,12 +1757,21 @@
       }
     }
   }
-  if (!done) rc = backward_body(h, io.gout, gx_s, B, workspace, workspace_bytes, st, nullptr);
+  if (!done) rc = backward_body(h, io.gout, gx_s, B, workspace, workspace_bytes, st, nullptr, gout_cl);
   if (rc == 0 && h->tape_cond) h->cond_grads_dirty = true;
   if (rc == 0 && grad_x_nhwc && grad_x_nhwc != io.gx &&
       hipMemcpyAsync(grad_x_nhwc, io.gx, io.x_bytes, hipMemcpyDeviceToDevice, st) != hipSuccess)
     return fail("unet_backward: input-gradient copy failed");
   return rc;
+}
+
+extern "C" int pidm_unet_backward(pidm_unet* h, const float* grad_out_nchw, float* grad_x_nhwc, int B, void* workspace,
+                                  size_t workspace_bytes, void* stream) {
+  return unet_backward_any(h, grad_out_nchw, grad_x_nhwc, B, workspace, workspace_bytes, stream, false);
+}
+extern "C" int pidm_unet_backward_cl(pidm_unet* h, const float* grad_out_nhwc, float* grad_x_nhwc, int B, void* workspace,
+                                     size_t workspace_bytes, void* stream) {
+  return unet_backward_any(h, grad_out_nhwc, grad_x_nhwc, B, workspace, workspace_bytes, stream, true);
 }
 
 extern "C" int pidm_debug_launch_counts(long long* out4) {
@@ -1734,6 +1780,15 @@
   out4[1] = pidm::g_graph_launches;
   out4[2] = pidm::g_graph_kernels;
   out4[3] = pidm::g_graph_captures;
+  return 0;
+}
+
+extern "C" long long pidm_unet_debug_time_path(const pidm_unet* h, float* ss_out, void* stream) {
+  if (!h || !h->ss || h->tape_B <= 0) return fail("unet_debug_time_path: no training-mode forward on this handle");
+  const size_t n = (size_t)h->tape_B * h->ss_total;
+  if (!ss_out) return (long long)n;
+  if (hipMemcpyAsync(ss_out, h->ss, n * sizeof(float), hipMemcpyDeviceToDevice, as_stream(stream)) != hipSuccess)
+    return fail("unet_debug_time_path: copy failed");
   return 0;
 }
 
diff --git a/physicsinformeddiffusionmodels_amd/denoising_utils.py b/physicsinformeddiffusionmodels_amd/denoising_utils.py
--- a/physicsinformeddiffusionmodels_amd/denoising_utils.py
+++ b/physicsinformeddiffusionmodels_amd/denoising_utils.py
@@ -318,38 +318,46 @@
 class _DarcyPidmLossFn(torch.autograd.Function):
 
     @staticmethod
-    def forward(ctx, x0_pred, x0, f_s, t, p2w_table, var_table, c_data, c_residual, inv_h0, inv_h1, lib):
+    def forward(ctx, x0_pred, x0, f_s, t, p2w_table, var_table, c_data, c_residual, inv_h0, inv_h1, lib, gout=None):
         pred = x0_pred.contiguous()
         B, C, P, _ = pred.shape
         dev = pred.device
         res = torch.empty(B, P * P, 3, dtype=torch.float32, device=dev)
-        grad = torch.empty_like(pred)
+        grad = torch.empty_like(pred) if gout is None else torch.empty_like(gout)
         out = torch.empty(4, dtype=torch.float32, device=dev)
         ws = torch.empty(lib.pidm_darcy_loss_ws(B, P), dtype=torch.uint8, device=dev)
-        lib.check(lib.pidm_darcy_loss_fwd_bwd_t(ptr(x0), ptr(pred), ptr(f_s), ptr(t), ptr(p2w_table), ptr(var_table),
-                                                float(c_data), float(c_residual), inv_h0, inv_h1, ptr(res), ptr(grad), ptr(out),
-                                                ptr(ws), B, P, stream_ptr(dev)), 'pidm_darcy_loss_fwd_bwd_t')
+        fn, what = ((lib.pidm_darcy_loss_fwd_bwd_t, 'pidm_darcy_loss_fwd_bwd_t') if gout is None else
+                    (lib.pidm_darcy_loss_fwd_bwd_t_cl, 'pidm_darcy_loss_fwd_bwd_t_cl'))
+        lib.check(fn(ptr(x0), ptr(pred), ptr(f_s), ptr(t), ptr(p2w_table), ptr(var_table), float(c_data), float(c_residual), inv_h0,
+                     inv_h1, ptr(res), ptr(grad), ptr(out), ptr(ws), B, P, stream_ptr(dev)), what)
         ctx.save_for_backward(grad)
+        ctx.gout = gout
+        ctx.image = P
         ctx.mark_non_differentiable(out, res)
         return out[0].clone(), out, res
 
     @staticmethod
     def backward(ctx, g_loss, _g_out, _g_res):
         (grad,) = ctx.saved_tensors
-        return grad * g_loss, None, None, None, None, None, None, None, None, None, None
+        if ctx.gout is None:
+            return grad * g_loss, None, None, None, None, None, None, None, None, None, None, None
+        gout, P = ctx.gout, ctx.image
+        torch.mul(grad, g_loss, out=gout)
+        return (gout.view(gout.shape[0], P, P, gout.shape[2]).permute(0, 3, 1, 2),
+                None, None, None, None, None, None, None, None, None, None, None)
 
 
 class _EarlyStepFn(torch.autograd.Function):
 
     @staticmethod
-    def forward(ctx, anchor, eng, diffusion, x_bxyc, t, loss_call):
+    def forward(ctx, anchor, eng, diffusion, x_bxyc, t, loss_call, direct=False):
         eng.tape_generation += 1
         ctx.generation = eng.tape_generation
-        pred = eng.forward(x_bxyc, t, training=True, early=True)
+        pred = eng.forward(x_bxyc, t, training=True, early=True, out_static=direct)
         grad, out = loss_call(pred)
         ctx.fetch = diffusion._start_scalar_fetch(out) if out.is_cuda else None
         loss_t = out[0].clone()
-        eng.backward(grad, False, x_bxyc.shape[-1])
+        eng.backward(grad, False, x_bxyc.shape[-1], channels_last=direct)
         eng.early_generation = ctx.generation
         eng.tape_busy = False
         ctx.eng = eng
@@ -381,7 +389,7 @@
                 p.grad = gv
             elif p.grad.data_ptr() != gv.data_ptr():
                 p.grad.add_(eng.early_views[i] * g)
-        return None, None, None, None, None, None
+        return None, None, None, None, None, None, None
 
 
 class DenoisingDiffusion(nn.Module):
@@ -611,7 +619,8 @@
         t = t.to(device=dev, dtype=torch.int64).contiguous()
         if residual_func._f_s_flat.device != dev:
             residual_func._f_s_flat = residual_func._f_s_flat.to(dev)
-        xt = torch.empty(B, P * P, C, dtype=torch.float32, device=dev)
+        io_eng, io = self._io_step_views(residual_func, B, C, P, dev)
+        xt = io[0] if io is not None else torch.empty(B, P * P, C, dtype=torch.float32, device=dev)
         lib.check(lib.pidm_qsample_nhwc_t(ptr(x_0), ptr(e.contiguous()), ptr(t), ptr(dd['alphas_bar_sqrt']),
                                           ptr(dd['one_minus_alphas_bar_sqrt']), ptr(xt), B, C, P * P, stream_ptr(dev)),
                   'pidm_qsample_nhwc_t')
@@ -619,17 +628,20 @@
         if eng is not None:
             f_s = residual_func._f_s_flat
 
+            direct = io is not None and io_eng is eng
+
             def loss_call(pred):
                 res = torch.empty(B, P * P, 3, dtype=torch.float32, device=dev)
-                grad = torch.empty_like(pred)
+                grad = io[3] if direct else torch.empty_like(pred)
                 out = torch.empty(4, dtype=torch.float32, device=dev)
                 ws = torch.empty(lib.pidm_darcy_loss_ws(B, P), dtype=torch.uint8, device=dev)
-                lib.check(lib.pidm_darcy_loss_fwd_bwd_t(ptr(x_0), ptr(pred), ptr(f_s), ptr(t), ptr(dd['p2_loss_weight']),
-                                                        ptr(dd['posterior_variance_clipped']), float(c_data), float(c_residual),
-                                                        residual_func.inv_h0, residual_func.inv_h1, ptr(res), ptr(grad), ptr(out), ptr(ws),
-                                                        B, P, stream_ptr(dev)), 'pidm_darcy_loss_fwd_bwd_t')
+                fn = lib.pidm_darcy_loss_fwd_bwd_t_cl if direct else lib.pidm_darcy_loss_fwd_bwd_t
+                lib.check(fn(ptr(x_0), ptr(pred), ptr(f_s), ptr(t), ptr(dd['p2_loss_weight']),
+                             ptr(dd['posterior_variance_clipped']), float(c_data), float(c_residual),
+                             residual_func.inv_h0, residual_func.inv_h1, ptr(res), ptr(grad), ptr(out), ptr(ws),
+                             B, P, stream_ptr(dev)), 'pidm_darcy_loss_fwd_bwd_t')
                 return grad, out
-            loss, scalars = _EarlyStepFn.apply(eng.params[0], eng, self, xt, t, loss_call)
+            loss, scalars = _EarlyStepFn.apply(eng.params[0], eng, self, xt, t, loss_call, direct)
             fetch, self._early_fetch = self._early_fetch, None
             if fetch is not None:
                 v = fetch.values()
@@ -646,8 +658,18 @@
             l_res, s_res, _res = _DarcyPidmLossFn.apply(x0_pred, x_0, *args, 0., c_residual, *geo)
             d, r = self._host_scalars(torch.stack((s_data, s_res)), [(0, 1), (1, 2)])
             return l_data + l_res, d, r, 0., 0.
-        x0_pred = residual_func.model(xt, t)
-        loss, scalars, _res = _DarcyPidmLossFn.apply(x0_pred, x_0, *args, c_data, c_residual, *geo)
+        if io is None:
+            x0_pred = residual_func.model(xt, t)
+            loss, scalars, _res = _DarcyPidmLossFn.apply(x0_pred, x_0, *args, c_data, c_residual, *geo)
+        else:
+            model = residual_func.model
+            model._pidm_out_static = True
+            try:
+                x0_pred = model(xt, t)
+            finally:
+                del model._pidm_out_static
+            loss, scalars, _res = _DarcyPidmLossFn.apply(x0_pred, x_0, *args, c_data, c_residual, *geo,
+                                                         io[3] if x0_pred.data_ptr() == io[2].data_ptr() else None)
         d, r = self._host_scalars(scalars, [(1,), (2,)])
         return loss, d, r, 0., 0.
 
@@ -665,6 +687,21 @@
                 tabs[k] = v
             cache[dev] = got = (self.diff_dict, tabs)
         return got[1]
+
+    def _io_step_views(self, residual_func, B, channels, image_size, dev):
+        from ._engine import get_engine
+        from .unet_model import Unet3D
+        model = residual_func.model
+        first = next(model.parameters())
+        if (residual_func.use_ddim_x0 or type(model) is not Unet3D or model.self_condition or model.sigmoid_last_channel
+                or channels != model.channels or model.out_dim != channels or not (first.is_cuda or self._lib is not None)
+                or model._forward_hooks or model._forward_pre_hooks or getattr(model, '_pidm_tape_slot', None)):
+            return None, None
+        eng = get_engine(model, image_size, model._pidm_lib)
+        if eng.tape_busy:
+            return None, None
+        training = torch.is_grad_enabled() and eng.params[0].requires_grad
+        return eng, eng.io_views(B, training, dev)
 
     def _early_backward_engine(self, residual_func, channels, image_size):
         from ._engine import get_engine
```
